# phuang1024/Starst3r

Measured on AMD Instinct MI355X. Metric: 3DGS train iters/sec @ 1M Gaussians, 8x1080p views, higher is better.
Workload: dtype f32

## Files before the change

starst3r_amd/csrc/api.hip:

```cpp
#include <stdarg.h>

#include "stages.h"

static thread_local char g_err[512] = "";

void st3r_set_error(const char* fmt, ...) {
    va_list ap;
    va_start(ap, fmt);
    vsnprintf(g_err, sizeof(g_err), fmt, ap);
    va_end(ap);
}

ST3R_EXPORT int st3r_version(void) { return ST3R_VERSION; }
ST3R_EXPORT const char* st3r_last_error(void) { return g_err; }

ST3R_EXPORT int st3r_ctx_create(int device, st3r_ctx** out) {
    ARG_CHECK(out);
    int ndev = 0;
    HIP_TRY(hipGetDeviceCount(&ndev));
    ARG_CHECK(device >= 0 && device < ndev);
    HIP_TRY(hipSetDevice(device));
    st3r_ctx* c = new (std::nothrow) st3r_ctx();
    if (!c) { st3r_set_error("out of host memory"); return ST3R_ERR_NOMEM; }
    memset(c, 0, sizeof(*c));
    c->device = device;
    hipError_t e = hipHostMalloc((void**)&c->pinned, 64 * sizeof(int64_t), hipHostMallocDefault);
    if (e != hipSuccess) { delete c; st3r_set_error("hipHostMalloc: %s", hipGetErrorString(e)); return ST3R_ERR_HIP; }
    *out = c;
    return ST3R_OK;
}

ST3R_EXPORT int st3r_ctx_destroy(st3r_ctx* ctx) {
    if (!ctx) return ST3R_OK;
    (void)hipSetDevice(ctx->device);
    (void)st3r_comm_destroy(ctx);
    for (int i = 0; i < SLOT_COUNT; ++i)
        if (ctx->slot_ptr[i]) (void)hipFree(ctx->slot_ptr[i]);
    if (ctx->pinned) (void)hipHostFree(ctx->pinned);
    if (ctx->count_event) (void)hipEventDestroy(ctx->count_event);
    if (ctx->peer_event) (void)hipEventDestroy(ctx->peer_event);
    if (ctx->comm_stream) {
        for (int j = 0; j < ST3R_MAX_RANGES; ++j) {
            (void)hipEventDestroy(ctx->ev_range_bwd[j]); (void)hipEventDestroy(ctx->ev_range_red[j]);
        }
        (void)hipStreamDestroy(ctx->comm_stream);
    }
    if (ctx->prof_ev[0][0][0])
        for (int r = 0; r < PROF_RING; ++r)
            for (int st = 0; st < STG_COUNT; ++st)
                for (int k = 0; k < 2; ++k) (void)hipEventDestroy(ctx->prof_ev[r][st][k]);
    delete ctx;
    return ST3R_OK;
}

ST3R_EXPORT int64_t st3r_ctx_arena_bytes(st3r_ctx* ctx) {
    if (!ctx) return 0;
    int64_t t = 0;
    for (int i = 0; i < SLOT_COUNT; ++i) t += (int64_t)ctx->slot_bytes[i];
    return t;
}

int st3r_arena_get(st3r_ctx* ctx, int slot, size_t bytes, void** out) {
    int grown;
    return st3r_arena_get2(ctx, slot, bytes, out, &grown);
}

int st3r_arena_get2(st3r_ctx* ctx, int slot, size_t bytes, void** out, int* grown) {
    *grown = 0;
    if (bytes == 0) bytes = 16;
    if (ctx->slot_bytes[slot] < bytes) {
        size_t want = bytes + bytes / 4;
        want = (want + 255) & ~(size_t)255;
        if (ctx->slot_ptr[slot]) {
            HIP_TRY(hipDeviceSynchronize());
            HIP_TRY(hipFree(ctx->slot_ptr[slot]));
            ctx->slot_ptr[slot] = nullptr; ctx->slot_bytes[slot] = 0;
        }
        hipError_t e = hipMalloc(&ctx->slot_ptr[slot], want);
        if (e != hipSuccess) {
            st3r_set_error("arena slot %d: hipMalloc(%zu) failed: %s", slot, want, hipGetErrorString(e));
            return ST3R_ERR_NOMEM;
        }
        ctx->slot_bytes[slot] = want;
        *grown = 1;
    }
    *out = ctx->slot_ptr[slot];
    return ST3R_OK;
}

ST3R_EXPORT int st3r_ctx_peek(st3r_ctx* ctx, void* stream, int which, void* dst, int64_t bytes) {
    ARG_CHECK(ctx && dst && bytes >= 0 && which >= 0 && which <= 13);
    static const int slots[14] = {SLOT_VALS_B, SLOT_OFFSETS, SLOT_SPLATS, SLOT_CUM,
                                  SLOT_MCMC_CUM, SLOT_MCMC_DEAD, SLOT_MCMC_SAMPLED, SLOT_MCMC_COUNT,
                                  SLOT_RGB, SLOT_ALPHA, SLOT_COUNTS, SLOT_KEYS_A, SLOT_VALS_A, SLOT_KEYS_B};
    ARG_CHECK((size_t)bytes <= ctx->slot_bytes[slots[which]]);
    HIP_TRY(hipMemcpyAsync(dst, ctx->slot_ptr[slots[which]], (size_t)bytes, hipMemcpyDeviceToDevice,
                           (hipStream_t)stream));
    return ST3R_OK;
}

static const char* k_stage_names[STG_COUNT] = {"project", "scan", "emit", "sort", "offsets", "blend_fwd", "loss",
                                               "blend_bwd", "project_bwd", "adam", "sort_depth"};

ST3R_EXPORT const char* st3r_stage_name(int stage) {
    return (stage >= 0 && stage < STG_COUNT) ? k_stage_names[stage] : "";
}

static void prof_harvest_slot(st3r_ctx* ctx, int slot) {
    for (int st = 0; st < STG_COUNT; ++st) {
        if (!ctx->prof_used[slot][st]) continue;
        float ms = 0.f;
        if (hipEventSynchronize(ctx->prof_ev[slot][st][1]) == hipSuccess &&
            hipEventElapsedTime(&ms, ctx->prof_ev[slot][st][0], ctx->prof_ev[slot][st][1]) == hipSuccess) {
            ctx->prof_ms[st] += ms; ctx->prof_n[st] += 1;
        }
        ctx->prof_used[slot][st] = 0;
    }
}

void st3r_prof_begin(st3r_ctx* ctx, hipStream_t s, int stage) {
    if (!((ctx->prof_enabled >> stage) & 1)) return;
    (void)hipEventRecord(ctx->prof_ev[ctx->prof_slot][stage][0], s);
}

void st3r_prof_end(st3r_ctx* ctx, hipStream_t s, int stage) {
    if (!((ctx->prof_enabled >> stage) & 1)) return;
    (void)hipEventRecord(ctx->prof_ev[ctx->prof_slot][stage][1], s);
    ctx->prof_used[ctx->prof_slot][stage] = 1;
}

void st3r_prof_next_step(st3r_ctx* ctx) {
    if (!ctx->prof_enabled) return;
    ctx->prof_slot = (ctx->prof_slot + 1) % PROF_RING;
    prof_harvest_slot(ctx, ctx->prof_slot);
}

ST3R_EXPORT int st3r_ctx_set_debug(st3r_ctx* ctx, int flags) {
    ARG_CHECK(ctx);
    ctx->debug_flags = flags;
    if (flags & 256) {
        ctx->scan_gen = (ctx->scan_gen & 1u) ? 0x3FFDu : 0x3FFEu;
        ctx->scan_gen_b = (ctx->scan_gen_b & 1u) ? 0x3FFDu : 0x3FFEu;
    }
    return ST3R_OK;
}

ST3R_EXPORT int st3r_ctx_set_profiling(st3r_ctx* ctx, int enable) {
    ARG_CHECK(ctx && enable >= 0 && enable < 2 + STG_COUNT);
    if (enable && !ctx->prof_ev[0][0][0]) {
        for (int r = 0; r < PROF_RING; ++r)
            for (int st = 0; st < STG_COUNT; ++st)
                for (int k = 0; k < 2; ++k) HIP_TRY(hipEventCreate(&ctx->prof_ev[r][st][k]));
    }
    ctx->prof_enabled = enable == 0 ? 0 : (enable == 1 ? (1 << STG_COUNT) - 1 : (1 << (enable - 2)));
    return ST3R_OK;
}

ST3R_EXPORT int st3r_ctx_get_stage_ms(st3r_ctx* ctx, double* ms_out, int64_t* counts_out) {
    ARG_CHECK(ctx && ms_out && counts_out);
    HIP_TRY(hipDeviceSynchronize());
    if (ctx->prof_ev[0][0][0])
        for (int r = 0; r < PROF_RING; ++r) prof_harvest_slot(ctx, r);
    for (int st = 0; st < STG_COUNT; ++st) {
        ms_out[st] = ctx->prof_ms[st]; counts_out[st] = ctx->prof_n[st];
        ctx->prof_ms[st] = 0; ctx->prof_n[st] = 0;
    }
    return ST3R_OK;
}

ST3R_EXPORT int st3r_ctx_settle(st3r_ctx* ctx) {
    ARG_CHECK(ctx);
    int rc = st3r_peer_status_settle(ctx);
    if (rc) return rc;
    return st3r_count_settle(ctx);
}

ST3R_EXPORT int st3r_ctx_release_scratch(st3r_ctx* ctx) {
    ARG_CHECK(ctx);
    HIP_TRY(hipDeviceSynchronize());
    const int rc = st3r_ctx_settle(ctx);
    for (int i = 0; i < SLOT_COUNT; ++i) {
        if (ctx->slot_ptr[i]) (void)hipFree(ctx->slot_ptr[i]);
        ctx->slot_ptr[i] = nullptr; ctx->slot_bytes[i] = 0;
    }
    return rc;
}

int st3r_counts_buffer(st3r_ctx* ctx, hipStream_t s, int32_t** out) {
    void* p; int grown = 0;
    int rc = st3r_arena_get2(ctx, SLOT_COUNTS, sizeof(int32_t) * 16, &p, &grown);
    if (rc) return rc;
    if (grown) HIP_TRY(hipMemsetAsync(p, 0, ctx->slot_bytes[SLOT_COUNTS], s));
    *out = (int32_t*)p;
    return ST3R_OK;
}
```

starst3r_amd/csrc/blend_common.h:

```cpp
#pragma once
#include "stages.h"
#include "tile_rect.h"

#define BLK 256
#define LOG2E 1.4426950408889634f

#ifndef XCD_GROUP
#define XCD_GROUP(C, n_tiles, tile_w) (tile_w)
#endif
__device__ __forceinline__ int xcd_remap(int bid, int total, int G) {
    const int n_full = (total / (8 * G)) * (8 * G);
    if (bid >= n_full) return bid;
    const int xcd = bid & 7, k = bid >> 3;
    const int round = k / G, within = k - round * G;
    return (round * 8 + xcd) * G + within;
}

struct TileGeom {
    int lb, cam, i, j, start, end, tx0, ty0;
    bool inside;
    float px, py;
};

__device__ __forceinline__ TileGeom tile_geom(int C, int W, int H, int tile_w, int tile_h,
                                              const int32_t* __restrict__ offsets, int n_isects) {
    TileGeom g;
    const int n_tiles = tile_w * tile_h, total = C * n_tiles;
    g.lb = xcd_remap(blockIdx.x, total, XCD_GROUP(C, n_tiles, tile_w));
    g.cam = g.lb / n_tiles;
    const int tile = g.lb - g.cam * n_tiles;
    const int ty = tile / tile_w, tx = tile - ty * tile_w;
    g.tx0 = tx * 16; g.ty0 = ty * 16;
    const int w = threadIdx.x >> 6, lane = threadIdx.x & 63;
    g.j = g.tx0 + ((w & 1) << 3) + (lane & 7);
    g.i = g.ty0 + ((w >> 1) << 3) + (lane >> 3);
    g.inside = (g.i < H) && (g.j < W);
    g.px = (float)g.j + 0.5f; g.py = (float)g.i + 0.5f;
    g.start = offsets[g.lb];
    g.end = (g.lb == total - 1 && n_isects >= 0) ? n_isects : offsets[g.lb + 1];
    return g;
}

__device__ __forceinline__ uint64_t uniform_u64(uint64_t v) {
    const unsigned lo = __builtin_amdgcn_readfirstlane((unsigned)v);
    const unsigned hi = __builtin_amdgcn_readfirstlane((unsigned)(v >> 32));
    return ((uint64_t)hi << 32) | lo;
}

__device__ __forceinline__ void stage_qform(const float4& a, const float4& b, const float4& c, int t, float4* sR) {
    sR[3 * t + 0] = make_float4(a.x, a.y, a.z, -0.5f * LOG2E * a.w);
    sR[3 * t + 1] = make_float4(-LOG2E * b.x, -0.5f * LOG2E * b.y, b.z, b.w);
    sR[3 * t + 2] = make_float4(c.x, 0.f, 0.f, 0.f);
}

__device__ __forceinline__ int quadrant_relevance(const float4& a, const float4& b, int tx0, int ty0) {
    EllipseTest et;
    if (!ellipse_prepare(a.z, a.w, b.x, b.y, &et)) return 0;
    const float rx = ((float)tx0 + 0.5f) - a.x, ry = ((float)ty0 + 0.5f) - a.y;
    int rel = 0;
#pragma unroll
    for (int q = 0; q < 4; ++q) {
        const float dx0 = rx + (float)((q & 1) * 8), dy0 = ry + (float)((q >> 1) * 8);
        rel |= ellipse_hits_square(et, dx0, dx0 + 7.0f, dy0, dy0 + 7.0f) ? (1 << q) : 0;
    }
    return rel;
}

__device__ __forceinline__ int64_t mask_base(int lb, int start) { return (int64_t)(start >> 6) + 4 * (int64_t)lb; }

__device__ __forceinline__ float blend_power(float dx, float dy, float qa, float qb, float qc) {
#pragma clang fp contract(off)
    const float lx = __builtin_fmaf(dx, qa, qb * dy);
    return __builtin_fmaf(dx, lx, (qc * dy) * dy);
}

__device__ __forceinline__ uint64_t mask_not_less(float a, float b) {
    uint64_t m;
    asm("v_cmp_nlt_f32_e64 %0, %1, %2" : "=s"(m) : "v"(a), "v"(b));
    return m;
}
__device__ __forceinline__ uint64_t mask_not_positive(float a) {
    uint64_t m;
    asm("v_cmp_nlt_f32_e64 %0, 0, %1" : "=s"(m) : "v"(a));
    return m;
}
__device__ __forceinline__ float zero_unless(uint64_t m, float x) {
    float r;
    asm("s_nop 1\n\tv_cndmask_b32_e64 %0, 0, %1, %2" : "=v"(r) : "v"(x), "s"(m));
    return r;
}

__device__ __forceinline__ void reduce9_rows(float g0, float g1, float g2, float g3, float g4, float g5, float g6,
                                             float g7, float g8, float& k0, float& k1, float& k2) {
    float t0, t1, t2, t3, t4;
    asm volatile(
        "s_nop 1\n\t"
        "v_add_f32_dpp %0, %5, %5 row_ror:8 row_mask:0xf bank_mask:0x3\n\t"
        "v_add_f32_dpp %1, %7, %7 row_ror:8 row_mask:0xf bank_mask:0x3\n\t"
        "v_add_f32_dpp %2, %9, %9 row_ror:8 row_mask:0xf bank_mask:0x3\n\t"
        "v_add_f32_dpp %3, %11, %11 row_ror:8 row_mask:0xf bank_mask:0x3\n\t"
        "v_add_f32_dpp %4, %13, %13 row_ror:8 row_mask:0xf bank_mask:0x3\n\t"
        "v_add_f32_dpp %0, %6, %6 row_ror:8 row_mask:0xf bank_mask:0xc\n\t"
        "v_add_f32_dpp %1, %8, %8 row_ror:8 row_mask:0xf bank_mask:0xc\n\t"
        "v_add_f32_dpp %2, %10, %10 row_ror:8 row_mask:0xf bank_mask:0xc\n\t"
        "v_add_f32_dpp %3, %12, %12 row_ror:8 row_mask:0xf bank_mask:0xc"
        : "=&v"(t0), "=&v"(t1), "=&v"(t2), "=&v"(t3), "=&v"(t4)
        : "v"(g0), "v"(g1), "v"(g2), "v"(g3), "v"(g4), "v"(g5), "v"(g6), "v"(g7), "v"(g8));
    float u0, u1, u2;
    asm volatile(
        "s_nop 1\n\t"
        "v_add_f32_dpp %0, %3, %3 row_shl:4 row_mask:0xf bank_mask:0x5\n\t"
        "v_add_f32_dpp %1, %5, %5 row_shl:4 row_mask:0xf bank_mask:0x5\n\t"
        "v_add_f32_dpp %2, %7, %7 row_shl:4 row_mask:0xf bank_mask:0x1\n\t"
        "v_add_f32_dpp %0, %4, %4 row_shr:4 row_mask:0xf bank_mask:0xa\n\t"
        "v_add_f32_dpp %1, %6, %6 row_shr:4 row_mask:0xf bank_mask:0xa"
        : "=&v"(u0), "=&v"(u1), "=&v"(u2)
        : "v"(t0), "v"(t1), "v"(t2), "v"(t3), "v"(t4));
    asm volatile(
        "s_nop 1\n\t"
        "v_add_f32_dpp %0, %0, %0 quad_perm:[1,0,3,2] row_mask:0xf bank_mask:0xf\n\t"
        "v_add_f32_dpp %1, %1, %1 quad_perm:[1,0,3,2] row_mask:0xf bank_mask:0xf\n\t"
        "v_add_f32_dpp %2, %2, %2 quad_perm:[1,0,3,2] row_mask:0xf bank_mask:0xf\n\t"
        "v_add_f32_dpp %0, %0, %0 quad_perm:[2,3,0,1] row_mask:0xf bank_mask:0xf\n\t"
        "v_add_f32_dpp %1, %1, %1 quad_perm:[2,3,0,1] row_mask:0xf bank_mask:0xf\n\t"
        "v_add_f32_dpp %2, %2, %2 quad_perm:[2,3,0,1] row_mask:0xf bank_mask:0xf"
        : "+v"(u0), "+v"(u1), "+v"(u2));
    k0 = u0; k1 = u1; k2 = u2;
}
#define ACC_VALS 9
#define VT_STRIDE (ACC_VALS + 1)
#define DACC_VALS 7
#define DVT_STRIDE (DACC_VALS + 1)
#ifndef HB
#define HB 64
#endif
#define HB_WORDS (HB / 64)
static_assert(HB == 64, "the backward walks one mask word per round");
#ifndef CHUNK
#define CHUNK 4
#endif
#define PAIR_STRIDE 66
#define PAIR_AT(pix) ((pix) + ((pix) >> 5))

__device__ __forceinline__ int slot_of_rectbase(uint64_t r, int tx0, int ty0) {
    const int x0 = (int)(r & 0x3FF), y0 = (int)((r >> 10) & 0x3FF), rw = (int)((r >> 20) & 0x3FF);
    return (int)(r >> 32) + ((ty0 >> 4) - y0) * rw + ((tx0 >> 4) - x0);
}
__device__ __forceinline__ int slot_of_rect(int cum_excl, int x0, int y0, int rw, int tx0, int ty0) {
    return cum_excl + ((ty0 >> 4) - y0) * rw + ((tx0 >> 4) - x0);
}

struct RunSums { float So, Sx, Sxx, Sy, Sxy, Syy; };
__device__ __forceinline__ RunSums run_sums(float W0, float W1, float W2, float d0, float dy) {
    const float So = W0, Sx = fmaf(d0, W0, -W1), Sxx = fmaf(d0, Sx - W1, W2);
    const float Sy = So * dy, Sxy = Sx * dy, Syy = Sy * dy;
    return RunSums{So, Sx, Sxx, Sy, Sxy, Syy};
}

__device__ __forceinline__ void wave_lds_sync() {
    __builtin_amdgcn_fence(__ATOMIC_SEQ_CST, "wavefront");
    __builtin_amdgcn_wave_barrier();
}

__device__ __forceinline__ void store_pair_sums(float4* dst, const float (&acc)[ACC_VALS]) {
    dst[0] = make_float4(acc[0], acc[1], acc[2], acc[3]);
    dst[1] = make_float4(acc[4], acc[5], acc[6], acc[7]);
    dst[2] = make_float4(acc[8], 0.f, 0.f, 0.f);
}
__device__ __forceinline__ void store_pair_sums(float4* dst, const float (&acc)[DACC_VALS]) {
    dst[0] = make_float4(acc[0], acc[1], acc[2], acc[3]);
    dst[1] = make_float4(acc[4], acc[5], 0.f, 0.f);
    dst[2] = make_float4(0.f, acc[6], 0.f, 0.f);
}

template <int NV>
__global__ __launch_bounds__(256) void k_gather_vtile(int64_t n_pairs, const int32_t* __restrict__ cum,
                                                      const float* __restrict__ vtile, int stamp, unsigned vt_cap,
                                                      float4* __restrict__ v_splats) {
    static_assert(NV & 1, "the stamp closes the slot's last 8-byte word");
    constexpr int ROW = NV;
    constexpr int NQ = (NV + 1) / 2;
    __shared__ int sCum[257];
    __shared__ float sVal[256 * ROW];
    const int tid = threadIdx.x;
    const int64_t p0 = (int64_t)blockIdx.x * 256;
    const int np = (int)min((int64_t)256, n_pairs - p0);
    if (tid == 0) sCum[0] = p0 == 0 ? 0 : cum[p0 - 1];
    sCum[tid + 1] = cum[p0 + min(tid, np - 1)];
    __syncthreads();
    const int s0 = sCum[0], s1 = sCum[np];
    const int my_start = sCum[tid], my_end = tid < np ? sCum[tid + 1] : sCum[tid];
    float acc[NV];
#pragma unroll
    for (int k = 0; k < NV; ++k) acc[k] = 0.f;
    float2 q[NQ];
    auto fetch = [&](int u) {
#pragma unroll
        for (int k = 0; k < NQ; ++k) q[k] = make_float2(0.f, 0.f);
        if (u < s1 && (unsigned)u < vt_cap) {
            const float2* src = reinterpret_cast<const float2*>(vtile + (int64_t)u * (NV + 1));
#pragma unroll
            for (int k = 0; k < NQ; ++k) q[k] = src[k];
        }
    };
    fetch(s0 + tid);
    for (int base = s0; base < s1; base += 256) {
        const bool live = __float_as_int(q[NQ - 1].y) == stamp;
        float* row = sVal + tid * ROW;
#pragma unroll
        for (int k = 0; k < NV; ++k) row[k] = live ? ((k & 1) ? q[k >> 1].y : q[k >> 1].x) : 0.f;
        __syncthreads();
        fetch(base + 256 + tid);
        const int lo = max(my_start, base) - base, hi = min(my_end, base + 256) - base;
        for (int r = lo; r < hi; ++r) {
            const float* src = sVal + r * ROW;
#pragma unroll
            for (int k = 0; k < NV; ++k) acc[k] += src[k];
        }
        __syncthreads();
    }
    if (tid < np) store_pair_sums(v_splats + (p0 + tid) * 3, acc);
}

static inline int64_t cmask_words(int64_t n_isects, int64_t total) { return (n_isects >> 6) + 4 * total + 8; }

static int hand_off_buffers(st3r_ctx* ctx, int64_t total, int64_t n_isects, bool allocate, uint64_t** cmask,
                            int64_t* words, int32_t** tile_nb) {
    *words = cmask_words(n_isects, total);
    const size_t cm_bytes = sizeof(uint64_t) * 4 * (size_t)*words, nb_bytes = sizeof(int32_t) * (size_t)total;
    if (allocate) {
        void* p; int rc;
        if ((rc = st3r_arena_get(ctx, SLOT_CMASK, cm_bytes, &p)) || (rc = st3r_arena_get(ctx, SLOT_TILE_NB, nb_bytes, &p)))
            return rc;
    } else if (!ctx->slot_ptr[SLOT_CMASK] || ctx->slot_bytes[SLOT_CMASK] < cm_bytes || !ctx->slot_ptr[SLOT_TILE_NB] ||
               ctx->slot_bytes[SLOT_TILE_NB] < nb_bytes) {
        st3r_set_error("st3r_gs_blend_depth_bwd must follow st3r_gs_blend_fwd of the same lists on the same ctx");
        return ST3R_ERR_INVALID;
    }
    *cmask = (uint64_t*)ctx->slot_ptr[SLOT_CMASK];
    *tile_nb = (int32_t*)ctx->slot_ptr[SLOT_TILE_NB];
    return ST3R_OK;
}

struct StampedSlots { float* vtile; int stamp; unsigned cap; bool restarted; };
static int stamped_slots(st3r_ctx* ctx, hipStream_t s, int slot, int stride, int64_t n_isects, int* stamp_counter,
                         StampedSlots* out) {
    void* p; int grown = 0;
    int rc = st3r_arena_get2(ctx, slot, sizeof(float) * stride * (size_t)n_isects, &p, &grown);
    if (rc) return rc;
    const bool restart = grown || *stamp_counter >= 2147483000;
    if (restart) {
        HIP_TRY(hipMemsetAsync(p, 0, ctx->slot_bytes[slot], s));
        *stamp_counter = 0;
    }
    *out = StampedSlots{(float*)p, ++*stamp_counter, (unsigned)(ctx->slot_bytes[slot] / (sizeof(float) * stride)), restart};
    return ST3R_OK;
}

static int check_blend_args(st3r_ctx* ctx, int C, int width, int height, int tile_size, int tile_w, int tile_h,
                            const float* splats, const int32_t* offsets, const int32_t* flatten_ids, int64_t n_isects) {
    ARG_CHECK(ctx && C > 0 && width > 0 && height > 0 && tile_size == 16);
    ARG_CHECK(tile_w == (width + 15) / 16 && tile_h == (height + 15) / 16);
    ARG_CHECK(splats && offsets && n_isects >= 0 && n_isects < 2147483647LL);
    ARG_CHECK(n_isects == 0 || flatten_ids);
    return ST3R_OK;
}
```

starst3r_amd/csrc/common.h:

```cpp
#pragma once
#include <hip/hip_runtime.h>
#include <stdint.h>
#include <stdio.h>
#include <string.h>

#include "../../include/st3r.h"

#define ST3R_EXPORT extern "C" __attribute__((visibility("default")))

void st3r_set_error(const char* fmt, ...);

#define HIP_TRY(expr)                                                                              \
    do {                                                                                           \
        hipError_t _e = (expr);                                                                    \
        if (_e != hipSuccess) {                                                                    \
            st3r_set_error("%s:%d: %s -> %s", __FILE__, __LINE__, #expr, hipGetErrorString(_e));   \
            return ST3R_ERR_HIP;                                                                   \
        }                                                                                          \
    } while (0)

#define ARG_CHECK(cond)                                                                    \
    do {                                                                                   \
        if (!(cond)) {                                                                     \
            st3r_set_error("%s:%d: invalid argument: %s", __FILE__, __LINE__, #cond);      \
            return ST3R_ERR_INVALID;                                                       \
        }                                                                                  \
    } while (0)

#define LAUNCH_CHECK() HIP_TRY(hipGetLastError())

enum ArenaSlot {
    SLOT_SPLATS = 0,
    SLOT_TILES,
    SLOT_CUM,
    SLOT_KEYS_A,
    SLOT_KEYS_B,
    SLOT_VALS_A,
    SLOT_VALS_B,
    SLOT_OFFSETS,
    SLOT_RGB,
    SLOT_ALPHA,
    SLOT_LAST,
    SLOT_VRENDER,
    SLOT_VSPLATS,
    SLOT_SSIM_A,
    SLOT_SORT_TMP,
    SLOT_SCAN_TMP,
    SLOT_SMALL,
    SLOT_CMASK,
    SLOT_TILE_NB,
    SLOT_VTILE,
    SLOT_DKEYS_A,
    SLOT_DKEYS_B,
    SLOT_DVALS_A,
    SLOT_DVALS_B,
    SLOT_CUM_D,
    SLOT_NN_PART,
    SLOT_MCMC_CUM,
    SLOT_MCMC_DEAD,
    SLOT_MCMC_RANK,
    SLOT_MCMC_COUNT,
    SLOT_MCMC_SAMPLED,
    SLOT_MCMC_BINOMS,
    SLOT_REG_PART,
    SLOT_RECTS,
    SLOT_RECTS_D,
    SLOT_RECTBASE,
    SLOT_COUNTS,
    SLOT_PSTAGE,
    SLOT_GSTAGE,
    SLOT_ALIGN_CTL,
    SLOT_PAIR_TOUCH,
    SLOT_KRANGE_PART,
    SLOT_SCAN_CHAIN,
    SLOT_POSE_PART,
    SLOT_VTILE_DEPTH,
    SLOT_DEPTH_PART,
    SLOT_POSE_GRAD,
    SLOT_DEPTH,
    SLOT_VDEPTH,
    SLOT_VALPHA,
    SLOT_VSPLATS_D,
    SLOT_DPRIOR_PART,
    SLOT_DPRIOR_NORM,
    SLOT_DPRIOR_SUMS,
    SLOT_EXPOSURE_PART,
    SLOT_SCAN_CHAIN_B,
    SLOT_EXPOSED,
    SLOT_KGRAD_PART,
    SLOT_LWEIGHT_PART,
    SLOT_LWEIGHT_NORM,
    SLOT_COUNT
};

enum Stage {
    STG_PROJECT = 0,
    STG_SCAN,
    STG_EMIT,
    STG_SORT,
    STG_OFFSETS,
    STG_BLEND_FWD,
    STG_LOSS,
    STG_BLEND_BWD,
    STG_PROJECT_BWD,
    STG_ADAM,
    STG_SORT_DEPTH,
    STG_COUNT
};
#define PROF_RING 64
#define ST3R_MAX_RANGES 8

#define ST3R_SPLIT_VIEWS 1000

struct st3r_vtile_ref { const int32_t* cum; const float* vtile; int stamp; unsigned vt_cap; const uint32_t* touch; };

struct ViewReg { const float* gt; int c, h, w; };

static inline int64_t view_reg_first(const ViewReg& r, const float* gt, int C, int H, int W) {
    if (!r.gt || H != r.h || W != r.w) return -1;
    const int64_t img = (int64_t)H * W * 3;
    if (gt < r.gt || (gt - r.gt) % img != 0) return -1;
    const int64_t c0 = (gt - r.gt) / img;
    return c0 + C <= r.c ? c0 : -1;
}

static inline int view_reg_set(ViewReg* r, bool on, const float* gt, int C, int height, int width) {
    if (!on) { *r = ViewReg{}; return ST3R_OK; }
    ARG_CHECK(C > 0 && height > 0 && width > 0);
    *r = ViewReg{gt, C, height, width};
    return ST3R_OK;
}

struct st3r_ctx {
    int device;
    void* slot_ptr[SLOT_COUNT];
    size_t slot_bytes[SLOT_COUNT];
    int64_t* pinned;
    int debug_flags;
    ViewReg gtm; const float* gtm_mom;
    ViewReg dp; const float* dp_depth; const float* dp_weight; float dp_fac; int dp_norm_valid;
    ViewReg ex; const float* ex_exposure; float* ex_v_exposure;
    ViewReg kg; float* kg_v_Ks;
    ViewReg lw; const float* lw_weight; int lw_norm_valid;
    int bwd_stamp;
    int depth_stamp;
    uint32_t scan_gen;
    uint32_t scan_gen_b;
    int64_t isect_hint, count_cap;
    int64_t hint_sig;
    int count_pending;
    int view_chunks;
    hipEvent_t count_event;
    void* comm;
    int comm_owned, comm_rank, comm_size;
    int exchange;
    int comm_broken;
    int peer_pending;
    hipEvent_t peer_event;
    hipStream_t comm_stream;
    hipEvent_t ev_range_bwd[ST3R_MAX_RANGES], ev_range_red[ST3R_MAX_RANGES];
    void* xwin;
    int n_ranges;
    int ranges_recorded;
    int prof_enabled;
    hipEvent_t prof_ev[PROF_RING][STG_COUNT][2];
    unsigned char prof_used[PROF_RING][STG_COUNT];
    int prof_slot;
    double prof_ms[STG_COUNT];
    int64_t prof_n[STG_COUNT];
};

void st3r_prof_begin(st3r_ctx* ctx, hipStream_t s, int stage);
void st3r_prof_end(st3r_ctx* ctx, hipStream_t s, int stage);
void st3r_prof_next_step(st3r_ctx* ctx);

int st3r_arena_get(st3r_ctx* ctx, int slot, size_t bytes, void** out);
int st3r_arena_get2(st3r_ctx* ctx, int slot, size_t bytes, void** out, int* grown);
#define ARENA_GET(slot, type, count, var)                                                    \
    type* var;                                                                               \
    {                                                                                        \
        void* _p;                                                                            \
        int _rc = st3r_arena_get(ctx, slot, sizeof(type) * (size_t)(count), &_p);            \
        if (_rc) return _rc;                                                                 \
        var = (type*)_p;                                                                     \
    }

#define ST3R_BAND_TAB 257

static inline int ceil_div(int64_t a, int64_t b) { return (int)((a + b - 1) / b); }
static inline int bit_length_u32(uint32_t v) { int n = 0; while (v) { ++n; v >>= 1; } return n; }
```

starst3r_amd/csrc/fused_step.hip:

```cpp
#include "radix_sort.h"
#include "stages.h"

int st3r_count_settle(st3r_ctx* ctx) {
    if (!ctx->count_pending) return ST3R_OK;
    HIP_TRY(hipEventSynchronize(ctx->count_event));
    ctx->count_pending = 0;
    const int64_t n = (int64_t)((int32_t*)(ctx->pinned + 8))[0];
    if (n < 0) {
        ctx->isect_hint = 0;
        ctx->view_chunks = (ctx->view_chunks > 0 ? ctx->view_chunks : 1) * 2;
        st3r_set_error("the previous step produced more than 2^31 tile intersections: its gradients were incomplete -- "
                       "repeat it (st3r_gs_train_fwd_bwd / st3r_gs_train_step now walk the views in %d chunks)",
                       ctx->view_chunks);
        return ST3R_ERR_CAPACITY;
    }
    if (n > ctx->count_cap) {
        ctx->isect_hint = 0;
        st3r_set_error("the previous step produced %lld tile intersections, more than the %lld its buffers were sized "
                       "for from the step before (+25 %%): its gradients were incomplete and st3r_adam_step / "
                       "st3r_gs_train_step did NOT apply them (the update is guarded on the device) -- repeat that step",
                       (long long)n, (long long)ctx->count_cap);
        return ST3R_ERR_CAPACITY;
    }
    ctx->isect_hint = n;
    return ST3R_OK;
}

struct FrontPlan {
    int tile_w, tile_h;
    bool key32;
    bool segments;
    int rect32;
    bool rectbase;
    uint32_t key_base;
    int l1_end_bit;
    int end_bit;
};
static const float k_near_plane = 0.01f, k_far_plane = 1e10f;
static FrontPlan front_plan(int C, int W, int H, int debug_flags, bool with_reg, bool records) {
    FrontPlan p;
    const int tile = 16;
    p.tile_w = (W + tile - 1) / tile; p.tile_h = (H + tile - 1) / tile;
    uint32_t near_bits, far_bits;
    memcpy(&near_bits, &k_near_plane, 4); memcpy(&far_bits, &k_far_plane, 4);
    p.key32 = (C <= 8) && (far_bits - near_bits < 0x1FFFFFFFu);
    p.key_base = p.key32 ? near_bits : 0u;
    p.rect32 = (p.tile_w <= 255 && p.tile_h <= 255 && !(debug_flags & 64)) ? 1 : 0;
    p.segments = p.key32 && with_reg && !records && !(debug_flags & 4);
    p.l1_end_bit = (p.key32 ? 29 : 32) + bit_length_u32((uint32_t)(C - 1));
    p.rectbase = p.tile_w <= 1023 && p.tile_h <= 1023 && !(debug_flags & 64);
    p.end_bit = bit_length_u32((uint32_t)((int64_t)C * p.tile_w * p.tile_h - 1));
    return p;
}

static int rasterize_front(st3r_ctx* ctx, hipStream_t s, const GsParams& g, const GsViews& v, double* reg_sums, int tight,
                           const float* records_in, bool allow_async, RasterOut* o, double* loss_sums = nullptr) {
    const int N = g.N, C = v.C, W = v.W, H = v.H;
    const int tile = 16;
    const FrontPlan fp = front_plan(C, W, H, ctx->debug_flags, reg_sums != nullptr, records_in != nullptr);
    const int tile_w = fp.tile_w, tile_h = fp.tile_h;
    const int64_t n_pairs = (int64_t)N * C;
    float* splats = const_cast<float*>(records_in);
    if (!records_in) {
        ARENA_GET(SLOT_SPLATS, float, n_pairs * ST3R_SPLAT_STRIDE, own);
        splats = own;
    }
    ARENA_GET(SLOT_CUM, int32_t, n_pairs, cum);
    ARENA_GET(SLOT_OFFSETS, int32_t, (int64_t)C * tile_w * tile_h + 1, offsets);
    const float near_plane = k_near_plane, far_plane = k_far_plane;
    const bool key32 = fp.key32;
    ARENA_GET(SLOT_DKEYS_A, uint64_t, n_pairs, dkeys_a);
    ARENA_GET(SLOT_DKEYS_B, uint64_t, n_pairs, dkeys_b);
    ARENA_GET(SLOT_DVALS_A, int32_t, n_pairs, dvals_a);
    ARENA_GET(SLOT_DVALS_B, int32_t, n_pairs, perm);
    const int rect32 = fp.rect32;
    ARENA_GET(SLOT_RECTS, uint64_t, rect32 ? (n_pairs + 1) / 2 : n_pairs, rects);
    int32_t* counts = nullptr;
    { int rc_ = st3r_counts_buffer(ctx, s, &counts); if (rc_) return rc_; }
    uint32_t* const krange = fp.segments ? (uint32_t*)(counts + 8) : nullptr;
    st3r_prof_begin(ctx, s, STG_PROJECT);
    const uint32_t key_base = fp.key_base;
    int rc = records_in
                 ? st3r_records_prepare_impl(s, N, C, splats, tile, tile_w, tile_h, tight, nullptr, dkeys_a, dvals_a,
                                             key_base, rects, rect32)
                 : st3r_project_impl(ctx, s, g, v, tile, 0.3f, near_plane, far_plane, 0.0f, splats, nullptr, reg_sums,
                                     dkeys_a, dvals_a, tight, key_base, rects, rect32, 1, loss_sums, 2 * C, krange);
    if (!rc && records_in && loss_sums) HIP_TRY(hipMemsetAsync(loss_sums, 0, sizeof(double) * 2 * (size_t)C, s));
    st3r_prof_end(ctx, s, STG_PROJECT);
    if (rc) return rc;
    st3r_prof_begin(ctx, s, STG_SORT_DEPTH);
    rc = krange ? st3r_radix_sort_u32_segments(ctx, s, N, C, (uint32_t*)dkeys_a, dvals_a, (uint32_t*)dkeys_b, perm, krange)
         : key32 ? st3r_radix_sort_u32(ctx, s, n_pairs, 0, fp.l1_end_bit, (uint32_t*)dkeys_a, dvals_a, (uint32_t*)dkeys_b, perm, nullptr)
                 : st3r_radix_sort_u64(ctx, s, n_pairs, 0, fp.l1_end_bit, dkeys_a, dvals_a, dkeys_b, perm);
    st3r_prof_end(ctx, s, STG_SORT_DEPTH);
    if (rc) return rc;
    int64_t n_isects = 0;
    st3r_prof_begin(ctx, s, STG_SCAN);
    uint64_t* rectbase = nullptr;
    if (fp.rectbase) {
        ARENA_GET(SLOT_RECTBASE, uint64_t, n_pairs, rb);
        rectbase = rb;
    }
    const int64_t sig = ((int64_t)N << 34) ^ ((int64_t)C << 26) ^ ((int64_t)W << 13) ^ (int64_t)H;
    const bool async = allow_async && ctx->isect_hint > 0 && ctx->hint_sig == sig;
    int32_t* total_dev = nullptr;
    rc = st3r_isect_scan_impl(ctx, s, n_pairs, nullptr, cum, nullptr, rects, rect32, rectbase, &total_dev,
                              async ? counts : nullptr, async ? (int32_t*)(ctx->pinned + 8) : nullptr);
    st3r_prof_end(ctx, s, STG_SCAN);
    if (rc) return rc;
    if (async) {
        if (!ctx->count_event) HIP_TRY(hipEventCreateWithFlags(&ctx->count_event, hipEventDisableTiming));
        HIP_TRY(hipEventRecord(ctx->count_event, s));
        n_isects = ctx->isect_hint + ctx->isect_hint / 4 + 1024;
        if (ctx->debug_flags & 8) n_isects = ctx->isect_hint / 2;
        if (n_isects > 2147483647LL) n_isects = 2147483647LL;
        ctx->count_pending = 1; ctx->count_cap = n_isects;
        o->n_visible = -1; o->n_isects_ref = -1;
    } else {
        HIP_TRY(hipMemcpyAsync(ctx->pinned, total_dev, sizeof(int32_t), hipMemcpyDeviceToHost, s));
        if (reg_sums) HIP_TRY(hipMemcpyAsync(ctx->pinned + 1, reg_sums + 2, 2 * sizeof(double), hipMemcpyDeviceToHost, s));
        HIP_TRY(hipStreamSynchronize(s));
        n_isects = (int64_t)((int32_t*)ctx->pinned)[0];
        if (n_isects < 0) {
            st3r_set_error("more than 2^31 tile intersections in one call: split the views over more calls / GPUs");
            return ST3R_SPLIT_VIEWS;
        }
        o->n_visible = reg_sums ? (int64_t)((double*)ctx->pinned)[1] : -1;
        o->n_isects_ref = reg_sums ? (int64_t)((double*)ctx->pinned)[2] : n_isects;
        if (allow_async) { ctx->isect_hint = n_isects; ctx->hint_sig = sig; }
    }
    ARENA_GET(SLOT_KEYS_A, uint32_t, n_isects, tkeys_a);
    ARENA_GET(SLOT_KEYS_B, uint32_t, n_isects, tkeys_b);
    ARENA_GET(SLOT_VALS_A, int32_t, n_isects, vals_a);
    ARENA_GET(SLOT_VALS_B, int32_t, n_isects, vals_b);
    o->n_records = async ? -1 : n_isects;
    const int64_t n_keys = (int64_t)C * tile_w * tile_h;
    const uint32_t* band_table = nullptr;
    const uint32_t* band_hist = nullptr;
    int n_bands = 0;
    if (n_isects > 0) {
        const int end_bit = fp.end_bit;
        const bool banded = st3r_sort_tile_banded(end_bit, ctx->debug_flags) != 0;
        const bool packed = banded && n_pairs <= (1 << 24) && !(ctx->debug_flags & 1024);
        n_bands = (int)((n_keys - 1) >> 8) + 1;
        st3r_prof_begin(ctx, s, STG_EMIT);
        rc = st3r_isect_emit_chain_impl(ctx, s, N, C, perm, rects, rect32, tile_w, tile_h, packed ? nullptr : tkeys_a, vals_a,
                                        n_isects, banded ? st3r_radix_sort_band_tile(n_isects) : 0, total_dev, &band_table);
        st3r_prof_end(ctx, s, STG_EMIT);
        if (rc) return rc;
        st3r_prof_begin(ctx, s, STG_SORT);
        rc = packed ? st3r_radix_sort_u32_banded_packed(ctx, s, n_isects, n_bands, band_table, (const uint32_t*)vals_a, vals_b,
                                                        &band_hist)
             : banded ? st3r_radix_sort_u32_banded(ctx, s, n_isects, n_bands, band_table, tkeys_a, vals_a, tkeys_b, vals_b)
                      : st3r_sort_tile_impl(ctx, s, n_isects, end_bit, tkeys_a, vals_a, tkeys_b, vals_b, total_dev);
        st3r_prof_end(ctx, s, STG_SORT);
        if (rc) return rc;
    }
    st3r_prof_begin(ctx, s, STG_OFFSETS);
    rc = band_hist ? st3r_radix_band_offsets(s, n_bands, band_table, band_hist, n_keys, offsets)
                   : st3r_isect_offsets32_impl(s, n_isects, tkeys_b, C, tile_w, tile_h, offsets, total_dev);
    st3r_prof_end(ctx, s, STG_OFFSETS);
    if (rc) return rc;
    o->C = C; o->W = W; o->H = H; o->tile_w = tile_w; o->tile_h = tile_h;
    o->splats = splats; o->offsets = offsets; o->flat = vals_b; o->cum = cum; o->rects = rect32 ? nullptr : rects;
    o->rectbase = rectbase;
    o->tight = tight; o->n_pairs = n_pairs;
    o->n_isects = n_isects;
    return ST3R_OK;
}

__global__ void k_finalize_loss(int C, const double* __restrict__ sums, const double* __restrict__ reg_sums,
                                double inv_px, double inv_cnt, double w_l1, double w_ssim, double reg_views,
                                double opac_k, double scale_k, float* __restrict__ loss_out,
                                const double* __restrict__ dsums, const double* __restrict__ dnorm, double depth_fac,
                                const double* __restrict__ wnorm) {
    if (threadIdx.x == 0 && blockIdx.x == 0) {
        double loss = 0;
        if (wnorm)
            for (int c = 0; c < C; ++c)
                loss += w_l1 * sums[2 * c] / (3.0 * fmax(wnorm[2 * c], 1.0)) +
                        w_ssim * (3.0 * wnorm[2 * c + 1] - sums[2 * c + 1]) / (3.0 * fmax(wnorm[2 * c + 1], 1.0));
        else
            for (int c = 0; c < C; ++c) loss += w_l1 * sums[2 * c] * inv_px + w_ssim * (1.0 - sums[2 * c + 1] * inv_cnt);
        loss += reg_views * (opac_k * reg_sums[0] + scale_k * reg_sums[1]);
        if (dsums)
            for (int c = 0; c < C; ++c) loss += depth_fac * dsums[c] / dnorm[c];
        loss_out[0] = (float)loss;
    }
}

static int finalize_loss(hipStream_t s, int C, int H, int W, const double* sums, const double* reg_sums, float ssim_fac,
                         double reg_views, double opac_k, double scale_k, float* loss_out, const double* dp_sums,
                         const DepthPrior& dp, const LossWeight& lw) {
    const int Hi = H - 10, Wi = W - 10;
    const double cnt = (Hi > 0 && Wi > 0) ? (double)Hi * Wi * 3 : 0.0;
    hipLaunchKernelGGL(k_finalize_loss, dim3(1), dim3(64), 0, s, C, sums, reg_sums, 1.0 / ((double)H * W * 3),
                       cnt > 0 ? 1.0 / cnt : 0.0, (double)(1.0f - ssim_fac), (double)ssim_fac, reg_views, opac_k, scale_k,
                       loss_out, dp_sums, dp.norm, (double)dp.fac, lw.weight ? lw.norm : nullptr);
    LAUNCH_CHECK();
    return ST3R_OK;
}

struct LossFacs { float ssim, opac, scale; };

struct ViewBatch {
    GsViews v;
    const float* gt;
    double* sums;
    double* dp_sums;
    float* v_viewmats;
    bool exposure;
    bool weighted;
    ViewBatch slice(int c0, int c1) const {
        return {v.slice(c0, c1), gt + (int64_t)c0 * v.H * v.W * 3, sums + 2 * c0, dp_sums ? dp_sums + c0 : nullptr,
                v_viewmats ? v_viewmats + 16 * c0 : nullptr, exposure, weighted};
    }
};

struct StepImages { float *rgb, *alpha; int32_t* last; float *v_rgb, *depth, *v_depth, *v_alpha, *exposed; };

static int step_images(st3r_ctx* ctx, const RasterOut& ro, bool with_depth, bool with_exposure, StepImages* im) {
    const int64_t n_px = (int64_t)ro.C * ro.H * ro.W;
    ARENA_GET(SLOT_RGB, float, n_px * 3, rgb);
    ARENA_GET(SLOT_ALPHA, float, n_px, alpha);
    ARENA_GET(SLOT_LAST, int32_t, n_px, last);
    ARENA_GET(SLOT_VRENDER, float, n_px * 3, v_rgb);
    *im = StepImages{rgb, alpha, last, v_rgb, nullptr, nullptr, nullptr, nullptr};
    if (with_exposure) {
        ARENA_GET(SLOT_EXPOSED, float, n_px * 3, exposed);
        im->exposed = exposed;
    }
    if (with_depth) {
        ARENA_GET(SLOT_DEPTH, float, n_px, depth);
        ARENA_GET(SLOT_VDEPTH, float, n_px, v_depth);
        ARENA_GET(SLOT_VALPHA, float, n_px, v_alpha);
        im->depth = depth; im->v_depth = v_depth; im->v_alpha = v_alpha;
    }
    return ST3R_OK;
}

static int forward_and_losses(st3r_ctx* ctx, hipStream_t s, const RasterOut& ro, const ViewBatch& b, float ssim_fac,
                              bool sums_cleared, const DepthPrior& dp, const ExposureReg& ex, const LossWeight& lw,
                              const StepImages& im) {
    const bool eio = true;
    st3r_prof_begin(ctx, s, STG_BLEND_FWD);
    int rc = st3r_blend_fwd_impl(ctx, s, ro, im.rgb, im.alpha, im.last, true, eio);
    if (!rc && dp.prior) rc = st3r_blend_depth_fwd_impl(ctx, s, ro, im.last, im.depth, eio);
    st3r_prof_end(ctx, s, STG_BLEND_FWD);
    if (rc) return rc;
    st3r_prof_begin(ctx, s, STG_LOSS);
    if (ex.exposure) rc = st3r_exposure_fwd_impl(s, ro.C, ro.H, ro.W, im.rgb, ex.exposure, im.exposed);
    if (!rc)
        rc = st3r_loss_impl(ctx, s, ro.C, ro.H, ro.W, ex.exposure ? im.exposed : im.rgb, b.gt, 1.0f - ssim_fac, ssim_fac,
                            b.sums, im.v_rgb, sums_cleared, lw);
    if (!rc && ex.exposure)
        rc = st3r_exposure_bwd_impl(ctx, s, ro.C, ro.H, ro.W, im.rgb, ex.exposure, im.v_rgb, im.v_rgb, ex.v_exposure);
    if (!rc && dp.prior)
        rc = st3r_depth_prior_loss_impl(ctx, s, ro.C, ro.H, ro.W, im.depth, im.alpha, dp.prior, dp.weight, dp.norm, 1, dp.fac,
                                        b.dp_sums, 1, im.v_depth, im.v_alpha);
    st3r_prof_end(ctx, s, STG_LOSS);
    return rc;
}

static int blend_backward(st3r_ctx* ctx, hipStream_t s, const RasterOut& ro, const StepImages& im, bool need_pairs,
                          st3r_vtile_ref* slots, float* v_pairs) {
    RasterOut rb = ro;
    if (ctx->debug_flags & 2) { rb.rects = nullptr; rb.rectbase = nullptr; }
    const bool eio = true;
    st3r_prof_begin(ctx, s, STG_BLEND_BWD);
    int rc = st3r_blend_bwd_impl(ctx, s, rb, im.alpha, im.last, im.v_rgb, im.v_alpha, nullptr, eio, slots);
    if (!rc && need_pairs) {
        ARENA_GET(SLOT_VSPLATS_D, float, ro.n_pairs * ST3R_SPLAT_STRIDE, v_pairs_d);
        rc = st3r_blend_depth_bwd_impl(ctx, s, rb, im.alpha, im.last, im.v_depth, v_pairs_d, eio);
        if (!rc) {
            if (slots->vtile) rc = st3r_gather_vtile_impl(s, ro.n_pairs, slots, v_pairs);
            else HIP_TRY(hipMemsetAsync(v_pairs, 0, sizeof(float) * ST3R_SPLAT_STRIDE * (size_t)ro.n_pairs, s));
        }
        if (!rc) rc = st3r_add_pairs_impl(s, ro.n_pairs, v_pairs, v_pairs_d);
    }
    st3r_prof_end(ctx, s, STG_BLEND_BWD);
    return rc;
}

static int project_backward(st3r_ctx* ctx, hipStream_t s, const GsParams& g, const GsViews& v, const RasterOut& ro,
                            const LossFacs& f, const float* v_pairs, const st3r_vtile_ref* slots, bool accumulate,
                            float* grads) {
    ctx->ranges_recorded = 0;
    if (!(ctx->n_ranges > 1 && ctx->comm_stream))
        return st3r_project_sh_bwd_impl(s, g, v, 0.3f, ro.splats, v_pairs, (float)v.C, f.opac, f.scale, grads, accumulate, 0,
                                        -1, false, slots);
    ARENA_GET(SLOT_GSTAGE, float, (int64_t)23 * g.N, gstage);
    const int K = ctx->n_ranges;
    for (int j = 0; j < K; ++j) {
        const int g0 = (int)((int64_t)g.N * j / K), g1 = (int)((int64_t)g.N * (j + 1) / K);
        int rc = st3r_project_sh_bwd_impl(s, g, v, 0.3f, ro.splats, v_pairs, (float)v.C, f.opac, f.scale, gstage, accumulate,
                                          g0, g1, true, slots);
        if (rc) return rc;
        HIP_TRY(hipEventRecord(ctx->ev_range_bwd[j], s));
    }
    ctx->ranges_recorded = K;
    return ST3R_OK;
}

static int pose_backward(st3r_ctx* ctx, hipStream_t s, const GsParams& g, const GsViews& v, const RasterOut& ro,
                         const float* v_pairs, float* v_viewmats) {
    return st3r_gs_viewmat_bwd(ctx, s, g.N, v.C, g.means, g.quats, g.scales, g.sh, g.sh_stride, v.viewmats, v.Ks, v.campos,
                               v.W, v.H, 0.3f, ro.splats, v_pairs, v_viewmats);
}

static int train_views(st3r_ctx* ctx, hipStream_t s, const GsParams& g, const ViewBatch& b, const LossFacs& f,
                       double* reg_sums, bool allow_async, bool accumulate, float* grads, RasterOut* ro_out) {
    const GsViews& v = b.v;
    DepthPrior dp{};
    int rc = b.dp_sums ? st3r_depth_prior_for(ctx, s, b.gt, v.C, v.H, v.W, &dp) : ST3R_OK;
    if (rc) return rc;
    ExposureReg ex{};
    if (b.exposure) st3r_exposure_for(ctx, b.gt, v.C, v.H, v.W, &ex);
    LossWeight lw{};
    if (b.weighted) rc = st3r_loss_weight_for(ctx, s, b.gt, v.C, v.H, v.W, &lw);
    if (rc) return rc;
    const bool need_pairs = dp.prior != nullptr;
    RasterOut& ro = *ro_out;
    rc = rasterize_front(ctx, s, g, v, reg_sums, 1, nullptr, allow_async, &ro, b.sums);
    if (rc) return rc;
    StepImages im;
    rc = step_images(ctx, ro, need_pairs, ex.exposure != nullptr, &im);
    if (rc) return rc;
    float* const v_Ks = st3r_intrinsics_grad_for(ctx, b.gt, v.C, v.H, v.W);
    float* v_pairs = nullptr;
    if (need_pairs || b.v_viewmats || v_Ks) {
        ARENA_GET(SLOT_VSPLATS, float, ro.n_pairs * ST3R_SPLAT_STRIDE, vp);
        v_pairs = vp;
    }
    rc = forward_and_losses(ctx, s, ro, b, f.ssim, true, dp, ex, lw, im);
    if (rc) return rc;
    st3r_vtile_ref slots{};
    rc = blend_backward(ctx, s, ro, im, need_pairs, &slots, v_pairs);
    if (rc) return rc;
    st3r_prof_begin(ctx, s, STG_PROJECT_BWD);
    rc = project_backward(ctx, s, g, v, ro, f, need_pairs ? v_pairs : nullptr, need_pairs ? nullptr : &slots, accumulate,
                          grads);
    if (!rc && need_pairs && b.v_viewmats) rc = pose_backward(ctx, s, g, v, ro, v_pairs, b.v_viewmats);
    if (!rc && need_pairs) rc = st3r_gs_depth_bwd(ctx, s, g.N, v.C, g.means, v.viewmats, ro.splats, v_pairs, grads, b.v_viewmats);
    st3r_prof_end(ctx, s, STG_PROJECT_BWD);
    if (!rc && !need_pairs && (b.v_viewmats || v_Ks)) {
        rc = st3r_gather_vtile_impl(s, ro.n_pairs, &slots, v_pairs);
        if (!rc && b.v_viewmats) rc = pose_backward(ctx, s, g, v, ro, v_pairs, b.v_viewmats);
    }
    if (!rc && v_Ks)
        rc = st3r_gs_intrinsics_bwd(ctx, s, g.N, v.C, g.means, g.quats, g.scales, v.viewmats, v.Ks, v.W, v.H, 0.3f,
                                    ro.splats, v_pairs, v_Ks);
    return rc;
}

static int train_chunks(st3r_ctx* ctx, hipStream_t s, const GsParams& g, const ViewBatch& all, const LossFacs& f,
                        double* reg_sums, double* reg_scratch, bool want_stats, float* grads, int* chunks, int64_t stats[3]) {
    const int C = all.v.C;
    for (;;) {
        int rc = ST3R_OK;
        stats[0] = stats[1] = stats[2] = 0;
        bool first = true;
        for (int k = 0; k < *chunks && !rc; ++k) {
            const int c0 = (int)((int64_t)k * C / *chunks), c1 = (int)((int64_t)(k + 1) * C / *chunks);
            if (c1 == c0) continue;
            RasterOut ro;
            rc = train_views(ctx, s, g, all.slice(c0, c1), f, first ? reg_sums : reg_scratch,
                             !want_stats && *chunks == 1 && !ctx->comm, !first, grads, &ro);
            if (!rc) { stats[0] += ro.n_visible; stats[1] += ro.n_records; stats[2] += ro.n_isects_ref; }
            first = false;
        }
        if (rc == ST3R_SPLIT_VIEWS && *chunks < C) {
            *chunks = *chunks * 2 < C ? *chunks * 2 : C;
            continue;
        }
        return rc == ST3R_SPLIT_VIEWS ? ST3R_ERR_INVALID : rc;
    }
}

int st3r_train_fwd_bwd_impl(st3r_ctx* ctx, hipStream_t s, const GsParams& g, const GsViews& v, const float* gt_images,
                            float ssim_fac, float opac_fac, float scale_fac, float* grads, float* loss_out,
                            int64_t* stats_host, float* v_viewmats) {
    const int N = g.N, C = v.C;
    ARG_CHECK(ctx && N > 0 && C > 0 && C <= ST3R_MAX_VIEWS && v.W > 0 && v.H > 0 && g.sh_stride >= 12);
    ARG_CHECK((int64_t)N * C < 2147483647LL);
    ARG_CHECK(g.means && g.quats && g.scales && g.opacities && g.sh && v.viewmats && v.Ks && v.campos && gt_images && grads &&
              loss_out);
    ARENA_GET(SLOT_SMALL, double, 2 * (size_t)C + 12, small);
    double* sums = small;
    double* reg_sums = small + 2 * C;
    double* dp_sums = nullptr;
    DepthPrior dp;
    int rc = st3r_depth_prior_for(ctx, s, gt_images, C, v.H, v.W, &dp);
    if (rc) return rc;
    if (dp.prior) {
        if (ctx->comm) {
            st3r_set_error("a depth prior is registered and a communicator is attached -- the depth term is not "
                           "supported in view-sharded training (clear it with st3r_ctx_set_depth_prior(ctx, NULL, ...))");
            return ST3R_ERR_INVALID;
        }
        ARENA_GET(SLOT_DPRIOR_SUMS, double, (size_t)C, ds);
        dp_sums = ds;
    }
    ExposureReg ex;
    st3r_exposure_for(ctx, gt_images, C, v.H, v.W, &ex);
    if (ex.exposure && ctx->comm) {
        st3r_set_error("exposures are registered and a communicator is attached -- per-view exposures are not supported "
                       "in view-sharded training (clear them with st3r_ctx_set_exposure(ctx, NULL, ...))");
        return ST3R_ERR_INVALID;
    }
    if (ctx->comm && st3r_intrinsics_grad_for(ctx, gt_images, C, v.H, v.W)) {
        st3r_set_error("an intrinsics gradient is registered and a communicator is attached -- intrinsics refinement is "
                       "not supported in view-sharded training (clear it with st3r_ctx_set_intrinsics_grad(ctx, NULL, ...))");
        return ST3R_ERR_INVALID;
    }
    LossWeight lw;
    rc = st3r_loss_weight_for(ctx, s, gt_images, C, v.H, v.W, &lw);
    if (rc) return rc;
    if (lw.weight && ctx->comm) {
        st3r_set_error("loss weights are registered and a communicator is attached -- per-pixel loss weights are not "
                       "supported in view-sharded training (clear them with st3r_ctx_set_loss_weight(ctx, NULL, ...))");
        return ST3R_ERR_INVALID;
    }
    st3r_prof_next_step(ctx);
    rc = st3r_count_settle(ctx);
    if (rc) return rc;
    int chunks = ctx->view_chunks > 0 ? ctx->view_chunks : 1;
    if ((ctx->debug_flags & 32) && chunks < 2) chunks = 2;
    if (chunks > C) chunks = C;
    int64_t stats[3];
    rc = train_chunks(ctx, s, g, ViewBatch{v, gt_images, sums, dp_sums, v_viewmats, ex.exposure != nullptr, lw.weight != nullptr},
                      LossFacs{ssim_fac, opac_fac, scale_fac},
                      reg_sums, reg_sums + 4, stats_host != nullptr, grads, &chunks, stats);
    if (rc) return rc;
    if (chunks > 1) ctx->view_chunks = chunks;
    rc = finalize_loss(s, C, v.H, v.W, sums, reg_sums, ssim_fac, (double)C, (double)opac_fac / N,
                       (double)scale_fac / (3.0 * N), loss_out, dp_sums, dp, lw);
    if (rc) return rc;
    if (stats_host) {
        stats_host[0] = stats[0]; stats_host[1] = stats[1]; stats_host[2] = st3r_ctx_arena_bytes(ctx);
        stats_host[3] = stats[2];
    }
    return ST3R_OK;
}

ST3R_EXPORT int st3r_gs_train_fwd_bwd(st3r_ctx* ctx, void* stream, int N, int C, const float* means,
                                      const float* quats, const float* scales, const float* opacities,
                                      const float* sh, int sh_stride, const float* viewmats, const float* Ks,
                                      const float* campos, const float* gt_images, int width, int height,
                                      float ssim_fac, float opac_fac, float scale_fac, float* grads,
                                      float* loss_out, int64_t* stats_host) {
    return st3r_train_fwd_bwd_impl(ctx, (hipStream_t)stream, GsParams{N, means, quats, scales, opacities, sh, sh_stride},
                                   GsViews{C, width, height, viewmats, Ks, campos}, gt_images, ssim_fac, opac_fac,
                                   scale_fac, grads, loss_out, stats_host, nullptr);
}

ST3R_EXPORT int st3r_gs_raster_train(st3r_ctx* ctx, void* stream, int N, int C, const float* records,
                                     const float* gt_images, int width, int height, float ssim_fac,
                                     float* v_records, float* loss_out, int64_t* stats_host) {
    ARG_CHECK(ctx && N > 0 && C > 0 && width > 0 && height > 0 && records && gt_images && v_records && loss_out);
    ARG_CHECK(C <= ST3R_MAX_VIEWS && (int64_t)N * C < 2147483647LL);
    hipStream_t s = (hipStream_t)stream;
    ARENA_GET(SLOT_SMALL, double, 2 * (size_t)C + 8, sums);
    double* reg_sums = sums + 2 * C;
    const ViewBatch b{GsViews{C, width, height}, gt_images, sums, nullptr, nullptr, false, false};
    HIP_TRY(hipMemsetAsync(reg_sums, 0, sizeof(double) * 4, s));
    st3r_prof_next_step(ctx);
    RasterOut ro;
    int rc = st3r_count_settle(ctx);
    if (rc) return rc;
    rc = rasterize_front(ctx, s, GsParams{N}, b.v, nullptr, 1, records, stats_host == nullptr, &ro);
    if (rc == ST3R_SPLIT_VIEWS) rc = ST3R_ERR_INVALID;
    if (rc) return rc;
    StepImages im;
    rc = step_images(ctx, ro, false, false, &im);
    if (rc) return rc;
    rc = forward_and_losses(ctx, s, ro, b, ssim_fac, false, DepthPrior{}, ExposureReg{}, LossWeight{}, im);
    if (rc) return rc;
    st3r_prof_begin(ctx, s, STG_BLEND_BWD);
    rc = st3r_blend_bwd_impl(ctx, s, ro, im.alpha, im.last, im.v_rgb, nullptr, v_records, true, nullptr);
    st3r_prof_end(ctx, s, STG_BLEND_BWD);
    if (rc) return rc;
    rc = finalize_loss(s, C, height, width, sums, reg_sums, ssim_fac, 0.0, 0.0, 0.0, loss_out, nullptr, DepthPrior{},
                       LossWeight{});
    if (rc) return rc;
    if (stats_host) {
        stats_host[0] = -1; stats_host[1] = ro.n_records; stats_host[2] = st3r_ctx_arena_bytes(ctx); stats_host[3] = -1;
    }
    return ST3R_OK;
}

ST3R_EXPORT int st3r_gs_render(st3r_ctx* ctx, void* stream, int N, int C, const float* means, const float* quats,
                               const float* scales, const float* opacities, const float* sh, int sh_stride,
                               const float* viewmats, const float* Ks, const float* campos, int width, int height,
                               float* rgb, float* alpha, int64_t* stats_host) {
    ARG_CHECK(ctx && N > 0 && C > 0 && width > 0 && height > 0 && sh_stride >= 12);
    ARG_CHECK(C <= ST3R_MAX_VIEWS && (int64_t)N * C < 2147483647LL);
    ARG_CHECK(means && quats && scales && opacities && sh && viewmats && Ks && campos && rgb && alpha);
    hipStream_t s = (hipStream_t)stream;
    RasterOut ro;
    int rc = st3r_count_settle(ctx);
    if (rc) return rc;
    rc = rasterize_front(ctx, s, GsParams{N, means, quats, scales, opacities, sh, sh_stride},
                         GsViews{C, width, height, viewmats, Ks, campos}, nullptr, 0, nullptr, false, &ro);
    if (rc == ST3R_SPLIT_VIEWS) rc = ST3R_ERR_INVALID;
    if (rc) return rc;
    ARENA_GET(SLOT_LAST, int32_t, (int64_t)C * height * width, last);
    rc = st3r_blend_fwd_impl(ctx, s, ro, rgb, alpha, last, false, true);
    if (rc) return rc;
    if (stats_host) {
        stats_host[0] = -1; stats_host[1] = ro.n_records; stats_host[2] = st3r_ctx_arena_bytes(ctx); stats_host[3] = 0;
    }
    return ST3R_OK;
}

ST3R_EXPORT int st3r_front_plan(int N, int C, int width, int height, int debug_flags, int training, int records,
                                int64_t n_records, int64_t* out, int n_out) {
    ARG_CHECK(N > 0 && C > 0 && C <= ST3R_MAX_VIEWS && width > 0 && height > 0 && n_records >= 0 && out &&
              n_out >= ST3R_FRONT_PLAN_WORDS && !(training && records));
    const FrontPlan fp = front_plan(C, width, height, debug_flags, training != 0, records != 0);
    const int64_t n_pairs = (int64_t)N * C;
    for (int i = 0; i < n_out; ++i) out[i] = 0;
    out[0] = fp.rect32; out[1] = fp.rectbase; out[2] = fp.key32; out[3] = fp.segments;
    out[4] = st3r_scan_tiles(n_pairs);
    int bpc, grid, self_base;
    st3r_emit_grid(N, C, &bpc, &grid, &self_base);
    out[5] = bpc; out[6] = grid; out[7] = self_base;
    int64_t sh[8];
    if (fp.segments) st3r_radix_sort_shape(4, n_pairs, N, C, 0, 0, sh);
    else st3r_radix_sort_shape(fp.key32 ? 4 : 8, n_pairs, 0, 0, 0, fp.l1_end_bit, sh);
    out[8] = sh[0]; out[9] = sh[1]; out[10] = sh[2]; out[11] = sh[3]; out[12] = sh[4];
    out[25] = sh[5];
    out[fp.key32 ? 26 : 28] = sh[6]; out[fp.key32 ? 27 : 29] = sh[7];
    st3r_radix_sort_shape(fp.key32 ? 8 : 4, 1, 0, 0, 0, 8, sh);
    out[fp.key32 ? 28 : 26] = sh[6]; out[fp.key32 ? 29 : 27] = sh[7];
    out[13] = st3r_sort_tile_end_bit(fp.end_bit);
    if (n_records > 0) {
        st3r_radix_sort_shape(4, n_records, 0, 0, 0, (int)out[13], sh);
        out[14] = sh[0]; out[15] = sh[1]; out[16] = sh[2]; out[17] = sh[4];
    }
    if (st3r_sort_tile_banded(fp.end_bit, debug_flags)) {
        out[18] = 1;
        out[19] = (((int64_t)C * fp.tile_w * fp.tile_h - 1) >> 8) + 1;
        if (n_records > 0) out[30] = n_records / st3r_radix_sort_band_tile(n_records) + out[19];
    }
    int64_t k[5];
    st3r_isect_constants(k);
    for (int i = 0; i < 5; ++i) out[20 + i] = k[i];
    return ST3R_OK;
}
```

starst3r_amd/csrc/gs_blend.hip:

```cpp
#include <type_traits>

#include "stages.h"
#include "tile_rect.h"
#include "blend_common.h"

__device__ __forceinline__ int stage_record(const float4* __restrict__ splats, int64_t id, int t, int tx0, int ty0,
                                            float4* sR) {
    const float4 a = splats[id * 3 + 0];
    const float4 b = splats[id * 3 + 1];
    const float4 c = splats[id * 3 + 2];
    stage_qform(a, b, c, t, sR);
    return quadrant_relevance(a, b, tx0, ty0);
}

template <bool TRAIN>
__global__ __launch_bounds__(BLK) void k_blend_fwd(int C, int W, int H, int tile_w, int tile_h,
                                                   const float4* __restrict__ splats,
                                                   const int32_t* __restrict__ offsets,
                                                   const int32_t* __restrict__ flat, int n_isects,
                                                   float* __restrict__ out_rgb, float* __restrict__ out_alpha,
                                                   int32_t* __restrict__ last_ids,
                                                   uint64_t* __restrict__ cmask, int64_t cmask_words,
                                                   int32_t* __restrict__ tile_nb, int no_cull) {
    __shared__ float4 sR[BLK * 3];
    __shared__ uint64_t sMask[4][4];
    const TileGeom g = tile_geom(C, W, H, tile_w, tile_h, offsets, n_isects);
    const int w = threadIdx.x >> 6, lane = threadIdx.x & 63;
    float thr = g.inside ? 1.f / 255.f : __builtin_inff();
    float T = 1.0f, r = 0.f, gg = 0.f, b = 0.f;
    int cur = TRAIN ? 0x7fffffff : 0;
    int nb = 0;
    const int64_t mbase = mask_base(g.lb, g.start);
    for (int bs = g.start; bs < g.end; bs += BLK, ++nb) {
        if (__syncthreads_and(thr > 1.0f)) break;
        const int idx = bs + threadIdx.x;
        int rel = 0;
        if (idx < g.end) {
            rel = stage_record(splats, flat[idx], threadIdx.x, g.tx0, g.ty0, sR);
            if (no_cull) rel = 0xF;
        }
        const uint64_t m0 = __ballot(rel & 1), m1 = __ballot(rel & 2), m2 = __ballot(rel & 4), m3 = __ballot(rel & 8);
        if (lane == 0) { sMask[0][w] = m0; sMask[1][w] = m1; sMask[2][w] = m2; sMask[3][w] = m3; }
        __syncthreads();
#pragma unroll 1
        for (int jj = 0; jj < 4; ++jj) {
            uint64_t m64 = uniform_u64(sMask[w][jj]);
            uint64_t contributed = 0;
            if (__builtin_amdgcn_ballot_w64(thr < 1.0f) == 0) m64 = 0;
#pragma unroll 1
            for (int hh = 0; hh < 2; ++hh) {
            uint32_t m = hh ? (uint32_t)(m64 >> 32) : (uint32_t)m64;
            uint32_t cont32 = 0;
            while (m) {
                const int bit = __builtin_ctz(m);
                m &= m - 1;
                const int t = jj * 64 + hh * 32 + bit;
                const float4 a = sR[3 * t];
                const float4 q = sR[3 * t + 1];
                const float cb = sR[3 * t + 2].x;
                const float dx = a.x - g.px, dy = a.y - g.py;
                const float P = blend_power(dx, dy, a.w, q.x, q.y);
                const float al0 = fminf(0.999f, a.z * __builtin_amdgcn_exp2f(P));
                uint64_t okm = 0;
                bool ok = false;
                float al;
                if (TRAIN) {
                    okm = mask_not_positive(P) & mask_not_less(al0, thr);
                    al = zero_unless(okm, al0);
                } else {
                    ok = !(P > 0.f) && !(al0 < thr);
                    al = ok ? al0 : 0.f;
                }
                const float nT = T * (1.0f - al);
                const bool stop = nT <= 1e-4f;
                float vis = al * T;
                uint64_t tm;
                if (TRAIN) {
                    tm = okm;
                    float Tn = nT;
                    if (__builtin_expect(__builtin_amdgcn_ballot_w64(stop) != 0, 0)) {
                        thr = stop ? __builtin_inff() : thr;
                        vis = stop ? 0.0f : vis;
                        Tn = stop ? T : nT;
                        cur = stop ? bs + t : cur;
                        tm = okm & ~__builtin_amdgcn_ballot_w64(stop);
                    }
                    T = Tn;
                } else {
                    thr = stop ? __builtin_inff() : thr;
                    al = stop ? 0.0f : al;
                    vis = al * T;
                    T = stop ? T : nT;
                    const bool took = al > 0.0f;
                    cur = took ? bs + t : cur;
                    tm = __builtin_amdgcn_ballot_w64(took);
                }
                r = __builtin_fmaf(q.z, vis, r); gg = __builtin_fmaf(q.w, vis, gg); b = __builtin_fmaf(cb, vis, b);
                cont32 |= tm ? (1u << bit) : 0u;
            }
            contributed |= (uint64_t)cont32 << (32 * hh);
            }
            if (cmask && lane == 0) cmask[(int64_t)w * cmask_words + mbase + nb * 4 + jj] = contributed;
        }
    }
    if (g.inside) {
        const int64_t p = ((int64_t)g.cam * H + g.i) * W + g.j;
        out_rgb[3 * p] = r; out_rgb[3 * p + 1] = gg; out_rgb[3 * p + 2] = b;
        out_alpha[p] = 1.0f - T;
        last_ids[p] = TRAIN ? (cur == 0x7fffffff ? cur : cur - 1) : cur;
    }
    if (tile_nb && threadIdx.x == 0) tile_nb[g.lb] = nb;
}

int st3r_blend_fwd_impl(st3r_ctx* ctx, hipStream_t s, const RasterOut& ro, float* rgb, float* alpha, int32_t* last_ids,
                        bool for_backward, bool end_in_offsets) {
    const int C = ro.C, W = ro.W, H = ro.H, tile_w = ro.tile_w, tile_h = ro.tile_h;
    const int total = C * tile_w * tile_h;
    uint64_t* cmask = nullptr; int64_t words = 0; int32_t* tile_nb = nullptr;
    if (for_backward) {
        int rc = hand_off_buffers(ctx, total, ro.n_isects, true, &cmask, &words, &tile_nb);
        if (rc) return rc;
    }
    if ((for_backward && end_in_offsets && !(ctx->debug_flags & 128)) || (end_in_offsets && (ctx->debug_flags & 512)))
        return st3r_blend_fwd_cells_impl(ctx, s, ro, rgb, alpha, last_ids, cmask, words, tile_nb);
    if (for_backward && end_in_offsets)
        hipLaunchKernelGGL(k_blend_fwd<true>, dim3(total), dim3(BLK), 0, s, C, W, H, tile_w, tile_h, (const float4*)ro.splats,
                           ro.offsets, ro.flat, -1, rgb, alpha, last_ids, cmask, words, tile_nb, ctx->debug_flags & 1);
    else
        hipLaunchKernelGGL(k_blend_fwd<false>, dim3(total), dim3(BLK), 0, s, C, W, H, tile_w, tile_h, (const float4*)ro.splats,
                           ro.offsets, ro.flat, end_in_offsets ? -1 : (int)ro.n_isects, rgb, alpha, last_ids, cmask, words, tile_nb,
                           ctx->debug_flags & 1);
    LAUNCH_CHECK();
    return ST3R_OK;
}

ST3R_EXPORT int st3r_gs_blend_fwd(st3r_ctx* ctx, void* stream, int C, int width, int height, int tile_size,
                                  int tile_w, int tile_h, const float* splats, const int32_t* offsets,
                                  const int32_t* flatten_ids, int64_t n_isects, float* rgb, float* alpha,
                                  int32_t* last_ids) {
    if (int rc = check_blend_args(ctx, C, width, height, tile_size, tile_w, tile_h, splats, offsets, flatten_ids, n_isects))
        return rc;
    ARG_CHECK(rgb && alpha && last_ids);
    return st3r_blend_fwd_impl(ctx, (hipStream_t)stream,
                               stage_lists(C, width, height, tile_w, tile_h, splats, offsets, flatten_ids, n_isects), rgb,
                               alpha, last_ids, true, false);
}

__device__ __forceinline__ void bwd_phase2(const float2* __restrict__ pr, unsigned tpack, int cnt, int lane, const float4* sA, float* accw, float qxf_lane, float qyf_lane,
                                           const float (&pvr)[CHUNK], const float (&pvg)[CHUNK],
                                           const float (&pvb)[CHUNK]) {
    static_assert(CHUNK == 4, "one DPP row per record of the chunk");
    const int r = lane >> 4, part = lane & 15;
    wave_lds_sync();
    const int t = (tpack >> (8 * r)) & 0xFF;
    const float2 mean = *reinterpret_cast<const float2*>(&sA[t]);
    const float dy = mean.y - qyf_lane;
    const float2* src = pr + r * PAIR_STRIDE + PAIR_AT(part * CHUNK);
    float W0 = 0.f, W1 = 0.f, W2 = 0.f, Sr = 0.f, Sg = 0.f, Sb = 0.f;
#pragma unroll
    for (int i = 0; i < CHUNK; ++i) {
        const float2 v = src[i];
        W0 += v.x;
        if (i == 1) { W1 = v.x; W2 = v.x; }
        if (i > 1) { W1 = fmaf((float)i, v.x, W1); W2 = fmaf((float)(i * i), v.x, W2); }
        Sr = fmaf(v.y, pvr[i], Sr); Sg = fmaf(v.y, pvg[i], Sg); Sb = fmaf(v.y, pvb[i], Sb);
    }
    const RunSums m = run_sums(W0, W1, W2, mean.x - qxf_lane, dy);
    float k0, k1, k2;
    reduce9_rows(m.Sx, m.Sy, m.So, m.Sxx, m.Sxy, m.Syy, Sr, Sg, Sb, k0, k1, k2);
    if (r < cnt && (lane & 3) == 0) {
        const int b = (lane >> 2) & 3;
        const int slot0 = ((b & 1) << 1) | (b >> 1);
        float* acc = accw + t * ACC_VALS;
        acc[slot0] = k0;
        acc[4 + slot0] = k1;
        if (b == 0) acc[8] = k2;
    }
    wave_lds_sync();
}

template <bool HAS_VA, bool TOUCH = false>
__global__ __launch_bounds__(BLK) __attribute__((amdgpu_waves_per_eu(8))) void k_blend_bwd(int C, int W, int H, int tile_w, int tile_h,
                                                   const float4* __restrict__ splats,
                                                   const int32_t* __restrict__ offsets,
                                                   const int32_t* __restrict__ flat, int n_isects,
                                                   const float* __restrict__ out_alpha,
                                                   const int32_t* __restrict__ last_ids,
                                                   const float* __restrict__ v_rgb,
                                                   const float* __restrict__ v_alpha,
                                                   const uint64_t* __restrict__ cmask, int64_t cmask_words,
                                                   const int32_t* __restrict__ tile_nb,
                                                   const int32_t* __restrict__ cum,
                                                   const uint64_t* __restrict__ rects,
                                                   const uint64_t* __restrict__ rectbase, int tight,
                                                   float* __restrict__ vtile, int stamp, unsigned vt_cap) {

    __shared__ float4 sA[HB];
    __shared__ float4 sB[HB];
    __shared__ float sC[HB];
    __shared__ float sAccW[4][HB * ACC_VALS];
    __shared__ float2 sPair[4][CHUNK * PAIR_STRIDE];
    __shared__ uint64_t sClampW;
    const TileGeom g = tile_geom(C, W, H, tile_w, tile_h, offsets, n_isects);
    const int nb = tile_nb[g.lb];
    if (nb == 0) return;
    const int w = threadIdx.x >> 6, lane = threadIdx.x & 63;
    const int64_t p = ((int64_t)g.cam * H + g.i) * W + g.j;
    float T_final = 1.0f, vr = 0.f, vg = 0.f, vb = 0.f, va = 0.f;
    int bin_final = -1;
    if (g.inside) {
        T_final = 1.0f - out_alpha[p];
        vr = v_rgb[3 * p]; vg = v_rgb[3 * p + 1]; vb = v_rgb[3 * p + 2];
        if (HAS_VA) va = v_alpha[p];
        bin_final = last_ids[p];
    }
    const bool chk_index = __builtin_amdgcn_ballot_w64(bin_final != 0x7fffffff) != 0;
    float2* pr = sPair[w];
    float* accw = sAccW[w];
    float pvr[CHUNK], pvg[CHUNK], pvb[CHUNK];
    const int pbase = (lane & 15) * CHUNK;
    {
        float* px = reinterpret_cast<float*>(pr);
        px[lane] = vr; px[64 + lane] = vg; px[128 + lane] = vb;
        wave_lds_sync();
#pragma unroll
        for (int i = 0; i < CHUNK; ++i) { pvr[i] = px[pbase + i]; pvg[i] = px[64 + pbase + i]; pvb[i] = px[128 + pbase + i]; }
        wave_lds_sync();
    }
    const float qxf = (float)(g.tx0 + ((w & 1) << 3) + (pbase & 7)) + 0.5f;
    const float qyf_part = (float)(g.ty0 + ((w >> 1) << 3) + (pbase >> 3)) + 0.5f;
    float k_big = 0x1p64f, k_neg_thr = -__int_as_float(0x3b808080) * 0x1p64f;
    asm volatile("" : "+v"(k_big), "+v"(k_neg_thr));
    float T = T_final;
    float bv = 0.f;
    const int64_t mbase = mask_base(g.lb, g.start);
    const uint64_t* wmask = cmask + (int64_t)__builtin_amdgcn_readfirstlane(w) * cmask_words + mbase;
    uint64_t m_next = wmask[(BLK / HB) * nb - 1];
    for (int hb = (BLK / HB) * nb - 1; hb >= 0; --hb) {
        const int bs = g.start + hb * HB;
        const int bsz = min(HB, g.end - bs);
        const uint64_t m_cur = m_next;
        if (hb > 0) m_next = wmask[hb - 1];
        if (bsz <= 0) continue;
        int my_u = -1, my_cb = 0;
        float my_op = 0.f, my_ca = 0.f, my_cbb = 0.f, my_cc = 0.f;
        if ((int)threadIdx.x < bsz) {
            const int t = threadIdx.x;
            const int64_t my_id = flat[bs + t];
            const int64_t word = mbase + hb;
#pragma unroll
            for (int ww = 0; ww < 4; ++ww) my_cb |= (int)((cmask[ww * cmask_words + word] >> (t & 63)) & 1ull) << ww;
            float4 a = make_float4(0.f, 0.f, 0.f, 0.f), b = a, c = a;
            if (my_cb)
            {
                a = splats[my_id * 3 + 0];
                b = splats[my_id * 3 + 1];
                c = splats[my_id * 3 + 2];
                sA[t] = make_float4(a.x, a.y, a.z, -0.5f * LOG2E * a.w);
                sB[t] = make_float4(-LOG2E * b.x, -0.5f * LOG2E * b.y, b.z, b.w);
                sC[t] = c.x;
            }
            const float det_ = a.w * b.y - b.x * b.x;
            const bool hard = my_cb && !(a.z <= 0.998f && a.w > 0.f && b.y > 0.f && det_ >= 2e-3f * (a.w * b.y));
            const uint64_t cw = __builtin_amdgcn_ballot_w64(hard);
            if (t == 0) sClampW = cw;
            if (my_cb && rectbase) {
                if (TOUCH) reinterpret_cast<uint32_t*>(const_cast<uint64_t*>(rects))[my_id] = (uint32_t)stamp;
                my_u = slot_of_rectbase(rectbase[my_id], g.tx0, g.ty0);
                my_op = a.z; my_ca = a.w; my_cbb = b.x; my_cc = b.y;
            } else if (my_cb) {
                int x0, y0, rw;
                if (rects) {
                    const uint64_t r = rects[my_id];
                    x0 = (int)(r & 0xFFFF); y0 = (int)((r >> 16) & 0xFFFF); rw = (int)((r >> 32) & 0xFFFF);
                } else {
                    TileRect tr = ref_tile_rect(a.x, a.y, (float)__float_as_int(c.z), 16, tile_w, tile_h);
                    if (tight) tr = tight_tile_rect(tr, a.x, a.y, a.z, a.w, b.x, b.y);
                    x0 = tr.x0; y0 = tr.y0; rw = tr.x1 - tr.x0;
                }
                const int cum_excl = my_id == 0 ? 0 : cum[my_id - 1];
                my_u = slot_of_rect(cum_excl, x0, y0, rw, g.tx0, g.ty0);
                my_op = a.z; my_ca = a.w; my_cbb = b.x; my_cc = b.y;
            }
        }
        __syncthreads();
        auto walk = [&](auto chk_tag, auto clamp_tag) {
            constexpr bool CHK = decltype(chk_tag)::value, CLAMP = decltype(clamp_tag)::value;
            uint64_t m = m_cur;
            while (m) {
                unsigned tpack = 0;
                int cnt = 0;
#pragma unroll
                for (int k = 0; k < CHUNK; ++k) {
                    if (m) {
                        const int t = 63 - __builtin_clzll(m);
                        m &= ~(1ull << t);
                        const float4 a = sA[t];
                        const float4 q = sB[t];
                        const float cb_ = sC[t];
                        const float dx = a.x - g.px, dy = a.y - g.py;
                        const float P = blend_power(dx, dy, a.w, q.x, q.y);
                        const float vis0 = __builtin_amdgcn_exp2f(P);
                        const float ov0 = a.z * vis0;
                        float alpha;
                        if (CLAMP) {
                            const float al0 = fminf(0.999f, ov0);
                            uint64_t okm = mask_not_positive(P) & mask_not_less(al0, 1.f / 255.f);
                            if (CHK) okm &= __builtin_amdgcn_ballot_w64(bs + t <= bin_final);
                            alpha = zero_unless(okm, al0);
                        } else {
                            float step;
                            asm("v_fma_f32 %0, %1, %2, %3 clamp" : "=v"(step) : "v"(ov0), "v"(k_big), "v"(k_neg_thr));
                            alpha = ov0 * step;
                            if (CHK) alpha = zero_unless(__builtin_amdgcn_ballot_w64(bs + t <= bin_final), alpha);
                        }
                        float alpha_u = alpha;
                        if (CLAMP) alpha_u = ov0 <= 0.999f ? alpha : 0.f;
                        const float ra = __builtin_amdgcn_rcpf(1.0f - alpha);
                        const float cv = q.z * vr + q.w * vg + cb_ * vb;
                        T *= ra;
                        const float fac = alpha * T;
                        float v_al = cv * T - bv * ra;
                        if (HAS_VA) v_al += T_final * ra * va;
                        bv += cv * fac;
                        pr[k * PAIR_STRIDE + PAIR_AT(lane)] = make_float2(alpha_u * v_al, fac);
                        tpack |= (unsigned)t << (8 * k);
                        cnt = k + 1;
                    }
                }
                bwd_phase2(pr, tpack, cnt, lane, sA, accw, qxf, qyf_part, pvr, pvg, pvb);
            }
        };
        const bool clamp_round = (uniform_u64(sClampW) & m_cur) != 0;
        if (chk_index) {
            if (clamp_round) walk(std::true_type{}, std::true_type{}); else walk(std::true_type{}, std::false_type{});
        } else {
            if (clamp_round) walk(std::false_type{}, std::true_type{}); else walk(std::false_type{}, std::false_type{});
        }
        __syncthreads();
        if (my_cb && (unsigned)my_u < vt_cap) {
            float acc[ACC_VALS];
#pragma unroll
            for (int k = 0; k < ACC_VALS; ++k) acc[k] = 0.f;
#pragma unroll
            for (int ww = 0; ww < 4; ++ww) {
                if (my_cb & (1 << ww)) {
#pragma unroll
                    for (int k = 0; k < ACC_VALS; ++k) acc[k] += sAccW[ww][threadIdx.x * ACC_VALS + k];
                }
            }
            const float sx = -acc[0], sy = -acc[1];
            float2* dst = reinterpret_cast<float2*>(vtile + (int64_t)my_u * VT_STRIDE);
            dst[0] = make_float2(my_ca * sx + my_cbb * sy, my_cbb * sx + my_cc * sy);
            dst[1] = make_float2(my_op != 0.f ? acc[2] / my_op : 0.f, -0.5f * acc[3]);
            dst[2] = make_float2(-acc[4], -0.5f * acc[5]);
            dst[3] = make_float2(acc[6], acc[7]);
            dst[4] = make_float2(acc[8], __int_as_float(stamp));
        }
    }
}

int st3r_blend_bwd_impl(st3r_ctx* ctx, hipStream_t s, const RasterOut& ro, const float* alpha, const int32_t* last_ids,
                        const float* v_rgb, const float* v_alpha, float* v_splats, bool end_in_offsets,
                        st3r_vtile_ref* defer) {
    const int C = ro.C, W = ro.W, H = ro.H, tile_w = ro.tile_w, tile_h = ro.tile_h, tight = ro.tight;
    const int32_t* cum = ro.cum; const uint64_t* rects = ro.rects; const uint64_t* rectbase = ro.rectbase;
    const int64_t n_isects = ro.n_isects, n_pairs = ro.n_pairs;
    if (defer) *defer = st3r_vtile_ref{cum, nullptr, 0, 0u, nullptr};
    if (n_isects == 0) {
        if (!defer) HIP_TRY(hipMemsetAsync(v_splats, 0, sizeof(float) * ST3R_SPLAT_STRIDE * (size_t)n_pairs, s));
        return ST3R_OK;
    }
    const int total = C * tile_w * tile_h;
    uint64_t* cmask; int64_t words; int32_t* tile_nb;
    int rc = hand_off_buffers(ctx, total, n_isects, true, &cmask, &words, &tile_nb);
    if (rc) return rc;
    StampedSlots sl;
    rc = stamped_slots(ctx, s, SLOT_VTILE, VT_STRIDE, n_isects, &ctx->bwd_stamp, &sl);
    if (rc) return rc;
    uint32_t* touch = nullptr;
    int grown_t = 0;
    if (defer && rectbase && !v_alpha && n_isects > 8 * n_pairs) {
        void* pt;
        rc = st3r_arena_get2(ctx, SLOT_PAIR_TOUCH, sizeof(uint32_t) * (size_t)n_pairs, &pt, &grown_t);
        if (rc) return rc;
        touch = (uint32_t*)pt;
    }
    if (sl.restarted) {
        if (ctx->slot_ptr[SLOT_PAIR_TOUCH])
            HIP_TRY(hipMemsetAsync(ctx->slot_ptr[SLOT_PAIR_TOUCH], 0, ctx->slot_bytes[SLOT_PAIR_TOUCH], s));
    } else if (grown_t) {
        HIP_TRY(hipMemsetAsync(touch, 0, ctx->slot_bytes[SLOT_PAIR_TOUCH], s));
    }
    const auto kernel = v_alpha ? k_blend_bwd<true> : touch ? k_blend_bwd<false, true> : k_blend_bwd<false>;
    hipLaunchKernelGGL(kernel, dim3(total), dim3(BLK), 0, s, C, W, H, tile_w, tile_h, (const float4*)ro.splats, ro.offsets,
                       ro.flat, end_in_offsets ? -1 : (int)n_isects, alpha, last_ids, v_rgb, v_alpha, cmask, words, tile_nb, cum,
                       touch ? reinterpret_cast<const uint64_t*>(touch) : rects, rectbase, tight, sl.vtile, sl.stamp, sl.cap);
    LAUNCH_CHECK();
    if (defer) { *defer = st3r_vtile_ref{cum, sl.vtile, sl.stamp, sl.cap, touch}; return ST3R_OK; }
    hipLaunchKernelGGL(k_gather_vtile<ACC_VALS>, dim3(ceil_div(n_pairs, 256)), dim3(256), 0, s, n_pairs, cum, sl.vtile,
                       sl.stamp, sl.cap, (float4*)v_splats);
    LAUNCH_CHECK();
    return ST3R_OK;
}

int st3r_gather_vtile_impl(hipStream_t s, int64_t n_pairs, const st3r_vtile_ref* slots, float* v_splats) {
    if (n_pairs <= 0) return ST3R_OK;
    hipLaunchKernelGGL(k_gather_vtile<ACC_VALS>, dim3(ceil_div(n_pairs, 256)), dim3(256), 0, s, n_pairs, slots->cum,
                       slots->vtile, slots->stamp, slots->vt_cap, (float4*)v_splats);
    LAUNCH_CHECK();
    return ST3R_OK;
}

ST3R_EXPORT int st3r_gs_blend_bwd(st3r_ctx* ctx, void* stream, int C, int width, int height, int tile_size,
                                  int tile_w, int tile_h, const float* splats, const int32_t* offsets,
                                  const int32_t* flatten_ids, int64_t n_isects, const float* alpha,
                                  const int32_t* last_ids, const float* v_rgb, const float* v_alpha,
                                  const int32_t* cum_tiles, int64_t n_pairs, float* v_splats) {
    if (int rc = check_blend_args(ctx, C, width, height, tile_size, tile_w, tile_h, splats, offsets, flatten_ids, n_isects))
        return rc;
    ARG_CHECK(alpha && last_ids && v_rgb && v_splats && cum_tiles && n_pairs >= 0);
    return st3r_blend_bwd_impl(ctx, (hipStream_t)stream,
                               stage_lists(C, width, height, tile_w, tile_h, splats, offsets, flatten_ids, n_isects, cum_tiles,
                                           n_pairs),
                               alpha, last_ids, v_rgb, v_alpha, v_splats, false, nullptr);
}
```

starst3r_amd/csrc/gs_blend_depth.hip:

```cpp
#include <type_traits>

#include "stages.h"
#include "tile_rect.h"
#include "blend_common.h"
#include "per_view.h"

__device__ __forceinline__ int stage_record_depth(const float4* __restrict__ splats, int64_t id, int t, int tx0, int ty0,
                                                  float4* sR) {
    const float4 a = splats[id * 3 + 0];
    const float4 b = splats[id * 3 + 1];
    const float z = reinterpret_cast<const float*>(splats)[id * 12 + 9];
    sR[2 * t + 0] = make_float4(a.x, a.y, a.z, -0.5f * LOG2E * a.w);
    sR[2 * t + 1] = make_float4(-LOG2E * b.x, -0.5f * LOG2E * b.y, z, 0.f);
    return quadrant_relevance(a, b, tx0, ty0);
}

__global__ __launch_bounds__(BLK) void k_blend_depth_fwd(int C, int W, int H, int tile_w, int tile_h,
                                                         const float4* __restrict__ splats,
                                                         const int32_t* __restrict__ offsets,
                                                         const int32_t* __restrict__ flat, int n_isects,
                                                         const int32_t* __restrict__ last_ids,
                                                         float* __restrict__ out_depth) {
    __shared__ float4 sR[BLK * 2];
    __shared__ uint64_t sMask[4][4];
    const TileGeom g = tile_geom(C, W, H, tile_w, tile_h, offsets, n_isects);
    const int w = threadIdx.x >> 6, lane = threadIdx.x & 63;
    const int64_t p = ((int64_t)g.cam * H + g.i) * W + g.j;
    const int last = g.inside ? last_ids[p] : -1;
    float T = 1.0f, d = 0.f;
    for (int bs = g.start; bs < g.end; bs += BLK) {
        if (__syncthreads_and(last < bs)) break;
        const int idx = bs + threadIdx.x;
        int rel = 0;
        if (idx < g.end) rel = stage_record_depth(splats, flat[idx], threadIdx.x, g.tx0, g.ty0, sR);
        const uint64_t m0 = __ballot(rel & 1), m1 = __ballot(rel & 2), m2 = __ballot(rel & 4), m3 = __ballot(rel & 8);
        if (lane == 0) { sMask[0][w] = m0; sMask[1][w] = m1; sMask[2][w] = m2; sMask[3][w] = m3; }
        __syncthreads();
#pragma unroll 1
        for (int jj = 0; jj < 4; ++jj) {
            uint64_t m64 = uniform_u64(sMask[w][jj]);
            if (__builtin_amdgcn_ballot_w64(last >= bs + jj * 64) == 0) m64 = 0;
#pragma unroll 1
            for (int hh = 0; hh < 2; ++hh) {
                uint32_t m = hh ? (uint32_t)(m64 >> 32) : (uint32_t)m64;
                while (m) {
                    const int bit = __builtin_ctz(m);
                    m &= m - 1;
                    const int t = jj * 64 + hh * 32 + bit;
                    const float4 a = sR[2 * t];
                    const float4 q = sR[2 * t + 1];
                    const float dx = a.x - g.px, dy = a.y - g.py;
                    const float P = blend_power(dx, dy, a.w, q.x, q.y);
                    const float al0 = fminf(0.999f, a.z * __builtin_amdgcn_exp2f(P));
                    const bool ok = !(P > 0.f) && !(al0 < 1.f / 255.f) && (bs + t <= last);
                    const float al = ok ? al0 : 0.f;
                    const float vis = al * T;
                    T = T * (1.0f - al);
                    d = __builtin_fmaf(q.z, vis, d);
                }
            }
        }
    }
    if (g.inside) out_depth[p] = d;
}

int st3r_blend_depth_fwd_impl(st3r_ctx* ctx, hipStream_t s, const RasterOut& ro, const int32_t* last_ids, float* depth,
                              bool end_in_offsets) {
    (void)ctx;
    hipLaunchKernelGGL(k_blend_depth_fwd, dim3(ro.C * ro.tile_w * ro.tile_h), dim3(BLK), 0, s, ro.C, ro.W, ro.H, ro.tile_w,
                       ro.tile_h, (const float4*)ro.splats, ro.offsets, ro.flat, end_in_offsets ? -1 : (int)ro.n_isects,
                       last_ids, depth);
    LAUNCH_CHECK();
    return ST3R_OK;
}

ST3R_EXPORT int st3r_gs_blend_depth_fwd(st3r_ctx* ctx, void* stream, int C, int width, int height, int tile_size,
                                        int tile_w, int tile_h, const float* splats, const int32_t* offsets,
                                        const int32_t* flatten_ids, int64_t n_isects, const float* alpha,
                                        const int32_t* last_ids, float* depth) {
    if (int rc = check_blend_args(ctx, C, width, height, tile_size, tile_w, tile_h, splats, offsets, flatten_ids, n_isects))
        return rc;
    ARG_CHECK(alpha && last_ids && depth);
    (void)alpha;
    return st3r_blend_depth_fwd_impl(ctx, (hipStream_t)stream,
                                     stage_lists(C, width, height, tile_w, tile_h, splats, offsets, flatten_ids, n_isects),
                                     last_ids, depth, false);
}

__device__ __forceinline__ void depth_bwd_phase2(const float2* __restrict__ pr, unsigned tpack, int cnt, int lane,
                                                 const float4* sA, float* accw, float qxf_lane, float qyf_lane,
                                                 const float (&pvd)[CHUNK]) {
    static_assert(CHUNK == 4, "one DPP row per record of the chunk");
    const int r = lane >> 4, part = lane & 15;
    wave_lds_sync();
    const int t = (tpack >> (8 * r)) & 0xFF;
    const float2 mean = *reinterpret_cast<const float2*>(&sA[t]);
    const float dy = mean.y - qyf_lane;
    const float2* src = pr + r * PAIR_STRIDE + PAIR_AT(part * CHUNK);
    float W0 = 0.f, W1 = 0.f, W2 = 0.f, Sz = 0.f;
#pragma unroll
    for (int i = 0; i < CHUNK; ++i) {
        const float2 v = src[i];
        W0 += v.x;
        if (i == 1) { W1 = v.x; W2 = v.x; }
        if (i > 1) { W1 = fmaf((float)i, v.x, W1); W2 = fmaf((float)(i * i), v.x, W2); }
        Sz = fmaf(v.y, pvd[i], Sz);
    }
    const RunSums m = run_sums(W0, W1, W2, mean.x - qxf_lane, dy);
    float k0, k1, k2;
    reduce9_rows(m.Sx, m.Sy, m.So, m.Sxx, m.Sxy, m.Syy, Sz, 0.f, 0.f, k0, k1, k2);
    (void)k2;
    if (r < cnt && (lane & 3) == 0) {
        const int b = (lane >> 2) & 3;
        const int slot0 = ((b & 1) << 1) | (b >> 1);
        float* acc = accw + t * DACC_VALS;
        acc[slot0] = k0;
        if (slot0 < 3) acc[4 + slot0] = k1;
    }
    wave_lds_sync();
}

__global__ __launch_bounds__(BLK) __attribute__((amdgpu_waves_per_eu(8))) void k_blend_depth_bwd(
    int C, int W, int H, int tile_w, int tile_h, const float4* __restrict__ splats, const int32_t* __restrict__ offsets,
    const int32_t* __restrict__ flat, int n_isects, const float* __restrict__ out_alpha,
    const int32_t* __restrict__ last_ids, const float* __restrict__ v_depth, const uint64_t* __restrict__ cmask,
    int64_t cmask_words, const int32_t* __restrict__ tile_nb, const int32_t* __restrict__ cum,
    const uint64_t* __restrict__ rectbase, int tight, float* __restrict__ vtile, int stamp, unsigned vt_cap) {
    __shared__ float4 sA[HB];
    __shared__ float4 sB[HB];
    __shared__ float sAccW[4][HB * DACC_VALS];
    __shared__ float2 sPair[4][CHUNK * PAIR_STRIDE];
    __shared__ uint64_t sClampW;
    const TileGeom g = tile_geom(C, W, H, tile_w, tile_h, offsets, n_isects);
    const int nb = tile_nb[g.lb];
    if (nb == 0) return;
    const int w = threadIdx.x >> 6, lane = threadIdx.x & 63;
    const int64_t p = ((int64_t)g.cam * H + g.i) * W + g.j;
    float T_final = 1.0f, vd = 0.f;
    int bin_final = -1;
    if (g.inside) {
        T_final = 1.0f - out_alpha[p];
        vd = v_depth[p];
        bin_final = last_ids[p];
    }
    float2* pr = sPair[w];
    float* accw = sAccW[w];
    float pvd[CHUNK];
    const int pbase = (lane & 15) * CHUNK;
    {
        float* px = reinterpret_cast<float*>(pr);
        px[lane] = vd;
        wave_lds_sync();
#pragma unroll
        for (int i = 0; i < CHUNK; ++i) pvd[i] = px[pbase + i];
        wave_lds_sync();
    }
    const float qxf = (float)(g.tx0 + ((w & 1) << 3) + (pbase & 7)) + 0.5f;
    const float qyf_part = (float)(g.ty0 + ((w >> 1) << 3) + (pbase >> 3)) + 0.5f;
    float k_big = 0x1p64f, k_neg_thr = -__int_as_float(0x3b808080) * 0x1p64f;
    asm volatile("" : "+v"(k_big), "+v"(k_neg_thr));
    float T = T_final;
    float bv = 0.f;
    const int64_t mbase = mask_base(g.lb, g.start);
    const uint64_t* wmask = cmask + (int64_t)__builtin_amdgcn_readfirstlane(w) * cmask_words + mbase;
    uint64_t m_next = wmask[(BLK / HB) * nb - 1];
    for (int hb = (BLK / HB) * nb - 1; hb >= 0; --hb) {
        const int bs = g.start + hb * HB;
        const int bsz = min(HB, g.end - bs);
        const uint64_t m_cur = m_next;
        if (hb > 0) m_next = wmask[hb - 1];
        if (bsz <= 0) continue;
        int my_u = -1, my_cb = 0;
        float my_op = 0.f, my_ca = 0.f, my_cbb = 0.f, my_cc = 0.f;
        if ((int)threadIdx.x < bsz) {
            const int t = threadIdx.x;
            const int64_t my_id = flat[bs + t];
            const int64_t word = mbase + hb;
#pragma unroll
            for (int ww = 0; ww < 4; ++ww) my_cb |= (int)((cmask[ww * cmask_words + word] >> (t & 63)) & 1ull) << ww;
            float4 a = make_float4(0.f, 0.f, 0.f, 0.f), b = a, c = a;
            if (my_cb) {
                a = splats[my_id * 3 + 0];
                b = splats[my_id * 3 + 1];
                c = splats[my_id * 3 + 2];
                sA[t] = make_float4(a.x, a.y, a.z, -0.5f * LOG2E * a.w);
                sB[t] = make_float4(-LOG2E * b.x, -0.5f * LOG2E * b.y, c.y, 0.f);
            }
            const float det_ = a.w * b.y - b.x * b.x;
            const bool hard = my_cb && !(a.z <= 0.998f && a.w > 0.f && b.y > 0.f && det_ >= 2e-3f * (a.w * b.y));
            const uint64_t cw = __builtin_amdgcn_ballot_w64(hard);
            if (t == 0) sClampW = cw;
            if (my_cb) {
                if (rectbase) {
                    my_u = slot_of_rectbase(rectbase[my_id], g.tx0, g.ty0);
                } else {
                    TileRect tr = ref_tile_rect(a.x, a.y, (float)__float_as_int(c.z), 16, tile_w, tile_h);
                    if (tight) tr = tight_tile_rect(tr, a.x, a.y, a.z, a.w, b.x, b.y);
                    const int cum_excl = my_id == 0 ? 0 : cum[my_id - 1];
                    my_u = slot_of_rect(cum_excl, tr.x0, tr.y0, tr.x1 - tr.x0, g.tx0, g.ty0);
                }
                my_op = a.z; my_ca = a.w; my_cbb = b.x; my_cc = b.y;
            }
        }
        __syncthreads();
        auto walk = [&](auto clamp_tag) {
            constexpr bool CLAMP = decltype(clamp_tag)::value;
            uint64_t m = m_cur;
            while (m) {
                unsigned tpack = 0;
                int cnt = 0;
#pragma unroll
                for (int k = 0; k < CHUNK; ++k) {
                    if (m) {
                        const int t = 63 - __builtin_clzll(m);
                        m &= ~(1ull << t);
                        const float4 a = sA[t];
                        const float4 q = sB[t];
                        const float dx = a.x - g.px, dy = a.y - g.py;
                        const float P = blend_power(dx, dy, a.w, q.x, q.y);
                        const float vis0 = __builtin_amdgcn_exp2f(P);
                        const float ov0 = a.z * vis0;
                        float alpha;
                        if (CLAMP) {
                            const float al0 = fminf(0.999f, ov0);
                            uint64_t okm = mask_not_positive(P) & mask_not_less(al0, 1.f / 255.f);
                            okm &= __builtin_amdgcn_ballot_w64(bs + t <= bin_final);
                            alpha = zero_unless(okm, al0);
                        } else {
                            float step;
                            asm("v_fma_f32 %0, %1, %2, %3 clamp" : "=v"(step) : "v"(ov0), "v"(k_big), "v"(k_neg_thr));
                            alpha = ov0 * step;
                            alpha = zero_unless(__builtin_amdgcn_ballot_w64(bs + t <= bin_final), alpha);
                        }
                        float alpha_u = alpha;
                        if (CLAMP) alpha_u = ov0 <= 0.999f ? alpha : 0.f;
                        const float om = 1.0f - alpha;
                        float ra = __builtin_amdgcn_rcpf(om);
                        ra = __builtin_fmaf(__builtin_fmaf(-om, ra, 1.0f), ra, ra);
                        const float cv = q.z * vd;
                        T *= ra;
                        const float fac = alpha * T;
                        const float v_al = cv * T - bv * ra;
                        bv += cv * fac;
                        pr[k * PAIR_STRIDE + PAIR_AT(lane)] = make_float2(alpha_u * v_al, fac);
                        tpack |= (unsigned)t << (8 * k);
                        cnt = k + 1;
                    }
                }
                depth_bwd_phase2(pr, tpack, cnt, lane, sA, accw, qxf, qyf_part, pvd);
            }
        };
        const bool clamp_round = (uniform_u64(sClampW) & m_cur) != 0;
        if (clamp_round) walk(std::true_type{}); else walk(std::false_type{});
        __syncthreads();
        if (my_cb && (unsigned)my_u < vt_cap) {
            float acc[DACC_VALS];
#pragma unroll
            for (int k = 0; k < DACC_VALS; ++k) acc[k] = 0.f;
#pragma unroll
            for (int ww = 0; ww < 4; ++ww) {
                if (my_cb & (1 << ww)) {
#pragma unroll
                    for (int k = 0; k < DACC_VALS; ++k) acc[k] += sAccW[ww][threadIdx.x * DACC_VALS + k];
                }
            }
            const float sx = -acc[0], sy = -acc[1];
            float2* dst = reinterpret_cast<float2*>(vtile + (int64_t)my_u * DVT_STRIDE);
            dst[0] = make_float2(my_ca * sx + my_cbb * sy, my_cbb * sx + my_cc * sy);
            dst[1] = make_float2(my_op != 0.f ? acc[2] / my_op : 0.f, -0.5f * acc[3]);
            dst[2] = make_float2(-acc[4], -0.5f * acc[5]);
            dst[3] = make_float2(acc[6], __int_as_float(stamp));
        }
    }
}

int st3r_blend_depth_bwd_impl(st3r_ctx* ctx, hipStream_t s, const RasterOut& ro, const float* alpha,
                              const int32_t* last_ids, const float* v_depth, float* v_splats, bool end_in_offsets) {
    const int C = ro.C, tile_w = ro.tile_w, tile_h = ro.tile_h;
    const int32_t* cum = ro.cum;
    const int64_t n_isects = ro.n_isects, n_pairs = ro.n_pairs;
    if (n_isects == 0) {
        HIP_TRY(hipMemsetAsync(v_splats, 0, sizeof(float) * ST3R_SPLAT_STRIDE * (size_t)n_pairs, s));
        return ST3R_OK;
    }
    uint64_t* cmask; int64_t words; int32_t* tile_nb;
    int rc = hand_off_buffers(ctx, C * tile_w * tile_h, n_isects, false, &cmask, &words, &tile_nb);
    if (rc) return rc;
    StampedSlots sl;
    rc = stamped_slots(ctx, s, SLOT_VTILE_DEPTH, DVT_STRIDE, n_isects, &ctx->depth_stamp, &sl);
    if (rc) return rc;
    hipLaunchKernelGGL(k_blend_depth_bwd, dim3(C * tile_w * tile_h), dim3(BLK), 0, s, C, ro.W, ro.H, tile_w, tile_h,
                       (const float4*)ro.splats, ro.offsets, ro.flat, end_in_offsets ? -1 : (int)n_isects, alpha, last_ids,
                       v_depth, cmask, words, tile_nb, cum, ro.rectbase, ro.tight, sl.vtile, sl.stamp, sl.cap);
    LAUNCH_CHECK();
    hipLaunchKernelGGL(k_gather_vtile<DACC_VALS>, dim3(ceil_div(n_pairs, 256)), dim3(256), 0, s, n_pairs, cum, sl.vtile,
                       sl.stamp, sl.cap, (float4*)v_splats);
    LAUNCH_CHECK();
    return ST3R_OK;
}

ST3R_EXPORT int st3r_gs_blend_depth_bwd(st3r_ctx* ctx, void* stream, int C, int width, int height, int tile_size,
                                        int tile_w, int tile_h, const float* splats, const int32_t* offsets,
                                        const int32_t* flatten_ids, int64_t n_isects, const float* alpha,
                                        const int32_t* last_ids, const float* v_depth, const int32_t* cum_tiles,
                                        int64_t n_pairs, float* v_splats) {
    if (int rc = check_blend_args(ctx, C, width, height, tile_size, tile_w, tile_h, splats, offsets, flatten_ids, n_isects))
        return rc;
    ARG_CHECK(alpha && last_ids && v_depth && v_splats && cum_tiles && n_pairs >= 0);
    return st3r_blend_depth_bwd_impl(ctx, (hipStream_t)stream,
                                     stage_lists(C, width, height, tile_w, tile_h, splats, offsets, flatten_ids, n_isects,
                                                 cum_tiles, n_pairs),
                                     alpha, last_ids, v_depth, v_splats, false);
}

__global__ __launch_bounds__(256) void k_add_pairs(int64_t n4, float4* __restrict__ a, const float4* __restrict__ b) {
    for (int64_t i = (int64_t)blockIdx.x * blockDim.x + threadIdx.x; i < n4; i += (int64_t)gridDim.x * blockDim.x) {
        float4 x = a[i];
        const float4 y = b[i];
        x.x += y.x; x.y += y.y; x.z += y.z; x.w += y.w;
        a[i] = x;
    }
}

int st3r_add_pairs_impl(hipStream_t s, int64_t n_pairs, float* a, const float* b) {
    const int64_t n4 = n_pairs * (ST3R_SPLAT_STRIDE / 4);
    if (n4 <= 0) return ST3R_OK;
    int blocks = ceil_div(n4, 256);
    if (blocks > 256 * 8) blocks = 256 * 8;
    hipLaunchKernelGGL(k_add_pairs, dim3(blocks), dim3(256), 0, s, n4, (float4*)a, (const float4*)b);
    LAUNCH_CHECK();
    return ST3R_OK;
}

#define DPOSE_VALS 4

__global__ __launch_bounds__(256) void k_depth_bwd(int N, int C, const float* __restrict__ means,
                                                   const float* __restrict__ viewmats,
                                                   const float* __restrict__ splats, const float* __restrict__ v_splats,
                                                   float* __restrict__ grads, double* __restrict__ part) {
    __shared__ double red[4 * DPOSE_VALS];
    const int g = blockIdx.x * blockDim.x + threadIdx.x;
    float mx = 0.f, my = 0.f, mz = 0.f;
    if (g < N) { mx = means[3 * g]; my = means[3 * g + 1]; mz = means[3 * g + 2]; }
    float ax = 0.f, ay = 0.f, az = 0.f;
    for (int c = 0; c < C; ++c) {
        const int64_t pid = (int64_t)c * N + g;
        float vz = 0.f;
        if (g < N && __float_as_int(splats[pid * 12 + 10]) > 0) vz = v_splats[pid * 12 + 9];
        const float* V = viewmats + 16 * c;
        ax = fmaf(V[8], vz, ax); ay = fmaf(V[9], vz, ay); az = fmaf(V[10], vz, az);
        if (part) {
            double v[DPOSE_VALS] = {(double)vz * (double)mx, (double)vz * (double)my, (double)vz * (double)mz, (double)vz};
            __syncthreads();
            const double sum = block_sum_fixed(v, red);
            if (threadIdx.x < DPOSE_VALS) part[((int64_t)c * gridDim.x + blockIdx.x) * DPOSE_VALS + threadIdx.x] = sum;
        }
    }
    if (g < N) { grads[3 * g] += ax; grads[3 * g + 1] += ay; grads[3 * g + 2] += az; }
}

__global__ __launch_bounds__(256) void k_depth_bwd_finish(int n_part, const double* __restrict__ part,
                                                          float* __restrict__ v_viewmats) {
    __shared__ double red[4 * DPOSE_VALS];
    const int c = blockIdx.x;
    double v[DPOSE_VALS] = {0.0, 0.0, 0.0, 0.0};
    const double* pc = part + (int64_t)c * n_part * DPOSE_VALS;
    for (int b = threadIdx.x; b < n_part; b += blockDim.x) {
#pragma unroll
        for (int k = 0; k < DPOSE_VALS; ++k) v[k] += pc[(int64_t)b * DPOSE_VALS + k];
    }
    const double sum = block_sum_fixed(v, red);
    if (threadIdx.x < DPOSE_VALS) {
        const int k = threadIdx.x;
        float* dst = v_viewmats + 16 * c + 8 + k;
        *dst = (float)((double)*dst + sum);
    }
}

ST3R_EXPORT int st3r_gs_depth_bwd(st3r_ctx* ctx, void* stream, int N, int C, const float* means, const float* viewmats,
                                  const float* splats, const float* v_splats, float* grads, float* v_viewmats) {
    ARG_CHECK(ctx && N >= 0 && C > 0 && C <= ST3R_MAX_VIEWS);
    ARG_CHECK(means && viewmats && splats && v_splats && grads);
    hipStream_t s = (hipStream_t)stream;
    const int nb = ceil_div(N, 256);
    if (nb == 0) return ST3R_OK;
    double* part = nullptr;
    if (v_viewmats) {
        ARENA_GET(SLOT_DEPTH_PART, double, DPOSE_VALS * (size_t)nb * C, dpart);
        part = dpart;
    }
    hipLaunchKernelGGL(k_depth_bwd, dim3(nb), dim3(256), 0, s, N, C, means, viewmats, splats, v_splats, grads, part);
    LAUNCH_CHECK();
    if (v_viewmats) {
        hipLaunchKernelGGL(k_depth_bwd_finish, dim3(C), dim3(256), 0, s, nb, (const double*)part, v_viewmats);
        LAUNCH_CHECK();
    }
    return ST3R_OK;
}
```

starst3r_amd/csrc/gs_project.hip:

```cpp
#include "stages.h"
#include "tile_rect.h"
#include "project_common.h"

__device__ __forceinline__ float dot3f(float a0, float a1, float a2, float b0, float b1, float b2) {
    return (a0 * b0 + a1 * b1) + a2 * b2;
}

__global__ __launch_bounds__(256) void k_project_sh_fwd(
    int N, int C, const float* __restrict__ means, const float* __restrict__ quats,
    const float* __restrict__ scales, const float* __restrict__ opacities, const float* __restrict__ sh,
    int sh_stride, const float* __restrict__ viewmats, const float* __restrict__ Ks,
    const float* __restrict__ campos, int W, int H, int tile_size, int tile_w, int tile_h, float eps2d,
    float near_plane, float far_plane, float radius_clip, float4* __restrict__ splats,
    int32_t* __restrict__ tiles_per_gauss, double* __restrict__ reg_part,
    uint64_t* __restrict__ depth_keys, int32_t* __restrict__ depth_vals, int tight, uint32_t key_base,
    void* __restrict__ rects, int rect32, uint32_t* __restrict__ krange_part) {
    extern __shared__ float cam[];
    __shared__ float red[8];
    for (int c = threadIdx.x; c < C; c += blockDim.x) {
        float* o = cam + c * CAM_STRIDE;
        const float* V = viewmats + 16 * c;
        for (int k = 0; k < 12; ++k) o[k] = V[k];
        const float* K = Ks + 9 * c;
        float fx = K[0], fy = K[4], cx = K[2], cy = K[5];
        o[12] = fx; o[13] = fy; o[14] = cx; o[15] = cy;
        float tan_fovx = 0.5f * (float)W / fx;
        float tan_fovy = 0.5f * (float)H / fy;
        o[16] = ((float)W - cx) / fx + 0.3f * tan_fovx;
        o[17] = cx / fx + 0.3f * tan_fovx;
        o[18] = ((float)H - cy) / fy + 0.3f * tan_fovy;
        o[19] = cy / fy + 0.3f * tan_fovy;
        o[20] = campos[3 * c]; o[21] = campos[3 * c + 1]; o[22] = campos[3 * c + 2];
    }
    __syncthreads();

    const int g = blockIdx.x * blockDim.x + threadIdx.x;
    const bool active = g < N;
    float mx = 0, my = 0, mz = 0, opac = 0;
    float cov0 = 0, cov1 = 0, cov2 = 0, cov3 = 0, cov4 = 0, cov5 = 0;
    float k[12];
    float reg_o = 0.f, reg_s = 0.f;
    if (active) {
        mx = means[3 * g]; my = means[3 * g + 1]; mz = means[3 * g + 2];
        opac = opacities[g];
        float qw = quats[4 * g], qx = quats[4 * g + 1], qy = quats[4 * g + 2], qz = quats[4 * g + 3];
        float s0 = scales[3 * g], s1 = scales[3 * g + 1], s2 = scales[3 * g + 2];
        const float* kp = sh + (int64_t)g * sh_stride;
#pragma unroll
        for (int i = 0; i < 12; ++i) k[i] = kp[i];
        float n2 = ((qw * qw + qx * qx) + qy * qy) + qz * qz;
        float inv = 1.0f / sqrtf(n2);
        qw *= inv; qx *= inv; qy *= inv; qz *= inv;
        float x2 = qx * qx, y2 = qy * qy, z2 = qz * qz;
        float xy = qx * qy, xz = qx * qz, yz = qy * qz;
        float wx = qw * qx, wy = qw * qy, wz = qw * qz;
        float m0 = (1.0f - 2.0f * (y2 + z2)) * s0, m1 = (2.0f * (xy - wz)) * s1, m2 = (2.0f * (xz + wy)) * s2;
        float m3 = (2.0f * (xy + wz)) * s0, m4 = (1.0f - 2.0f * (x2 + z2)) * s1, m5 = (2.0f * (yz - wx)) * s2;
        float m6 = (2.0f * (xz - wy)) * s0, m7 = (2.0f * (yz + wx)) * s1, m8 = (1.0f - 2.0f * (x2 + y2)) * s2;
        cov0 = dot3f(m0, m1, m2, m0, m1, m2);
        cov1 = dot3f(m0, m1, m2, m3, m4, m5);
        cov2 = dot3f(m0, m1, m2, m6, m7, m8);
        cov3 = dot3f(m3, m4, m5, m3, m4, m5);
        cov4 = dot3f(m3, m4, m5, m6, m7, m8);
        cov5 = dot3f(m6, m7, m8, m6, m7, m8);
        if (reg_part) {
            reg_o = 1.0f / (1.0f + __expf(-opac));
            reg_s = (__expf(s0) + __expf(s1)) + __expf(s2);
        }
    }
    if (reg_part) {
        for (int off = 32; off > 0; off >>= 1) {
            reg_o += __shfl_down(reg_o, off);
            reg_s += __shfl_down(reg_s, off);
        }
        int w = threadIdx.x >> 6;
        if ((threadIdx.x & 63) == 0) { red[w] = reg_o; red[4 + w] = reg_s; }
        __syncthreads();
        if (threadIdx.x == 0) {
            reg_part[4 * blockIdx.x + 0] = (double)((red[0] + red[1]) + (red[2] + red[3]));
            reg_part[4 * blockIdx.x + 1] = (double)((red[4] + red[5]) + (red[6] + red[7]));
        }
    }
    int n_vis = 0, n_ref = 0;
    uint32_t kmin = 0xFFFFFFFFu, kmax = 0u;
    for (int c = 0; active && c < C; ++c) {
        const float* o = cam + c * CAM_STRIDE;
        const float R00 = o[0], R01 = o[1], R02 = o[2], t0 = o[3];
        const float R10 = o[4], R11 = o[5], R12 = o[6], t1 = o[7];
        const float R20 = o[8], R21 = o[9], R22 = o[10], t2 = o[11];
        const int64_t pid = (int64_t)c * N + g;
        float x = dot3f(R00, R01, R02, mx, my, mz) + t0;
        float y = dot3f(R10, R11, R12, mx, my, mz) + t1;
        float z = dot3f(R20, R21, R22, mx, my, mz) + t2;
        bool valid = !(z < near_plane || z > far_plane);
        float m2x = 0, m2y = 0, ca = 0, cb = 0, cc = 0, radius = 0;
        if (valid) {
            float T0 = dot3f(R00, R01, R02, cov0, cov1, cov2), T1 = dot3f(R00, R01, R02, cov1, cov3, cov4),
                  T2 = dot3f(R00, R01, R02, cov2, cov4, cov5);
            float T3 = dot3f(R10, R11, R12, cov0, cov1, cov2), T4 = dot3f(R10, R11, R12, cov1, cov3, cov4),
                  T5 = dot3f(R10, R11, R12, cov2, cov4, cov5);
            float T6 = dot3f(R20, R21, R22, cov0, cov1, cov2), T7 = dot3f(R20, R21, R22, cov1, cov3, cov4),
                  T8 = dot3f(R20, R21, R22, cov2, cov4, cov5);
            float c0 = dot3f(T0, T1, T2, R00, R01, R02);
            float c1 = dot3f(T0, T1, T2, R10, R11, R12);
            float c2 = dot3f(T0, T1, T2, R20, R21, R22);
            float c3 = dot3f(T3, T4, T5, R10, R11, R12);
            float c4 = dot3f(T3, T4, T5, R20, R21, R22);
            float c5 = dot3f(T6, T7, T8, R20, R21, R22);
            const float fx = o[12], fy = o[13], cx = o[14], cy = o[15];
            float rz = 1.0f / z;
            float rz2 = rz * rz;
            float xr = x * rz, yr = y * rz;
            float tx = z * fminf(o[16], fmaxf(-o[17], xr));
            float ty = z * fminf(o[18], fmaxf(-o[19], yr));
            float a = fx * rz, cj = -(fx * tx) * rz2;
            float b = fy * rz, d = -(fy * ty) * rz2;
            float t0x = a * c0 + cj * c2;
            float t0y = a * c1 + cj * c4;
            float t0z = a * c2 + cj * c5;
            float t1y = b * c3 + d * c4;
            float t1z = b * c4 + d * c5;
            float c00 = t0x * a + t0z * cj;
            float c01 = t0y * b + t0z * d;
            float c11 = t1y * b + t1z * d;
            m2x = (fx * x) * rz + cx;
            m2y = (fy * y) * rz + cy;
            c00 += eps2d; c11 += eps2d;
            float det = c00 * c11 - c01 * c01;
            if (det <= 0.0f) valid = false;
            else {
                float inv_det = 1.0f / det;
                ca = c11 * inv_det; cb = -c01 * inv_det; cc = c00 * inv_det;
                float bb = 0.5f * (c00 + c11);
                float v1 = bb + sqrtf(fmaxf(0.01f, bb * bb - det));
                radius = ceilf(3.0f * sqrtf(v1));
                if (radius <= radius_clip) valid = false;
                else if (m2x + radius <= 0.0f || m2x - radius >= (float)W || m2y + radius <= 0.0f ||
                         m2y - radius >= (float)H)
                    valid = false;
            }
        }
        float4 r0 = make_float4(0, 0, 0, 0), r1 = r0, r2 = r0;
        int ntiles = 0;
        TileRect tr = {0, 0, 0, 0};
        if (valid) {
            float dx = mx - o[20], dy = my - o[21], dz = mz - o[22];
            float inorm = 1.0f / sqrtf((dx * dx + dy * dy) + dz * dz);
            dx *= inorm; dy *= inorm; dz *= inorm;
            float col[3];
#pragma unroll
            for (int ch = 0; ch < 3; ++ch) {
                float r = SH_C0 * k[ch];
                r = r + SH_C1 * ((-dy * k[3 + ch] + dz * k[6 + ch]) - dx * k[9 + ch]);
                r = r + 0.5f;
                col[ch] = r < 0.0f ? 0.0f : r;
            }
            tr = ref_tile_rect(m2x, m2y, radius, tile_size, tile_w, tile_h);
            n_ref += (tr.y1 - tr.y0) * (tr.x1 - tr.x0);
            if (tight) tr = tight_tile_rect(tr, m2x, m2y, opac, ca, cb, cc);
            ntiles = (tr.y1 - tr.y0) * (tr.x1 - tr.x0);
            r0 = make_float4(m2x, m2y, opac, ca);
            r1 = make_float4(cb, cc, col[0], col[1]);
            r2 = make_float4(col[2], z, __int_as_float((int)radius), 0.0f);
        }
        splats[pid * 3 + 0] = r0;
        splats[pid * 3 + 1] = r1;
        splats[pid * 3 + 2] = r2;
        if (tiles_per_gauss) tiles_per_gauss[pid] = ntiles;
        if (rects) rect_store(rects, rect32, pid, tr);
        if (depth_keys) {
            const uint32_t dbits = valid ? (uint32_t)__float_as_int(z) : 0xFFFFFFFFu;
            if (key_base) {
                const uint32_t kk = valid ? dbits - key_base : 0x1FFFFFFFu;
                reinterpret_cast<uint32_t*>(depth_keys)[pid] = (krange_part ? 0u : ((uint32_t)c << 29)) | kk;
                if (valid) { kmin = min(kmin, kk); kmax = max(kmax, kk); }
            } else
                depth_keys[pid] = ((uint64_t)c << 32) | dbits;
            if (!krange_part) depth_vals[pid] = (int32_t)pid;
        }
        n_vis += valid ? 1 : 0;
    }
    if (krange_part) {
        for (int off = 32; off > 0; off >>= 1) { kmin = min(kmin, (uint32_t)__shfl_down((int)kmin, off)); kmax = max(kmax, (uint32_t)__shfl_down((int)kmax, off)); }
        __shared__ uint32_t redk[8];
        const int w = threadIdx.x >> 6;
        if ((threadIdx.x & 63) == 0) { redk[w] = kmin; redk[4 + w] = kmax; }
        __syncthreads();
        if (threadIdx.x == 0) {
            krange_part[2 * blockIdx.x + 0] = min(min(redk[0], redk[1]), min(redk[2], redk[3]));
            krange_part[2 * blockIdx.x + 1] = max(max(redk[4], redk[5]), max(redk[6], redk[7]));
        }
    }
    if (reg_part) {
        for (int off = 32; off > 0; off >>= 1) { n_vis += __shfl_down(n_vis, off); n_ref += __shfl_down(n_ref, off); }
        __shared__ int redi[8];
        const int w = threadIdx.x >> 6;
        if ((threadIdx.x & 63) == 0) { redi[w] = n_vis; redi[4 + w] = n_ref; }
        __syncthreads();
        if (threadIdx.x == 0) {
            reg_part[4 * blockIdx.x + 2] = (double)((redi[0] + redi[1]) + (redi[2] + redi[3]));
            reg_part[4 * blockIdx.x + 3] = (double)((redi[4] + redi[5]) + (redi[6] + redi[7]));
        }
    }
}

__global__ __launch_bounds__(256) void k_reg_reduce(int n_blocks, const double* __restrict__ reg_part,
                                                    double* __restrict__ reg_sums, int overwrite,
                                                    double* __restrict__ zero_ptr, int zero_n,
                                                    const uint32_t* __restrict__ krange_part,
                                                    uint32_t* __restrict__ krange) {
    for (int i = threadIdx.x; i < zero_n; i += 256) zero_ptr[i] = 0.0;
    if (krange_part) {
        __shared__ uint32_t shk[2][256];
        uint32_t lo = 0xFFFFFFFFu, hi = 0u;
        for (int b = threadIdx.x; b < n_blocks; b += 256) { lo = min(lo, krange_part[2 * b]); hi = max(hi, krange_part[2 * b + 1]); }
        shk[0][threadIdx.x] = lo; shk[1][threadIdx.x] = hi;
        __syncthreads();
        for (int off = 128; off > 0; off >>= 1) {
            if (threadIdx.x < off) {
                shk[0][threadIdx.x] = min(shk[0][threadIdx.x], shk[0][threadIdx.x + off]);
                shk[1][threadIdx.x] = max(shk[1][threadIdx.x], shk[1][threadIdx.x + off]);
            }
            __syncthreads();
        }
        if (threadIdx.x == 0) {
            lo = shk[0][0]; hi = shk[1][0];
            if (hi < lo) { lo = 0u; hi = 0u; }
            const uint32_t top = hi - lo + 1u;
            krange[0] = lo; krange[1] = top;
            krange[2] = top < (1u << 8) ? 1u : top < (1u << 16) ? 2u : top < (1u << 24) ? 3u : 4u;
        }
        __syncthreads();
    }
    __shared__ double sh[4][256];
    double acc[4] = {0, 0, 0, 0};
    for (int b = threadIdx.x; b < n_blocks; b += 256)
        for (int k = 0; k < 4; ++k) acc[k] += reg_part[4 * b + k];
    for (int k = 0; k < 4; ++k) sh[k][threadIdx.x] = acc[k];
    __syncthreads();
    for (int off = 128; off > 0; off >>= 1) {
        if (threadIdx.x < off)
            for (int k = 0; k < 4; ++k) sh[k][threadIdx.x] += sh[k][threadIdx.x + off];
        __syncthreads();
    }
    if (threadIdx.x < 4) reg_sums[threadIdx.x] = (overwrite ? 0.0 : reg_sums[threadIdx.x]) + sh[threadIdx.x][0];
}

int st3r_project_impl(st3r_ctx* ctx, hipStream_t s, const GsParams& g, const GsViews& v, int tile_size, float eps2d,
                      float near_plane, float far_plane, float radius_clip, float* splats, int32_t* tiles_per_gauss,
                      double* reg_sums, uint64_t* depth_keys, int32_t* depth_vals, int tight, uint32_t key_base, void* rects,
                      int rect32, int reg_overwrite, double* zero_ptr, int zero_n, uint32_t* krange) {
    const int N = g.N, C = v.C, width = v.W, height = v.H;
    if (N == 0) {
        if (reg_sums && reg_overwrite) HIP_TRY(hipMemsetAsync(reg_sums, 0, sizeof(double) * 4, s));
        if (zero_ptr && zero_n > 0) HIP_TRY(hipMemsetAsync(zero_ptr, 0, sizeof(double) * (size_t)zero_n, s));
        return ST3R_OK;
    }
    int tile_w = (width + tile_size - 1) / tile_size, tile_h = (height + tile_size - 1) / tile_size;
    dim3 grid(ceil_div(N, 256)), block(256);
    size_t shmem = (size_t)C * CAM_STRIDE * sizeof(float);
    double* reg_part = nullptr;
    if (reg_sums) {
        ARENA_GET(SLOT_REG_PART, double, 4 * (size_t)grid.x, p);
        reg_part = p;
    }
    uint32_t* krange_part = nullptr;
    if (krange && reg_sums) {
        ARENA_GET(SLOT_KRANGE_PART, uint32_t, 2 * (size_t)grid.x, p);
        krange_part = p;
    }
    hipLaunchKernelGGL(k_project_sh_fwd, grid, block, shmem, s, N, C, g.means, g.quats, g.scales, g.opacities, g.sh,
                       g.sh_stride, v.viewmats, v.Ks, v.campos, width, height, tile_size, tile_w, tile_h, eps2d, near_plane, far_plane,
                       radius_clip, (float4*)splats, tiles_per_gauss, reg_part, depth_keys, depth_vals, tight, key_base,
                       rects, rect32, krange_part);
    if (reg_sums)
        hipLaunchKernelGGL(k_reg_reduce, dim3(1), dim3(256), 0, s, (int)grid.x, reg_part, reg_sums, reg_overwrite, zero_ptr,
                           zero_ptr ? zero_n : 0, (const uint32_t*)krange_part, krange);
    else if (zero_ptr && zero_n > 0)
        HIP_TRY(hipMemsetAsync(zero_ptr, 0, sizeof(double) * (size_t)zero_n, s));
    LAUNCH_CHECK();
    return ST3R_OK;
}

ST3R_EXPORT int st3r_gs_project_sh(st3r_ctx* ctx, void* stream, int N, int C, const float* means,
                                   const float* quats, const float* scales, const float* opacities,
                                   const float* sh, int sh_stride, const float* viewmats, const float* Ks,
                                   const float* campos, int width, int height, int tile_size, float eps2d,
                                   float near_plane, float far_plane, float radius_clip, float* splats,
                                   int32_t* tiles_per_gauss, double* reg_sums) {
    ARG_CHECK(ctx && N >= 0 && C > 0 && C <= ST3R_MAX_VIEWS && sh_stride >= 12 && width > 0 && height > 0 && tile_size > 0);
    ARG_CHECK(means && quats && scales && opacities && sh && viewmats && Ks && campos && splats && tiles_per_gauss);
    return st3r_project_impl(ctx, (hipStream_t)stream, GsParams{N, means, quats, scales, opacities, sh, sh_stride},
                             GsViews{C, width, height, viewmats, Ks, campos}, tile_size, eps2d, near_plane, far_plane, radius_clip, splats,
                             tiles_per_gauss, reg_sums, nullptr, nullptr, 0, 0u, nullptr, 0, 0, nullptr, 0, nullptr);
}
```

starst3r_amd/csrc/gs_project_bwd.hip:

```cpp
#include "stages.h"
#include "blend_common.h"
#include "project_common.h"

#ifndef GATHER_WIDE_ABOVE
#define GATHER_WIDE_ABOVE 6
#endif

template <bool GATHER>
__global__ __launch_bounds__(256) __attribute__((amdgpu_waves_per_eu(4))) void k_project_sh_bwd(
    int N, int C, const float* __restrict__ means, const float* __restrict__ quats,
    const float* __restrict__ scales, const float* __restrict__ opacities, const float* __restrict__ sh,
    int sh_stride, const float* __restrict__ viewmats, const float* __restrict__ Ks,
    const float* __restrict__ campos, int W, int H, float eps2d, const float4* __restrict__ splats,
    const float4* __restrict__ v_splats, float reg_o_k, float reg_s_k, float* __restrict__ grads, int accumulate,
    int g_begin, int g_end, int range_major, const int32_t* __restrict__ cum, const float* __restrict__ vtile, int stamp,
    unsigned vt_cap, const uint32_t* __restrict__ touch) {
    extern __shared__ float cam[];
    constexpr int ROW = ACC_VALS;
    __shared__ float sVal[GATHER ? 256 * ROW : 1];
    __shared__ float sAcc[GATHER ? 256 * ROW : 1];
    __shared__ int sStart[GATHER ? 4 * 65 : 1];
    for (int c = threadIdx.x; c < C; c += blockDim.x) {
        float* o = cam + c * CAM_STRIDE;
        const float* V = viewmats + 16 * c;
        for (int k = 0; k < 12; ++k) o[k] = V[k];
        const float* K = Ks + 9 * c;
        float fx = K[0], fy = K[4], cx = K[2], cy = K[5];
        o[12] = fx; o[13] = fy; o[14] = cx; o[15] = cy;
        float tan_fovx = 0.5f * (float)W / fx;
        float tan_fovy = 0.5f * (float)H / fy;
        o[16] = ((float)W - cx) / fx + 0.3f * tan_fovx;
        o[17] = cx / fx + 0.3f * tan_fovx;
        o[18] = ((float)H - cy) / fy + 0.3f * tan_fovy;
        o[19] = cy / fy + 0.3f * tan_fovy;
        o[20] = campos[3 * c]; o[21] = campos[3 * c + 1]; o[22] = campos[3 * c + 2];
    }
    __syncthreads();
    const int gbase = g_begin + blockIdx.x * blockDim.x;
    const bool valid = gbase + (int)threadIdx.x < g_end;
    if (!GATHER && !valid) return;
    const int g = valid ? gbase + (int)threadIdx.x : g_end - 1;

    const float mx = means[3 * g], my = means[3 * g + 1], mz = means[3 * g + 2];
    const float opac = opacities[g];
    float qw = quats[4 * g], qx = quats[4 * g + 1], qy = quats[4 * g + 2], qz = quats[4 * g + 3];
    const float s0 = scales[3 * g], s1 = scales[3 * g + 1], s2 = scales[3 * g + 2];
    float k[12];
    const float* kp = sh + (int64_t)g * sh_stride;
#pragma unroll
    for (int i = 0; i < 12; ++i) k[i] = kp[i];
    const float inv_norm = 1.0f / sqrtf(((qw * qw + qx * qx) + qy * qy) + qz * qz);
    qw *= inv_norm; qx *= inv_norm; qy *= inv_norm; qz *= inv_norm;
    const float sc[3] = {s0, s1, s2};
    auto rot_and_m = [&](float (&Rq)[9], float (&M)[9]) {
        float x2 = qx * qx, y2 = qy * qy, z2 = qz * qz, xy = qx * qy, xz = qx * qz, yz = qy * qz;
        float wx = qw * qx, wy = qw * qy, wz = qw * qz;
        Rq[0] = 1.0f - 2.0f * (y2 + z2); Rq[1] = 2.0f * (xy - wz); Rq[2] = 2.0f * (xz + wy);
        Rq[3] = 2.0f * (xy + wz); Rq[4] = 1.0f - 2.0f * (x2 + z2); Rq[5] = 2.0f * (yz - wx);
        Rq[6] = 2.0f * (xz - wy); Rq[7] = 2.0f * (yz + wx); Rq[8] = 1.0f - 2.0f * (x2 + y2);
#pragma unroll
        for (int i = 0; i < 3; ++i)
#pragma unroll
            for (int j = 0; j < 3; ++j) M[i * 3 + j] = Rq[i * 3 + j] * sc[j];
    };
    float cov[6];
    {
        float Rq[9], M[9];
        rot_and_m(Rq, M);
        cov[0] = M[0] * M[0] + M[1] * M[1] + M[2] * M[2];
        cov[1] = M[0] * M[3] + M[1] * M[4] + M[2] * M[5];
        cov[2] = M[0] * M[6] + M[1] * M[7] + M[2] * M[8];
        cov[3] = M[3] * M[3] + M[4] * M[4] + M[5] * M[5];
        cov[4] = M[3] * M[6] + M[4] * M[7] + M[5] * M[8];
        cov[5] = M[6] * M[6] + M[7] * M[7] + M[8] * M[8];
        asm volatile("" : "+v"(cov[0]), "+v"(cov[1]), "+v"(cov[2]), "+v"(cov[3]), "+v"(cov[4]), "+v"(cov[5]));
    }

    float v_mean[3] = {0, 0, 0};
    float vSw[6] = {0, 0, 0, 0, 0, 0};
    float v_k[12];
#pragma unroll
    for (int i = 0; i < 12; ++i) v_k[i] = 0.f;
    float v_opac = 0.f;

    for (int c = 0; c < C; ++c) {
        const int64_t pid = (int64_t)c * N + g;
        float4 g0, g1, g2;
        if (GATHER) {
            const int lane = threadIdx.x & 63, wv = threadIdx.x >> 6;
            float* wval = sVal + wv * (64 * ROW);
            const int my_end = cum[pid];
            const int my_start = !valid ? my_end : (pid == 0 ? 0 : cum[pid - 1]);
            const int s0 = __builtin_amdgcn_readfirstlane(my_start);
            const int s1 = __builtin_amdgcn_readlane(my_end, 63);
            float acc[ACC_VALS];
            float2 q0, q1, q2, q3, q4;
            auto fetch = [&](int u) {
                q0 = q1 = q2 = q3 = q4 = make_float2(0.f, 0.f);
                if (u < s1 && (unsigned)u < vt_cap) {
                    const float2* src = reinterpret_cast<const float2*>(vtile + (int64_t)u * VT_STRIDE);
                    q0 = src[0]; q1 = src[1]; q2 = src[2]; q3 = src[3]; q4 = src[4];
                }
            };
            auto rows_to_lds = [&]() {
                const bool live = __float_as_int(q4.y) == stamp;
                float* row = wval + lane * ROW;
                row[0] = live ? q0.x : 0.f; row[1] = live ? q0.y : 0.f; row[2] = live ? q1.x : 0.f;
                row[3] = live ? q1.y : 0.f; row[4] = live ? q2.x : 0.f; row[5] = live ? q2.y : 0.f;
                row[6] = live ? q3.x : 0.f; row[7] = live ? q3.y : 0.f; row[8] = live ? q4.x : 0.f;
            };
            if (s1 - s0 <= 64 * GATHER_WIDE_ABOVE) {
                if (s1 > s0) fetch(s0 + lane);
#pragma unroll
                for (int k2 = 0; k2 < ACC_VALS; ++k2) acc[k2] = 0.f;
                for (int base = s0; base < s1; base += 64) {
                    rows_to_lds();
                    wave_lds_sync();
                    fetch(base + 64 + lane);
                    const int lo = max(my_start, base) - base, hi = min(my_end, base + 64) - base;
                    for (int r = lo; r < hi; ++r) {
                        const float* src = wval + r * ROW;
#pragma unroll
                        for (int k2 = 0; k2 < ACC_VALS; ++k2) acc[k2] += src[k2];
                    }
                    wave_lds_sync();
                }
            } else {
                float* wacc = sAcc + wv * (64 * ROW);
                int* wst = sStart + wv * 65;
                wst[lane] = my_start;
                if (lane == 63) wst[64] = my_end;
#pragma unroll
                for (int k2 = 0; k2 < ACC_VALS; ++k2) wacc[lane * ROW + k2] = 0.f;
                const uint64_t tmask = touch ? __builtin_amdgcn_ballot_w64(valid && touch[pid] == (uint32_t)stamp) : ~0ull;
                auto meets = [&](int b) {
                    return __builtin_amdgcn_ballot_w64(my_end > my_start && my_start < b + 64 && my_end > b);
                };
                uint64_t pm_next = meets(s0);
                bool have = false;
                if (pm_next & tmask) { fetch(s0 + lane); have = true; }
                for (int base = s0; base < s1; base += 64) {
                    const uint64_t pm = pm_next & tmask;
                    const bool cur = have;
                    if (cur) { rows_to_lds(); wave_lds_sync(); }
                    pm_next = base + 64 < s1 ? meets(base + 64) : 0ull;
                    have = (pm_next & tmask) != 0;
                    if (have) fetch(base + 64 + lane);
                    if (cur) {
                        const int pa = __builtin_ctzll(pm), pb = 63 - __builtin_clzll(pm);
                        const int items = (pb - pa + 1) * ROW;
                        for (int it = lane; it < items; it += 64) {
                            const int q = (it * 7282) >> 16;
                            const int k2 = it - q * ROW, pp = pa + q;
                            const int lo = max(wst[pp], base) - base, hi = min(wst[pp + 1], base + 64) - base;
                            if (hi > lo) {
                                float sum = wacc[pp * ROW + k2];
                                const float* src = wval + k2;
                                int r = lo;
                                for (; r + 4 <= hi; r += 4) {
                                    const float a0 = src[r * ROW], a1 = src[(r + 1) * ROW], a2 = src[(r + 2) * ROW], a3 = src[(r + 3) * ROW];
                                    sum += a0; sum += a1; sum += a2; sum += a3;
                                }
                                for (; r < hi; ++r) sum += src[r * ROW];
                                wacc[pp * ROW + k2] = sum;
                            }
                        }
                        wave_lds_sync();
                    }
                }
                wave_lds_sync();
#pragma unroll
                for (int k2 = 0; k2 < ACC_VALS; ++k2) acc[k2] = wacc[lane * ROW + k2];
                wave_lds_sync();
            }
            g0 = make_float4(acc[0], acc[1], acc[2], acc[3]);
            g1 = make_float4(acc[4], acc[5], acc[6], acc[7]);
            g2 = make_float4(acc[8], 0.f, 0.f, 0.f);
            if (!valid) continue;
        }
        const float4 r2 = splats[pid * 3 + 2];
        if (__float_as_int(r2.z) <= 0) continue;
        const float4 r0 = splats[pid * 3 + 0];
        const float4 r1 = splats[pid * 3 + 1];
        if (!GATHER) {
            g0 = v_splats[pid * 3 + 0];
            g1 = v_splats[pid * 3 + 1];
            g2 = v_splats[pid * 3 + 2];
        }
        const float* o = cam + c * CAM_STRIDE;
        const float R[9] = {o[0], o[1], o[2], o[4], o[5], o[6], o[8], o[9], o[10]};
        v_opac += g0.z;
        {
            float dx = mx - o[20], dy = my - o[21], dz = mz - o[22];
            float nrm = sqrtf(dx * dx + dy * dy + dz * dz);
            float inrm = 1.0f / nrm;
            float ux = dx * inrm, uy = dy * inrm, uz = dz * inrm;
            const float vcol[3] = {g1.z, g1.w, g2.x};
            const float colf[3] = {r1.z, r1.w, r2.x};
            float vdx = 0.f, vdy = 0.f, vdz = 0.f;
#pragma unroll
            for (int ch = 0; ch < 3; ++ch) {
                float pre = SH_C0 * k[ch] + SH_C1 * ((-uy * k[3 + ch] + uz * k[6 + ch]) - ux * k[9 + ch]) + 0.5f;
                float vc = (colf[ch] > 0.0f || pre >= 0.0f) ? vcol[ch] : 0.0f;
                v_k[ch] += SH_C0 * vc;
                v_k[3 + ch] += -SH_C1 * uy * vc;
                v_k[6 + ch] += SH_C1 * uz * vc;
                v_k[9 + ch] += -SH_C1 * ux * vc;
                vdx += -SH_C1 * k[9 + ch] * vc;
                vdy += -SH_C1 * k[3 + ch] * vc;
                vdz += SH_C1 * k[6 + ch] * vc;
            }
            float dotp = vdx * ux + vdy * uy + vdz * uz;
            v_mean[0] += (vdx - dotp * ux) * inrm;
            v_mean[1] += (vdy - dotp * uy) * inrm;
            v_mean[2] += (vdz - dotp * uz) * inrm;
        }
        const float x = R[0] * mx + R[1] * my + R[2] * mz + o[3];
        const float y = R[3] * mx + R[4] * my + R[5] * mz + o[7];
        const float z = R[6] * mx + R[7] * my + R[8] * mz + o[11];
        float T[9];
#pragma unroll
        for (int i = 0; i < 3; ++i) {
            T[i * 3 + 0] = R[i * 3] * cov[0] + R[i * 3 + 1] * cov[1] + R[i * 3 + 2] * cov[2];
            T[i * 3 + 1] = R[i * 3] * cov[1] + R[i * 3 + 1] * cov[3] + R[i * 3 + 2] * cov[4];
            T[i * 3 + 2] = R[i * 3] * cov[2] + R[i * 3 + 1] * cov[4] + R[i * 3 + 2] * cov[5];
        }
        const float S00 = T[0] * R[0] + T[1] * R[1] + T[2] * R[2];
        const float S01 = T[0] * R[3] + T[1] * R[4] + T[2] * R[5];
        const float S02 = T[0] * R[6] + T[1] * R[7] + T[2] * R[8];
        const float S11 = T[3] * R[3] + T[4] * R[4] + T[5] * R[5];
        const float S12 = T[3] * R[6] + T[4] * R[7] + T[5] * R[8];
        const float S22 = T[6] * R[6] + T[7] * R[7] + T[8] * R[8];
        const float fx = o[12], fy = o[13];
        const float rz = 1.0f / z, rz2 = rz * rz, rz3 = rz2 * rz;
        const float xr = x * rz, yr = y * rz;
        const bool x_in = (xr <= o[16]) && (xr >= -o[17]);
        const bool y_in = (yr <= o[18]) && (yr >= -o[19]);
        const float tx = z * fminf(o[16], fmaxf(-o[17], xr));
        const float ty = z * fminf(o[18], fmaxf(-o[19], yr));
        const float a = fx * rz, cj = -fx * tx * rz2, b = fy * rz, d = -fy * ty * rz2;
        const Sym3 S = {S00, S01, S02, S11, S12, S22};
        Sym3 vS;
        float vJ00, vJ02, vJ11, vJ12;
        conic_chain(r0, r1, g0, g1, a, cj, b, d, S, vS, vJ00, vJ02, vJ11, vJ12);
        const float vm2x = g0.x, vm2y = g0.y;
        float vpx = fx * rz * vm2x;
        float vpy = fy * rz * vm2y;
        float vpz = -(fx * x * vm2x + fy * y * vm2y) * rz2;
        vpz += -fx * rz2 * vJ00 - fy * rz2 * vJ11;
        if (x_in) { vpx += -fx * rz2 * vJ02; vpz += 2.0f * fx * x * rz3 * vJ02; }
        else { vpz += fx * tx * rz3 * vJ02; }
        if (y_in) { vpy += -fy * rz2 * vJ12; vpz += 2.0f * fy * y * rz3 * vJ12; }
        else { vpz += fy * ty * rz3 * vJ12; }
        v_mean[0] += R[0] * vpx + R[3] * vpy + R[6] * vpz;
        v_mean[1] += R[1] * vpx + R[4] * vpy + R[7] * vpz;
        v_mean[2] += R[2] * vpx + R[5] * vpy + R[8] * vpz;
        float U[9];
        const float vSm[9] = {vS.xx, vS.xy, vS.xz, vS.xy, vS.yy, vS.yz, vS.xz, vS.yz, vS.zz};
#pragma unroll
        for (int i = 0; i < 3; ++i)
#pragma unroll
            for (int j = 0; j < 3; ++j)
                U[i * 3 + j] = vSm[i * 3] * R[j] + vSm[i * 3 + 1] * R[3 + j] + vSm[i * 3 + 2] * R[6 + j];
        vSw[0] += R[0] * U[0] + R[3] * U[3] + R[6] * U[6];
        vSw[1] += R[0] * U[1] + R[3] * U[4] + R[6] * U[7];
        vSw[2] += R[0] * U[2] + R[3] * U[5] + R[6] * U[8];
        vSw[3] += R[1] * U[1] + R[4] * U[4] + R[7] * U[7];
        vSw[4] += R[1] * U[2] + R[4] * U[5] + R[7] * U[8];
        vSw[5] += R[2] * U[2] + R[5] * U[5] + R[8] * U[8];
    }

    if (GATHER && !valid) return;
    float Rq[9], M[9];
    asm volatile("" : "+v"(qw), "+v"(qx), "+v"(qy), "+v"(qz));
    rot_and_m(Rq, M);
    const float W9[9] = {vSw[0], vSw[1], vSw[2], vSw[1], vSw[3], vSw[4], vSw[2], vSw[4], vSw[5]};
    float vM[9];
#pragma unroll
    for (int r = 0; r < 3; ++r)
#pragma unroll
        for (int s = 0; s < 3; ++s)
            vM[r * 3 + s] = 2.0f * (W9[r * 3] * M[s] + W9[r * 3 + 1] * M[3 + s] + W9[r * 3 + 2] * M[6 + s]);
    float v_scale[3], vR[9];
#pragma unroll
    for (int s = 0; s < 3; ++s) {
        v_scale[s] = Rq[s] * vM[s] + Rq[3 + s] * vM[3 + s] + Rq[6 + s] * vM[6 + s];
        vR[s] = vM[s] * sc[s]; vR[3 + s] = vM[3 + s] * sc[s]; vR[6 + s] = vM[6 + s] * sc[s];
    }
    float vq0 = 2.0f * (qx * (vR[7] - vR[5]) + qy * (vR[2] - vR[6]) + qz * (vR[3] - vR[1]));
    float vq1 = 2.0f * (-2.0f * qx * (vR[4] + vR[8]) + qy * (vR[3] + vR[1]) + qz * (vR[6] + vR[2]) + qw * (vR[7] - vR[5]));
    float vq2 = 2.0f * (qx * (vR[3] + vR[1]) - 2.0f * qy * (vR[0] + vR[8]) + qz * (vR[7] + vR[5]) + qw * (vR[2] - vR[6]));
    float vq3 = 2.0f * (qx * (vR[6] + vR[2]) + qy * (vR[7] + vR[5]) - 2.0f * qz * (vR[0] + vR[4]) + qw * (vR[3] - vR[1]));
    const float dq = vq0 * qw + vq1 * qx + vq2 * qy + vq3 * qz;
    vq0 = (vq0 - dq * qw) * inv_norm; vq1 = (vq1 - dq * qx) * inv_norm;
    vq2 = (vq2 - dq * qy) * inv_norm; vq3 = (vq3 - dq * qz) * inv_norm;

    const float sg = 1.0f / (1.0f + __expf(-opac));
    v_opac += reg_o_k * sg * (1.0f - sg);
    v_scale[0] += reg_s_k * __expf(s0);
    v_scale[1] += reg_s_k * __expf(s1);
    v_scale[2] += reg_s_k * __expf(s2);

    const int64_t Nl = range_major ? g_end - g_begin : N;
    float* gb = range_major ? grads + (int64_t)23 * g_begin : grads;
    const int gw = range_major ? g - g_begin : g;
    float* gm = gb; float* gq = gb + 3 * Nl; float* gs = gb + 7 * Nl;
    float* go = gb + 10 * Nl; float* gsh = gb + 11 * Nl;
    if (accumulate) {
        v_mean[0] += gm[3 * gw]; v_mean[1] += gm[3 * gw + 1]; v_mean[2] += gm[3 * gw + 2];
        vq0 += gq[4 * gw]; vq1 += gq[4 * gw + 1]; vq2 += gq[4 * gw + 2]; vq3 += gq[4 * gw + 3];
        v_scale[0] += gs[3 * gw]; v_scale[1] += gs[3 * gw + 1]; v_scale[2] += gs[3 * gw + 2];
        v_opac += go[gw];
#pragma unroll
        for (int i = 0; i < 12; ++i) v_k[i] += gsh[(int64_t)gw * 12 + i];
    }
    gm[3 * gw] = v_mean[0]; gm[3 * gw + 1] = v_mean[1]; gm[3 * gw + 2] = v_mean[2];
    gq[4 * gw] = vq0; gq[4 * gw + 1] = vq1; gq[4 * gw + 2] = vq2; gq[4 * gw + 3] = vq3;
    gs[3 * gw] = v_scale[0]; gs[3 * gw + 1] = v_scale[1]; gs[3 * gw + 2] = v_scale[2];
    go[gw] = v_opac;
#pragma unroll
    for (int i = 0; i < 12; ++i) gsh[(int64_t)gw * 12 + i] = v_k[i];
}

int st3r_project_sh_bwd_impl(hipStream_t s, const GsParams& g, const GsViews& v, float eps2d, const float* splats,
                             const float* v_splats, float reg_views, float opac_fac, float scale_fac, float* grads,
                             bool accumulate, int g_begin, int g_end, bool range_major, const st3r_vtile_ref* slots) {
    const int N = g.N, C = v.C;
    if (g_end < 0) g_end = N;
    if (N == 0 || g_end <= g_begin) return ST3R_OK;
    float reg_o_k = reg_views * opac_fac / (float)N;
    float reg_s_k = reg_views * scale_fac / (3.0f * (float)N);
    size_t shmem = (size_t)C * CAM_STRIDE * sizeof(float);
    if (slots)
        hipLaunchKernelGGL(k_project_sh_bwd<true>, dim3(ceil_div(g_end - g_begin, 256)), dim3(256), shmem, s, N, C, g.means,
                           g.quats, g.scales, g.opacities, g.sh, g.sh_stride, v.viewmats, v.Ks, v.campos, v.W, v.H, eps2d,
                           (const float4*)splats, (const float4*)nullptr, reg_o_k, reg_s_k, grads, accumulate ? 1 : 0, g_begin,
                           g_end, range_major ? 1 : 0, slots->cum, slots->vtile, slots->stamp, slots->vt_cap, slots->touch);
    else
        hipLaunchKernelGGL(k_project_sh_bwd<false>, dim3(ceil_div(g_end - g_begin, 256)), dim3(256), shmem, s, N, C, g.means,
                           g.quats, g.scales, g.opacities, g.sh, g.sh_stride, v.viewmats, v.Ks, v.campos, v.W, v.H, eps2d,
                           (const float4*)splats, (const float4*)v_splats, reg_o_k, reg_s_k, grads, accumulate ? 1 : 0, g_begin,
                           g_end, range_major ? 1 : 0, (const int32_t*)nullptr, (const float*)nullptr, 0, 0u, (const uint32_t*)nullptr);
    LAUNCH_CHECK();
    return ST3R_OK;
}

ST3R_EXPORT int st3r_gs_project_sh_bwd(st3r_ctx* ctx, void* stream, int N, int C, const float* means,
                                       const float* quats, const float* scales, const float* opacities,
                                       const float* sh, int sh_stride, const float* viewmats, const float* Ks,
                                       const float* campos, int width, int height, float eps2d,
                                       const float* splats, const float* v_splats, float reg_views,
                                       float opac_fac, float scale_fac, float* grads) {
    ARG_CHECK(ctx && N >= 0 && C > 0 && C <= ST3R_MAX_VIEWS && sh_stride >= 12);
    ARG_CHECK(means && quats && scales && opacities && sh && viewmats && Ks && campos && splats && v_splats && grads);
    return st3r_project_sh_bwd_impl((hipStream_t)stream, GsParams{N, means, quats, scales, opacities, sh, sh_stride},
                                    GsViews{C, width, height, viewmats, Ks, campos}, eps2d, splats, v_splats, reg_views, opac_fac, scale_fac,
                                    grads, false, 0, -1, false, nullptr);
}
```

starst3r_amd/csrc/stages.h:

```cpp
#pragma once
#include "common.h"

struct GsParams {
    int N;
    const float *means, *quats, *scales, *opacities, *sh;
    int sh_stride;
};

struct GsViews {
    int C, W, H;
    const float *viewmats, *Ks, *campos;
    GsViews slice(int c0, int c1) const { return {c1 - c0, W, H, viewmats + 16 * c0, Ks + 9 * c0, campos + 3 * c0}; }
};

struct RasterOut {
    int C, W, H, tile_w, tile_h;
    const float* splats; const int32_t *offsets, *flat, *cum; const uint64_t *rects, *rectbase;
    int tight;
    int64_t n_pairs;
    int64_t n_isects, n_records, n_isects_ref, n_visible;
};

static inline RasterOut stage_lists(int C, int W, int H, int tile_w, int tile_h, const float* splats, const int32_t* offsets,
                                    const int32_t* flat, int64_t n_isects, const int32_t* cum = nullptr,
                                    int64_t n_pairs = 0) {
    return RasterOut{C, W, H, tile_w, tile_h, splats, offsets, flat, cum, nullptr, nullptr, 0, n_pairs, n_isects, n_isects,
                     n_isects, -1};
}

struct DepthPrior { const float* prior; const float* weight; const double* norm; float fac; };

struct ExposureReg { const float* exposure; float* v_exposure; };

struct LossWeight { const float* weight = nullptr; const double* norm = nullptr; int norm_stride = 0; int sums_stride = 2; };

int st3r_counts_buffer(st3r_ctx* ctx, hipStream_t s, int32_t** out);
int st3r_count_settle(st3r_ctx* ctx);
int st3r_train_fwd_bwd_impl(st3r_ctx* ctx, hipStream_t s, const GsParams& g, const GsViews& v, const float* gt_images,
                            float ssim_fac, float opac_fac, float scale_fac, float* grads, float* loss_out,
                            int64_t* stats_host, float* v_viewmats);
int st3r_peer_status_settle(st3r_ctx* ctx);

int st3r_project_impl(st3r_ctx* ctx, hipStream_t s, const GsParams& g, const GsViews& v, int tile_size, float eps2d,
                      float near_plane, float far_plane, float radius_clip, float* splats, int32_t* tiles_per_gauss,
                      double* reg_sums, uint64_t* depth_keys, int32_t* depth_vals, int tight, uint32_t key_base, void* rects,
                      int rect32, int reg_overwrite, double* zero_ptr, int zero_n, uint32_t* krange);
int st3r_project_sh_bwd_impl(hipStream_t s, const GsParams& g, const GsViews& v, float eps2d, const float* splats,
                             const float* v_splats, float reg_views, float opac_fac, float scale_fac, float* grads,
                             bool accumulate, int g_begin, int g_end, bool range_major, const st3r_vtile_ref* slots);

int st3r_isect_scan_impl(st3r_ctx* ctx, hipStream_t s, int64_t n_pairs, const int32_t* tiles, int32_t* cum,
                         int64_t* n_isects_host, const void* pack_rects, int rect32, uint64_t* pack_out,
                         int32_t** total_dev_out, int32_t* total_copy, int32_t* total_host);
int st3r_scan_tiles(int64_t n);
void st3r_emit_grid(int N, int C, int* bpc, int* grid, int* self_base);
void st3r_isect_constants(int64_t out[5]);
int st3r_isect_emit_chain_impl(st3r_ctx* ctx, hipStream_t s, int N, int C, const int32_t* perm, const void* rects,
                               int rect32, int tile_w, int tile_h, uint32_t* tile_keys, int32_t* vals, int64_t cap,
                               int band_tile, const int32_t* n_dev, const uint32_t** band_table);
int st3r_records_prepare_impl(hipStream_t s, int N, int C, const float* splats, int tile_size, int tile_w, int tile_h,
                              int tight, int32_t* tiles, uint64_t* depth_keys, int32_t* depth_vals, uint32_t key_base,
                              void* rects, int rect32);
int st3r_isect_offsets32_impl(hipStream_t s, int64_t n_isects, const uint32_t* keys, int C, int tile_w, int tile_h,
                              int32_t* offsets, const int32_t* n_dev);
int st3r_sort_tile_end_bit(int end_bit);
int st3r_sort_tile_impl(st3r_ctx* ctx, hipStream_t s, int64_t n, int end_bit, uint32_t* keys_in, int32_t* vals_in,
                        uint32_t* keys_out, int32_t* vals_out, const int32_t* n_dev);
int st3r_sort_tile_banded(int end_bit, int debug_flags);

int st3r_blend_fwd_impl(st3r_ctx* ctx, hipStream_t s, const RasterOut& ro, float* rgb, float* alpha, int32_t* last_ids,
                        bool for_backward, bool end_in_offsets);
int st3r_blend_fwd_cells_impl(st3r_ctx* ctx, hipStream_t s, const RasterOut& ro, float* rgb, float* alpha,
                              int32_t* last_ids, uint64_t* cmask, int64_t cmask_words, int32_t* tile_nb);
int st3r_blend_bwd_impl(st3r_ctx* ctx, hipStream_t s, const RasterOut& ro, const float* alpha, const int32_t* last_ids,
                        const float* v_rgb, const float* v_alpha, float* v_splats, bool end_in_offsets,
                        st3r_vtile_ref* defer);
int st3r_gather_vtile_impl(hipStream_t s, int64_t n_pairs, const st3r_vtile_ref* slots, float* v_splats);
int st3r_blend_depth_fwd_impl(st3r_ctx* ctx, hipStream_t s, const RasterOut& ro, const int32_t* last_ids, float* depth,
                              bool end_in_offsets);
int st3r_blend_depth_bwd_impl(st3r_ctx* ctx, hipStream_t s, const RasterOut& ro, const float* alpha,
                              const int32_t* last_ids, const float* v_depth, float* v_splats, bool end_in_offsets);
int st3r_add_pairs_impl(hipStream_t s, int64_t n_pairs, float* a, const float* b);

int st3r_loss_impl(st3r_ctx* ctx, hipStream_t s, int C, int H, int W, const float* render, const float* gt,
                   float w_l1, float w_ssim, double* sums, float* v_render, bool sums_cleared, const LossWeight& lw);
int st3r_loss_weight_for(st3r_ctx* ctx, hipStream_t s, const float* gt, int C, int H, int W, LossWeight* out);
int st3r_weight_norms(st3r_ctx* ctx, hipStream_t s, int C, int H, int W, const float* weight, double* out, int stride,
                      int at_least_one, bool interior, int slot);
int st3r_registered_weight_norms(st3r_ctx* ctx, hipStream_t s, const ViewReg& reg, const float* weight, int at_least_one,
                                 bool interior, int part_slot, int norm_slot, int* valid, const double** norms);
int st3r_depth_prior_for(st3r_ctx* ctx, hipStream_t s, const float* gt, int C, int H, int W, DepthPrior* out);
int st3r_depth_prior_loss_impl(st3r_ctx* ctx, hipStream_t s, int C, int H, int W, const float* depth, const float* alpha,
                               const float* prior, const float* weight, const double* norm, int norm_stride,
                               float depth_fac, double* sums, int sums_stride, float* v_depth, float* v_alpha);

void st3r_exposure_for(st3r_ctx* ctx, const float* gt, int C, int H, int W, ExposureReg* out);
int st3r_exposure_fwd_impl(hipStream_t s, int C, int H, int W, const float* rgb, const float* exposure, float* out);
int st3r_exposure_bwd_impl(st3r_ctx* ctx, hipStream_t s, int C, int H, int W, const float* rgb, const float* exposure,
                           const float* v_out, float* v_rgb, float* v_exposure);

float* st3r_intrinsics_grad_for(st3r_ctx* ctx, const float* gt, int C, int H, int W);

int st3r_adam_impl(hipStream_t s, int N, float* means, float* quats, float* scales, float* opacities, float* sh,
                   int sh_stride, const float* grads, float* m, float* v, double lr, double b1, double b2,
                   double eps, int step, const int32_t* count_dev, uint32_t count_cap, const int32_t* status_dev, int64_t i0,
                   int64_t i1, int64_t g0, int64_t g1, float* pstage, const float* gstage, float* grads_out);
int st3r_params_from_stage_impl(hipStream_t s, int N, float* means, float* quats, float* scales, float* opacities,
                                float* sh, int sh_stride, const float* pstage, int64_t i0, int64_t i1, int64_t lim,
                                const int32_t* count_dev, uint32_t count_cap, const int32_t* status_dev);
int st3r_params_from_peers_impl(hipStream_t s, int N, float* means, float* quats, float* scales, float* opacities,
                                float* sh, int sh_stride, const float* const* tab, int r, int64_t q, int64_t lim,
                                const int32_t* status_dev);
void st3r_adam_guard(st3r_ctx* ctx, const int32_t** count_dev, uint32_t* count_cap);
```

Measured before the change: 200.6.

## Replace per-pair intersection scan with per-wave slot bases computed in projection

The projection kernel now writes per-64-Gaussian wave tile totals and per-Gaussian intra-wave offsets into the rectbase words. The scan stage then scans only C*groups wave totals instead of all C*N pairs. Blend backward, depth backward, gather and project backward rebuild each pair's slot range from the wave base plus the local offset. This shrinks the scan pass and the cum array traffic, at the cost of extra indirection in the consumers and an on-demand expansion kernel when the debug peek asks for cum.

```diff
diff --git a/starst3r_amd/csrc/api.hip b/starst3r_amd/csrc/api.hip
--- a/starst3r_amd/csrc/api.hip
+++ b/starst3r_amd/csrc/api.hip
@@ -94,6 +94,11 @@
                                   SLOT_MCMC_CUM, SLOT_MCMC_DEAD, SLOT_MCMC_SAMPLED, SLOT_MCMC_COUNT,
                                   SLOT_RGB, SLOT_ALPHA, SLOT_COUNTS, SLOT_KEYS_A, SLOT_VALS_A, SLOT_KEYS_B};
     ARG_CHECK((size_t)bytes <= ctx->slot_bytes[slots[which]]);
+    if (which == 3 && bytes > 0 && ctx->rel.tab && ctx->rel.tab == ctx->slot_ptr[SLOT_WAVE_BASE] &&
+        ctx->rel.words == ctx->slot_ptr[SLOT_RECTBASE] && ctx->slot_bytes[SLOT_CUM] >= sizeof(int32_t) * (size_t)ctx->rel_pairs) {
+        int rc = st3r_slot_scan_expand_impl((hipStream_t)stream, ctx->rel_pairs, ctx->rel, (int32_t*)ctx->slot_ptr[SLOT_CUM]);
+        if (rc) return rc;
+    }
     HIP_TRY(hipMemcpyAsync(dst, ctx->slot_ptr[slots[which]], (size_t)bytes, hipMemcpyDeviceToDevice,
                            (hipStream_t)stream));
     return ST3R_OK;
@@ -183,6 +188,7 @@
         if (ctx->slot_ptr[i]) (void)hipFree(ctx->slot_ptr[i]);
         ctx->slot_ptr[i] = nullptr; ctx->slot_bytes[i] = 0;
     }
+    ctx->rel = st3r_slot_bases{};
     return rc;
 }
 
diff --git a/starst3r_amd/csrc/blend_common.h b/starst3r_amd/csrc/blend_common.h
--- a/starst3r_amd/csrc/blend_common.h
+++ b/starst3r_amd/csrc/blend_common.h
@@ -150,6 +150,16 @@
     return cum_excl + ((ty0 >> 4) - y0) * rw + ((tx0 >> 4) - x0);
 }
 
+__device__ __forceinline__ int wave_slot_base(const int32_t* __restrict__ tab, int groups, int c, int g) {
+    return tab[c * groups + (g >> 6)];
+}
+__device__ __forceinline__ int slot_base(const st3r_slot_bases& sb, int c, int g) {
+    return wave_slot_base(sb.tab, sb.groups, c, g) + reinterpret_cast<const int32_t*>(sb.words)[2 * ((int64_t)c * sb.N + g) + 1];
+}
+__device__ __forceinline__ int slot_end(const st3r_slot_bases& sb, int c, int g) {
+    return g + 1 < sb.N ? slot_base(sb, c, g + 1) : sb.tab[(c + 1) * sb.groups];
+}
+
 struct RunSums { float So, Sx, Sxx, Sy, Sxy, Syy; };
 __device__ __forceinline__ RunSums run_sums(float W0, float W1, float W2, float d0, float dy) {
     const float So = W0, Sx = fmaf(d0, W0, -W1), Sxx = fmaf(d0, Sx - W1, W2);
@@ -176,7 +186,7 @@
 template <int NV>
 __global__ __launch_bounds__(256) void k_gather_vtile(int64_t n_pairs, const int32_t* __restrict__ cum,
                                                       const float* __restrict__ vtile, int stamp, unsigned vt_cap,
-                                                      float4* __restrict__ v_splats) {
+                                                      float4* __restrict__ v_splats, st3r_slot_bases rel) {
     static_assert(NV & 1, "the stamp closes the slot's last 8-byte word");
     constexpr int ROW = NV;
     constexpr int NQ = (NV + 1) / 2;
@@ -185,8 +195,15 @@
     const int tid = threadIdx.x;
     const int64_t p0 = (int64_t)blockIdx.x * 256;
     const int np = (int)min((int64_t)256, n_pairs - p0);
-    if (tid == 0) sCum[0] = p0 == 0 ? 0 : cum[p0 - 1];
-    sCum[tid + 1] = cum[p0 + min(tid, np - 1)];
+    if (rel.tab) {
+        const int64_t pe = p0 + min(tid, np - 1);
+        const int c = (int)(pe / rel.N);
+        sCum[tid + 1] = slot_end(rel, c, (int)(pe - (int64_t)c * rel.N));
+        if (tid == 0) sCum[0] = slot_base(rel, c, (int)(pe - (int64_t)c * rel.N));
+    } else {
+        if (tid == 0) sCum[0] = p0 == 0 ? 0 : cum[p0 - 1];
+        sCum[tid + 1] = cum[p0 + min(tid, np - 1)];
+    }
     __syncthreads();
     const int s0 = sCum[0], s1 = sCum[np];
     const int my_start = sCum[tid], my_end = tid < np ? sCum[tid + 1] : sCum[tid];
diff --git a/starst3r_amd/csrc/common.h b/starst3r_amd/csrc/common.h
--- a/starst3r_amd/csrc/common.h
+++ b/starst3r_amd/csrc/common.h
@@ -90,6 +90,8 @@
     SLOT_KGRAD_PART,
     SLOT_LWEIGHT_PART,
     SLOT_LWEIGHT_NORM,
+    SLOT_WAVE_TILES,
+    SLOT_WAVE_BASE,
     SLOT_COUNT
 };
 
@@ -112,7 +114,8 @@
 
 #define ST3R_SPLIT_VIEWS 1000
 
-struct st3r_vtile_ref { const int32_t* cum; const float* vtile; int stamp; unsigned vt_cap; const uint32_t* touch; };
+struct st3r_slot_bases { const uint64_t* words; const int32_t* tab; int N, groups; };
+struct st3r_vtile_ref { const int32_t* cum; const float* vtile; int stamp; unsigned vt_cap; const uint32_t* touch; st3r_slot_bases rel; };
 
 struct ViewReg { const float* gt; int c, h, w; };
 
@@ -146,6 +149,7 @@
     int depth_stamp;
     uint32_t scan_gen;
     uint32_t scan_gen_b;
+    st3r_slot_bases rel; int64_t rel_pairs;
     int64_t isect_hint, count_cap;
     int64_t hint_sig;
     int count_pending;
diff --git a/starst3r_amd/csrc/fused_step.hip b/starst3r_amd/csrc/fused_step.hip
--- a/starst3r_amd/csrc/fused_step.hip
+++ b/starst3r_amd/csrc/fused_step.hip
@@ -78,13 +78,32 @@
     int32_t* counts = nullptr;
     { int rc_ = st3r_counts_buffer(ctx, s, &counts); if (rc_) return rc_; }
     uint32_t* const krange = fp.segments ? (uint32_t*)(counts + 8) : nullptr;
+    uint64_t* rectbase = nullptr;
+    if (fp.rectbase) {
+        ARENA_GET(SLOT_RECTBASE, uint64_t, n_pairs, rb);
+        rectbase = rb;
+    }
+    st3r_slot_bases rel{};
+    int32_t* wave_tiles = nullptr;
+    if (!records_in && rectbase && !(ctx->debug_flags & (4096 | 2))) {
+        const int groups = (N + 63) / 64;
+        ARENA_GET(SLOT_WAVE_TILES, int32_t, (int64_t)C * groups, wt);
+        void* wb; int grown = 0;
+        int rc_ = st3r_arena_get2(ctx, SLOT_WAVE_BASE, sizeof(int32_t) * ((size_t)C * groups + 1), &wb, &grown);
+        if (rc_) return rc_;
+        if (grown) HIP_TRY(hipMemsetAsync(wb, 0, sizeof(int32_t), s));
+        wave_tiles = wt;
+        rel = st3r_slot_bases{rectbase, (const int32_t*)wb, N, groups};
+    }
+    ctx->rel = rel; ctx->rel_pairs = n_pairs;
     st3r_prof_begin(ctx, s, STG_PROJECT);
     const uint32_t key_base = fp.key_base;
     int rc = records_in
                  ? st3r_records_prepare_impl(s, N, C, splats, tile, tile_w, tile_h, tight, nullptr, dkeys_a, dvals_a,
                                              key_base, rects, rect32)
                  : st3r_project_impl(ctx, s, g, v, tile, 0.3f, near_plane, far_plane, 0.0f, splats, nullptr, reg_sums,
-                                     dkeys_a, dvals_a, tight, key_base, rects, rect32, 1, loss_sums, 2 * C, krange);
+                                     dkeys_a, dvals_a, tight, key_base, rects, rect32, 1, loss_sums, 2 * C, krange,
+                                     rel.tab ? rectbase : nullptr, wave_tiles);
     if (!rc && records_in && loss_sums) HIP_TRY(hipMemsetAsync(loss_sums, 0, sizeof(double) * 2 * (size_t)C, s));
     st3r_prof_end(ctx, s, STG_PROJECT);
     if (rc) return rc;
@@ -96,16 +115,15 @@
     if (rc) return rc;
     int64_t n_isects = 0;
     st3r_prof_begin(ctx, s, STG_SCAN);
-    uint64_t* rectbase = nullptr;
-    if (fp.rectbase) {
-        ARENA_GET(SLOT_RECTBASE, uint64_t, n_pairs, rb);
-        rectbase = rb;
-    }
     const int64_t sig = ((int64_t)N << 34) ^ ((int64_t)C << 26) ^ ((int64_t)W << 13) ^ (int64_t)H;
     const bool async = allow_async && ctx->isect_hint > 0 && ctx->hint_sig == sig;
     int32_t* total_dev = nullptr;
-    rc = st3r_isect_scan_impl(ctx, s, n_pairs, nullptr, cum, nullptr, rects, rect32, rectbase, &total_dev,
-                              async ? counts : nullptr, async ? (int32_t*)(ctx->pinned + 8) : nullptr);
+    int32_t* const total_copy = async ? counts : nullptr;
+    int32_t* const total_host = async ? (int32_t*)(ctx->pinned + 8) : nullptr;
+    rc = rel.tab ? st3r_isect_scan_impl(ctx, s, (int64_t)C * rel.groups, wave_tiles, const_cast<int32_t*>(rel.tab) + 1, nullptr,
+                                        nullptr, 0, nullptr, &total_dev, total_copy, total_host)
+                 : st3r_isect_scan_impl(ctx, s, n_pairs, nullptr, cum, nullptr, rects, rect32, rectbase, &total_dev,
+                                        total_copy, total_host);
     st3r_prof_end(ctx, s, STG_SCAN);
     if (rc) return rc;
     if (async) {
@@ -163,7 +181,7 @@
     if (rc) return rc;
     o->C = C; o->W = W; o->H = H; o->tile_w = tile_w; o->tile_h = tile_h;
     o->splats = splats; o->offsets = offsets; o->flat = vals_b; o->cum = cum; o->rects = rect32 ? nullptr : rects;
-    o->rectbase = rectbase;
+    o->rectbase = rectbase; o->rel = rel;
     o->tight = tight; o->n_pairs = n_pairs;
     o->n_isects = n_isects;
     return ST3R_OK;
diff --git a/starst3r_amd/csrc/gs_blend.hip b/starst3r_amd/csrc/gs_blend.hip
--- a/starst3r_amd/csrc/gs_blend.hip
+++ b/starst3r_amd/csrc/gs_blend.hip
@@ -179,7 +179,7 @@
     wave_lds_sync();
 }
 
-template <bool HAS_VA, bool TOUCH = false>
+template <bool HAS_VA, bool TOUCH = false, bool REL = false>
 __global__ __launch_bounds__(BLK) __attribute__((amdgpu_waves_per_eu(8))) void k_blend_bwd(int C, int W, int H, int tile_w, int tile_h,
                                                    const float4* __restrict__ splats,
                                                    const int32_t* __restrict__ offsets,
@@ -193,7 +193,8 @@
                                                    const int32_t* __restrict__ cum,
                                                    const uint64_t* __restrict__ rects,
                                                    const uint64_t* __restrict__ rectbase, int tight,
-                                                   float* __restrict__ vtile, int stamp, unsigned vt_cap) {
+                                                   float* __restrict__ vtile, int stamp, unsigned vt_cap,
+                                                   const int32_t* __restrict__ wave_base, int N, int groups) {
 
     __shared__ float4 sA[HB];
     __shared__ float4 sB[HB];
@@ -264,11 +265,12 @@
             const bool hard = my_cb && !(a.z <= 0.998f && a.w > 0.f && b.y > 0.f && det_ >= 2e-3f * (a.w * b.y));
             const uint64_t cw = __builtin_amdgcn_ballot_w64(hard);
             if (t == 0) sClampW = cw;
-            if (my_cb && rectbase) {
+            if (my_cb && (REL || rectbase)) {
                 if (TOUCH) reinterpret_cast<uint32_t*>(const_cast<uint64_t*>(rects))[my_id] = (uint32_t)stamp;
                 my_u = slot_of_rectbase(rectbase[my_id], g.tx0, g.ty0);
+                if (REL) my_u += wave_slot_base(wave_base, groups, g.cam, (int)my_id - g.cam * N);
                 my_op = a.z; my_ca = a.w; my_cbb = b.x; my_cc = b.y;
-            } else if (my_cb) {
+            } else if (my_cb && !REL) {
                 int x0, y0, rw;
                 if (rects) {
                     const uint64_t r = rects[my_id];
@@ -366,7 +368,8 @@
     const int C = ro.C, W = ro.W, H = ro.H, tile_w = ro.tile_w, tile_h = ro.tile_h, tight = ro.tight;
     const int32_t* cum = ro.cum; const uint64_t* rects = ro.rects; const uint64_t* rectbase = ro.rectbase;
     const int64_t n_isects = ro.n_isects, n_pairs = ro.n_pairs;
-    if (defer) *defer = st3r_vtile_ref{cum, nullptr, 0, 0u, nullptr};
+    const st3r_slot_bases rel = rectbase ? ro.rel : st3r_slot_bases{};
+    if (defer) *defer = st3r_vtile_ref{cum, nullptr, 0, 0u, nullptr, rel};
     if (n_isects == 0) {
         if (!defer) HIP_TRY(hipMemsetAsync(v_splats, 0, sizeof(float) * ST3R_SPLAT_STRIDE * (size_t)n_pairs, s));
         return ST3R_OK;
@@ -392,14 +395,17 @@
     } else if (grown_t) {
         HIP_TRY(hipMemsetAsync(touch, 0, ctx->slot_bytes[SLOT_PAIR_TOUCH], s));
     }
-    const auto kernel = v_alpha ? k_blend_bwd<true> : touch ? k_blend_bwd<false, true> : k_blend_bwd<false>;
+    const auto kernel = rel.tab ? (v_alpha ? k_blend_bwd<true, false, true>
+                                           : touch ? k_blend_bwd<false, true, true> : k_blend_bwd<false, false, true>)
+                                : (v_alpha ? k_blend_bwd<true> : touch ? k_blend_bwd<false, true> : k_blend_bwd<false>);
     hipLaunchKernelGGL(kernel, dim3(total), dim3(BLK), 0, s, C, W, H, tile_w, tile_h, (const float4*)ro.splats, ro.offsets,
                        ro.flat, end_in_offsets ? -1 : (int)n_isects, alpha, last_ids, v_rgb, v_alpha, cmask, words, tile_nb, cum,
-                       touch ? reinterpret_cast<const uint64_t*>(touch) : rects, rectbase, tight, sl.vtile, sl.stamp, sl.cap);
+                       touch ? reinterpret_cast<const uint64_t*>(touch) : rects, rectbase, tight, sl.vtile, sl.stamp, sl.cap,
+                       rel.tab, rel.N, rel.groups);
     LAUNCH_CHECK();
-    if (defer) { *defer = st3r_vtile_ref{cum, sl.vtile, sl.stamp, sl.cap, touch}; return ST3R_OK; }
+    if (defer) { *defer = st3r_vtile_ref{cum, sl.vtile, sl.stamp, sl.cap, touch, rel}; return ST3R_OK; }
     hipLaunchKernelGGL(k_gather_vtile<ACC_VALS>, dim3(ceil_div(n_pairs, 256)), dim3(256), 0, s, n_pairs, cum, sl.vtile,
-                       sl.stamp, sl.cap, (float4*)v_splats);
+                       sl.stamp, sl.cap, (float4*)v_splats, rel);
     LAUNCH_CHECK();
     return ST3R_OK;
 }
@@ -407,7 +413,21 @@
 int st3r_gather_vtile_impl(hipStream_t s, int64_t n_pairs, const st3r_vtile_ref* slots, float* v_splats) {
     if (n_pairs <= 0) return ST3R_OK;
     hipLaunchKernelGGL(k_gather_vtile<ACC_VALS>, dim3(ceil_div(n_pairs, 256)), dim3(256), 0, s, n_pairs, slots->cum,
-                       slots->vtile, slots->stamp, slots->vt_cap, (float4*)v_splats);
+                       slots->vtile, slots->stamp, slots->vt_cap, (float4*)v_splats, slots->rel);
+    LAUNCH_CHECK();
+    return ST3R_OK;
+}
+
+__global__ __launch_bounds__(256) void k_slot_scan_expand(int64_t n_pairs, st3r_slot_bases rel, int32_t* __restrict__ cum) {
+    const int64_t p = (int64_t)blockIdx.x * 256 + threadIdx.x;
+    if (p >= n_pairs) return;
+    const int c = (int)(p / rel.N);
+    cum[p] = slot_end(rel, c, (int)(p - (int64_t)c * rel.N));
+}
+
+int st3r_slot_scan_expand_impl(hipStream_t s, int64_t n_pairs, const st3r_slot_bases& rel, int32_t* cum) {
+    if (n_pairs <= 0) return ST3R_OK;
+    hipLaunchKernelGGL(k_slot_scan_expand, dim3(ceil_div(n_pairs, 256)), dim3(256), 0, s, n_pairs, rel, cum);
     LAUNCH_CHECK();
     return ST3R_OK;
 }
diff --git a/starst3r_amd/csrc/gs_blend_depth.hip b/starst3r_amd/csrc/gs_blend_depth.hip
--- a/starst3r_amd/csrc/gs_blend_depth.hip
+++ b/starst3r_amd/csrc/gs_blend_depth.hip
@@ -125,7 +125,8 @@
     const int32_t* __restrict__ flat, int n_isects, const float* __restrict__ out_alpha,
     const int32_t* __restrict__ last_ids, const float* __restrict__ v_depth, const uint64_t* __restrict__ cmask,
     int64_t cmask_words, const int32_t* __restrict__ tile_nb, const int32_t* __restrict__ cum,
-    const uint64_t* __restrict__ rectbase, int tight, float* __restrict__ vtile, int stamp, unsigned vt_cap) {
+    const uint64_t* __restrict__ rectbase, int tight, float* __restrict__ vtile, int stamp, unsigned vt_cap,
+    const int32_t* __restrict__ wave_base, int N, int groups) {
     __shared__ float4 sA[HB];
     __shared__ float4 sB[HB];
     __shared__ float sAccW[4][HB * DACC_VALS];
@@ -193,6 +194,7 @@
             if (my_cb) {
                 if (rectbase) {
                     my_u = slot_of_rectbase(rectbase[my_id], g.tx0, g.ty0);
+                    if (wave_base) my_u += wave_slot_base(wave_base, groups, g.cam, (int)my_id - g.cam * N);
                 } else {
                     TileRect tr = ref_tile_rect(a.x, a.y, (float)__float_as_int(c.z), 16, tile_w, tile_h);
                     if (tight) tr = tight_tile_rect(tr, a.x, a.y, a.z, a.w, b.x, b.y);
@@ -278,6 +280,7 @@
                               const int32_t* last_ids, const float* v_depth, float* v_splats, bool end_in_offsets) {
     const int C = ro.C, tile_w = ro.tile_w, tile_h = ro.tile_h;
     const int32_t* cum = ro.cum;
+    const st3r_slot_bases rel = ro.rectbase ? ro.rel : st3r_slot_bases{};
     const int64_t n_isects = ro.n_isects, n_pairs = ro.n_pairs;
     if (n_isects == 0) {
         HIP_TRY(hipMemsetAsync(v_splats, 0, sizeof(float) * ST3R_SPLAT_STRIDE * (size_t)n_pairs, s));
@@ -291,10 +294,11 @@
     if (rc) return rc;
     hipLaunchKernelGGL(k_blend_depth_bwd, dim3(C * tile_w * tile_h), dim3(BLK), 0, s, C, ro.W, ro.H, tile_w, tile_h,
                        (const float4*)ro.splats, ro.offsets, ro.flat, end_in_offsets ? -1 : (int)n_isects, alpha, last_ids,
-                       v_depth, cmask, words, tile_nb, cum, ro.rectbase, ro.tight, sl.vtile, sl.stamp, sl.cap);
+                       v_depth, cmask, words, tile_nb, cum, ro.rectbase, ro.tight, sl.vtile, sl.stamp, sl.cap, rel.tab, rel.N,
+                       rel.groups);
     LAUNCH_CHECK();
     hipLaunchKernelGGL(k_gather_vtile<DACC_VALS>, dim3(ceil_div(n_pairs, 256)), dim3(256), 0, s, n_pairs, cum, sl.vtile,
-                       sl.stamp, sl.cap, (float4*)v_splats);
+                       sl.stamp, sl.cap, (float4*)v_splats, rel);
     LAUNCH_CHECK();
     return ST3R_OK;
 }
diff --git a/starst3r_amd/csrc/gs_project.hip b/starst3r_amd/csrc/gs_project.hip
--- a/starst3r_amd/csrc/gs_project.hip
+++ b/starst3r_amd/csrc/gs_project.hip
@@ -1,6 +1,7 @@
 #include "stages.h"
 #include "tile_rect.h"
 #include "project_common.h"
+#include "wave_prims.h"
 
 __device__ __forceinline__ float dot3f(float a0, float a1, float a2, float b0, float b1, float b2) {
     return (a0 * b0 + a1 * b1) + a2 * b2;
@@ -14,7 +15,8 @@
     float near_plane, float far_plane, float radius_clip, float4* __restrict__ splats,
     int32_t* __restrict__ tiles_per_gauss, double* __restrict__ reg_part,
     uint64_t* __restrict__ depth_keys, int32_t* __restrict__ depth_vals, int tight, uint32_t key_base,
-    void* __restrict__ rects, int rect32, uint32_t* __restrict__ krange_part) {
+    void* __restrict__ rects, int rect32, uint32_t* __restrict__ krange_part, uint64_t* __restrict__ slot_words,
+    int32_t* __restrict__ wave_tiles) {
     extern __shared__ float cam[];
     __shared__ float red[8];
     for (int c = threadIdx.x; c < C; c += blockDim.x) {
@@ -83,102 +85,115 @@
     }
     int n_vis = 0, n_ref = 0;
     uint32_t kmin = 0xFFFFFFFFu, kmax = 0u;
-    for (int c = 0; active && c < C; ++c) {
-        const float* o = cam + c * CAM_STRIDE;
-        const float R00 = o[0], R01 = o[1], R02 = o[2], t0 = o[3];
-        const float R10 = o[4], R11 = o[5], R12 = o[6], t1 = o[7];
-        const float R20 = o[8], R21 = o[9], R22 = o[10], t2 = o[11];
+    const bool hand_out = slot_words != nullptr;
+    const int groups = (N + 63) >> 6;
+    for (int c = 0; (active || hand_out) && c < C; ++c) {
         const int64_t pid = (int64_t)c * N + g;
-        float x = dot3f(R00, R01, R02, mx, my, mz) + t0;
-        float y = dot3f(R10, R11, R12, mx, my, mz) + t1;
-        float z = dot3f(R20, R21, R22, mx, my, mz) + t2;
-        bool valid = !(z < near_plane || z > far_plane);
-        float m2x = 0, m2y = 0, ca = 0, cb = 0, cc = 0, radius = 0;
-        if (valid) {
-            float T0 = dot3f(R00, R01, R02, cov0, cov1, cov2), T1 = dot3f(R00, R01, R02, cov1, cov3, cov4),
-                  T2 = dot3f(R00, R01, R02, cov2, cov4, cov5);
-            float T3 = dot3f(R10, R11, R12, cov0, cov1, cov2), T4 = dot3f(R10, R11, R12, cov1, cov3, cov4),
-                  T5 = dot3f(R10, R11, R12, cov2, cov4, cov5);
-            float T6 = dot3f(R20, R21, R22, cov0, cov1, cov2), T7 = dot3f(R20, R21, R22, cov1, cov3, cov4),
-                  T8 = dot3f(R20, R21, R22, cov2, cov4, cov5);
-            float c0 = dot3f(T0, T1, T2, R00, R01, R02);
-            float c1 = dot3f(T0, T1, T2, R10, R11, R12);
-            float c2 = dot3f(T0, T1, T2, R20, R21, R22);
-            float c3 = dot3f(T3, T4, T5, R10, R11, R12);
-            float c4 = dot3f(T3, T4, T5, R20, R21, R22);
-            float c5 = dot3f(T6, T7, T8, R20, R21, R22);
-            const float fx = o[12], fy = o[13], cx = o[14], cy = o[15];
-            float rz = 1.0f / z;
-            float rz2 = rz * rz;
-            float xr = x * rz, yr = y * rz;
-            float tx = z * fminf(o[16], fmaxf(-o[17], xr));
-            float ty = z * fminf(o[18], fmaxf(-o[19], yr));
-            float a = fx * rz, cj = -(fx * tx) * rz2;
-            float b = fy * rz, d = -(fy * ty) * rz2;
-            float t0x = a * c0 + cj * c2;
-            float t0y = a * c1 + cj * c4;
-            float t0z = a * c2 + cj * c5;
-            float t1y = b * c3 + d * c4;
-            float t1z = b * c4 + d * c5;
-            float c00 = t0x * a + t0z * cj;
-            float c01 = t0y * b + t0z * d;
-            float c11 = t1y * b + t1z * d;
-            m2x = (fx * x) * rz + cx;
-            m2y = (fy * y) * rz + cy;
-            c00 += eps2d; c11 += eps2d;
-            float det = c00 * c11 - c01 * c01;
-            if (det <= 0.0f) valid = false;
-            else {
-                float inv_det = 1.0f / det;
-                ca = c11 * inv_det; cb = -c01 * inv_det; cc = c00 * inv_det;
-                float bb = 0.5f * (c00 + c11);
-                float v1 = bb + sqrtf(fmaxf(0.01f, bb * bb - det));
-                radius = ceilf(3.0f * sqrtf(v1));
-                if (radius <= radius_clip) valid = false;
-                else if (m2x + radius <= 0.0f || m2x - radius >= (float)W || m2y + radius <= 0.0f ||
-                         m2y - radius >= (float)H)
-                    valid = false;
-            }
-        }
-        float4 r0 = make_float4(0, 0, 0, 0), r1 = r0, r2 = r0;
         int ntiles = 0;
         TileRect tr = {0, 0, 0, 0};
-        if (valid) {
-            float dx = mx - o[20], dy = my - o[21], dz = mz - o[22];
-            float inorm = 1.0f / sqrtf((dx * dx + dy * dy) + dz * dz);
-            dx *= inorm; dy *= inorm; dz *= inorm;
-            float col[3];
+        if (active) {
+            const float* o = cam + c * CAM_STRIDE;
+            const float R00 = o[0], R01 = o[1], R02 = o[2], t0 = o[3];
+            const float R10 = o[4], R11 = o[5], R12 = o[6], t1 = o[7];
+            const float R20 = o[8], R21 = o[9], R22 = o[10], t2 = o[11];
+            float x = dot3f(R00, R01, R02, mx, my, mz) + t0;
+            float y = dot3f(R10, R11, R12, mx, my, mz) + t1;
+            float z = dot3f(R20, R21, R22, mx, my, mz) + t2;
+            bool valid = !(z < near_plane || z > far_plane);
+            float m2x = 0, m2y = 0, ca = 0, cb = 0, cc = 0, radius = 0;
+            if (valid) {
+                float T0 = dot3f(R00, R01, R02, cov0, cov1, cov2), T1 = dot3f(R00, R01, R02, cov1, cov3, cov4),
+                      T2 = dot3f(R00, R01, R02, cov2, cov4, cov5);
+                float T3 = dot3f(R10, R11, R12, cov0, cov1, cov2), T4 = dot3f(R10, R11, R12, cov1, cov3, cov4),
+                      T5 = dot3f(R10, R11, R12, cov2, cov4, cov5);
+                float T6 = dot3f(R20, R21, R22, cov0, cov1, cov2), T7 = dot3f(R20, R21, R22, cov1, cov3, cov4),
+                      T8 = dot3f(R20, R21, R22, cov2, cov4, cov5);
+                float c0 = dot3f(T0, T1, T2, R00, R01, R02);
+                float c1 = dot3f(T0, T1, T2, R10, R11, R12);
+                float c2 = dot3f(T0, T1, T2, R20, R21, R22);
+                float c3 = dot3f(T3, T4, T5, R10, R11, R12);
+                float c4 = dot3f(T3, T4, T5, R20, R21, R22);
+                float c5 = dot3f(T6, T7, T8, R20, R21, R22);
+                const float fx = o[12], fy = o[13], cx = o[14], cy = o[15];
+                float rz = 1.0f / z;
+                float rz2 = rz * rz;
+                float xr = x * rz, yr = y * rz;
+                float tx = z * fminf(o[16], fmaxf(-o[17], xr));
+                float ty = z * fminf(o[18], fmaxf(-o[19], yr));
+                float a = fx * rz, cj = -(fx * tx) * rz2;
+                float b = fy * rz, d = -(fy * ty) * rz2;
+                float t0x = a * c0 + cj * c2;
+                float t0y = a * c1 + cj * c4;
+                float t0z = a * c2 + cj * c5;
+                float t1y = b * c3 + d * c4;
+                float t1z = b * c4 + d * c5;
+                float c00 = t0x * a + t0z * cj;
+                float c01 = t0y * b + t0z * d;
+                float c11 = t1y * b + t1z * d;
+                m2x = (fx * x) * rz + cx;
+                m2y = (fy * y) * rz + cy;
+                c00 += eps2d; c11 += eps2d;
+                float det = c00 * c11 - c01 * c01;
+                if (det <= 0.0f) valid = false;
+                else {
+                    float inv_det = 1.0f / det;
+                    ca = c11 * inv_det; cb = -c01 * inv_det; cc = c00 * inv_det;
+                    float bb = 0.5f * (c00 + c11);
+                    float v1 = bb + sqrtf(fmaxf(0.01f, bb * bb - det));
+                    radius = ceilf(3.0f * sqrtf(v1));
+                    if (radius <= radius_clip) valid = false;
+                    else if (m2x + radius <= 0.0f || m2x - radius >= (float)W || m2y + radius <= 0.0f ||
+                             m2y - radius >= (float)H)
+                        valid = false;
+                }
+            }
+            float4 r0 = make_float4(0, 0, 0, 0), r1 = r0, r2 = r0;
+            if (valid) {
+                float dx = mx - o[20], dy = my - o[21], dz = mz - o[22];
+                float inorm = 1.0f / sqrtf((dx * dx + dy * dy) + dz * dz);
+                dx *= inorm; dy *= inorm; dz *= inorm;
+                float col[3];
 #pragma unroll
-            for (int ch = 0; ch < 3; ++ch) {
-                float r = SH_C0 * k[ch];
-                r = r + SH_C1 * ((-dy * k[3 + ch] + dz * k[6 + ch]) - dx * k[9 + ch]);
-                r = r + 0.5f;
-                col[ch] = r < 0.0f ? 0.0f : r;
-            }
-            tr = ref_tile_rect(m2x, m2y, radius, tile_size, tile_w, tile_h);
-            n_ref += (tr.y1 - tr.y0) * (tr.x1 - tr.x0);
-            if (tight) tr = tight_tile_rect(tr, m2x, m2y, opac, ca, cb, cc);
-            ntiles = (tr.y1 - tr.y0) * (tr.x1 - tr.x0);
-            r0 = make_float4(m2x, m2y, opac, ca);
-            r1 = make_float4(cb, cc, col[0], col[1]);
-            r2 = make_float4(col[2], z, __int_as_float((int)radius), 0.0f);
-        }
-        splats[pid * 3 + 0] = r0;
-        splats[pid * 3 + 1] = r1;
-        splats[pid * 3 + 2] = r2;
-        if (tiles_per_gauss) tiles_per_gauss[pid] = ntiles;
-        if (rects) rect_store(rects, rect32, pid, tr);
-        if (depth_keys) {
-            const uint32_t dbits = valid ? (uint32_t)__float_as_int(z) : 0xFFFFFFFFu;
-            if (key_base) {
-                const uint32_t kk = valid ? dbits - key_base : 0x1FFFFFFFu;
-                reinterpret_cast<uint32_t*>(depth_keys)[pid] = (krange_part ? 0u : ((uint32_t)c << 29)) | kk;
-                if (valid) { kmin = min(kmin, kk); kmax = max(kmax, kk); }
-            } else
-                depth_keys[pid] = ((uint64_t)c << 32) | dbits;
-            if (!krange_part) depth_vals[pid] = (int32_t)pid;
-        }
-        n_vis += valid ? 1 : 0;
+                for (int ch = 0; ch < 3; ++ch) {
+                    float r = SH_C0 * k[ch];
+                    r = r + SH_C1 * ((-dy * k[3 + ch] + dz * k[6 + ch]) - dx * k[9 + ch]);
+                    r = r + 0.5f;
+                    col[ch] = r < 0.0f ? 0.0f : r;
+                }
+                tr = ref_tile_rect(m2x, m2y, radius, tile_size, tile_w, tile_h);
+                n_ref += (tr.y1 - tr.y0) * (tr.x1 - tr.x0);
+                if (tight) tr = tight_tile_rect(tr, m2x, m2y, opac, ca, cb, cc);
+                ntiles = (tr.y1 - tr.y0) * (tr.x1 - tr.x0);
+                r0 = make_float4(m2x, m2y, opac, ca);
+                r1 = make_float4(cb, cc, col[0], col[1]);
+                r2 = make_float4(col[2], z, __int_as_float((int)radius), 0.0f);
+            }
+            splats[pid * 3 + 0] = r0;
+            splats[pid * 3 + 1] = r1;
+            splats[pid * 3 + 2] = r2;
+            if (tiles_per_gauss) tiles_per_gauss[pid] = ntiles;
+            if (rects) rect_store(rects, rect32, pid, tr);
+            if (depth_keys) {
+                const uint32_t dbits = valid ? (uint32_t)__float_as_int(z) : 0xFFFFFFFFu;
+                if (key_base) {
+                    const uint32_t kk = valid ? dbits - key_base : 0x1FFFFFFFu;
+                    reinterpret_cast<uint32_t*>(depth_keys)[pid] = (krange_part ? 0u : ((uint32_t)c << 29)) | kk;
+                    if (valid) { kmin = min(kmin, kk); kmax = max(kmax, kk); }
+                } else
+                    depth_keys[pid] = ((uint64_t)c << 32) | dbits;
+                if (!krange_part) depth_vals[pid] = (int32_t)pid;
+            }
+            n_vis += valid ? 1 : 0;
+        }
+        if (hand_out) {
+            const int inc = wave_incl_scan(ntiles);
+            if (active) {
+                const uint32_t w_ = (uint32_t)(tr.x1 - tr.x0);
+                const uint32_t geo = ntiles ? ((uint32_t)tr.x0 & 0x3FF) | (((uint32_t)tr.y0 & 0x3FF) << 10) | ((w_ & 0x3FF) << 20) : 0u;
+                slot_words[pid] = ((uint64_t)(uint32_t)(inc - ntiles) << 32) | geo;
+            }
+            if ((threadIdx.x & 63) == 63 && (g >> 6) < groups) wave_tiles[c * groups + (g >> 6)] = inc;
+        }
     }
     if (krange_part) {
         for (int off = 32; off > 0; off >>= 1) { kmin = min(kmin, (uint32_t)__shfl_down((int)kmin, off)); kmax = max(kmax, (uint32_t)__shfl_down((int)kmax, off)); }
@@ -249,7 +264,8 @@
 int st3r_project_impl(st3r_ctx* ctx, hipStream_t s, const GsParams& g, const GsViews& v, int tile_size, float eps2d,
                       float near_plane, float far_plane, float radius_clip, float* splats, int32_t* tiles_per_gauss,
                       double* reg_sums, uint64_t* depth_keys, int32_t* depth_vals, int tight, uint32_t key_base, void* rects,
-                      int rect32, int reg_overwrite, double* zero_ptr, int zero_n, uint32_t* krange) {
+                      int rect32, int reg_overwrite, double* zero_ptr, int zero_n, uint32_t* krange, uint64_t* slot_words,
+                      int32_t* wave_tiles) {
     const int N = g.N, C = v.C, width = v.W, height = v.H;
     if (N == 0) {
         if (reg_sums && reg_overwrite) HIP_TRY(hipMemsetAsync(reg_sums, 0, sizeof(double) * 4, s));
@@ -272,7 +288,7 @@
     hipLaunchKernelGGL(k_project_sh_fwd, grid, block, shmem, s, N, C, g.means, g.quats, g.scales, g.opacities, g.sh,
                        g.sh_stride, v.viewmats, v.Ks, v.campos, width, height, tile_size, tile_w, tile_h, eps2d, near_plane, far_plane,
                        radius_clip, (float4*)splats, tiles_per_gauss, reg_part, depth_keys, depth_vals, tight, key_base,
-                       rects, rect32, krange_part);
+                       rects, rect32, krange_part, slot_words, wave_tiles);
     if (reg_sums)
         hipLaunchKernelGGL(k_reg_reduce, dim3(1), dim3(256), 0, s, (int)grid.x, reg_part, reg_sums, reg_overwrite, zero_ptr,
                            zero_ptr ? zero_n : 0, (const uint32_t*)krange_part, krange);
@@ -292,5 +308,5 @@
     ARG_CHECK(means && quats && scales && opacities && sh && viewmats && Ks && campos && splats && tiles_per_gauss);
     return st3r_project_impl(ctx, (hipStream_t)stream, GsParams{N, means, quats, scales, opacities, sh, sh_stride},
                              GsViews{C, width, height, viewmats, Ks, campos}, tile_size, eps2d, near_plane, far_plane, radius_clip, splats,
-                             tiles_per_gauss, reg_sums, nullptr, nullptr, 0, 0u, nullptr, 0, 0, nullptr, 0, nullptr);
-}
+                             tiles_per_gauss, reg_sums, nullptr, nullptr, 0, 0u, nullptr, 0, 0, nullptr, 0, nullptr, nullptr, nullptr);
+}
diff --git a/starst3r_amd/csrc/gs_project_bwd.hip b/starst3r_amd/csrc/gs_project_bwd.hip
--- a/starst3r_amd/csrc/gs_project_bwd.hip
+++ b/starst3r_amd/csrc/gs_project_bwd.hip
@@ -6,7 +6,7 @@
 #define GATHER_WIDE_ABOVE 6
 #endif
 
-template <bool GATHER>
+template <bool GATHER, bool REL = false>
 __global__ __launch_bounds__(256) __attribute__((amdgpu_waves_per_eu(4))) void k_project_sh_bwd(
     int N, int C, const float* __restrict__ means, const float* __restrict__ quats,
     const float* __restrict__ scales, const float* __restrict__ opacities, const float* __restrict__ sh,
@@ -14,7 +14,7 @@
     const float* __restrict__ campos, int W, int H, float eps2d, const float4* __restrict__ splats,
     const float4* __restrict__ v_splats, float reg_o_k, float reg_s_k, float* __restrict__ grads, int accumulate,
     int g_begin, int g_end, int range_major, const int32_t* __restrict__ cum, const float* __restrict__ vtile, int stamp,
-    unsigned vt_cap, const uint32_t* __restrict__ touch) {
+    unsigned vt_cap, const uint32_t* __restrict__ touch, st3r_slot_bases rel) {
     extern __shared__ float cam[];
     constexpr int ROW = ACC_VALS;
     __shared__ float sVal[GATHER ? 256 * ROW : 1];
@@ -89,8 +89,14 @@
         if (GATHER) {
             const int lane = threadIdx.x & 63, wv = threadIdx.x >> 6;
             float* wval = sVal + wv * (64 * ROW);
-            const int my_end = cum[pid];
-            const int my_start = !valid ? my_end : (pid == 0 ? 0 : cum[pid - 1]);
+            int my_end, my_start;
+            if (REL) {
+                my_end = slot_end(rel, c, g);
+                my_start = valid ? slot_base(rel, c, g) : my_end;
+            } else {
+                my_end = cum[pid];
+                my_start = !valid ? my_end : (pid == 0 ? 0 : cum[pid - 1]);
+            }
             const int s0 = __builtin_amdgcn_readfirstlane(my_start);
             const int s1 = __builtin_amdgcn_readlane(my_end, 63);
             float acc[ACC_VALS];
@@ -332,15 +338,17 @@
     float reg_s_k = reg_views * scale_fac / (3.0f * (float)N);
     size_t shmem = (size_t)C * CAM_STRIDE * sizeof(float);
     if (slots)
-        hipLaunchKernelGGL(k_project_sh_bwd<true>, dim3(ceil_div(g_end - g_begin, 256)), dim3(256), shmem, s, N, C, g.means,
+        hipLaunchKernelGGL((slots->rel.tab ? k_project_sh_bwd<true, true> : k_project_sh_bwd<true, false>), dim3(ceil_div(g_end - g_begin, 256)), dim3(256), shmem, s, N, C, g.means,
                            g.quats, g.scales, g.opacities, g.sh, g.sh_stride, v.viewmats, v.Ks, v.campos, v.W, v.H, eps2d,
                            (const float4*)splats, (const float4*)nullptr, reg_o_k, reg_s_k, grads, accumulate ? 1 : 0, g_begin,
-                           g_end, range_major ? 1 : 0, slots->cum, slots->vtile, slots->stamp, slots->vt_cap, slots->touch);
+                           g_end, range_major ? 1 : 0, slots->cum, slots->vtile, slots->stamp, slots->vt_cap, slots->touch,
+                           slots->rel);
     else
-        hipLaunchKernelGGL(k_project_sh_bwd<false>, dim3(ceil_div(g_end - g_begin, 256)), dim3(256), shmem, s, N, C, g.means,
+        hipLaunchKernelGGL((k_project_sh_bwd<false, false>), dim3(ceil_div(g_end - g_begin, 256)), dim3(256), shmem, s, N, C, g.means,
                            g.quats, g.scales, g.opacities, g.sh, g.sh_stride, v.viewmats, v.Ks, v.campos, v.W, v.H, eps2d,
                            (const float4*)splats, (const float4*)v_splats, reg_o_k, reg_s_k, grads, accumulate ? 1 : 0, g_begin,
-                           g_end, range_major ? 1 : 0, (const int32_t*)nullptr, (const float*)nullptr, 0, 0u, (const uint32_t*)nullptr);
+                           g_end, range_major ? 1 : 0, (const int32_t*)nullptr, (const float*)nullptr, 0, 0u, (const uint32_t*)nullptr,
+                           st3r_slot_bases{});
     LAUNCH_CHECK();
     return ST3R_OK;
 }
diff --git a/starst3r_amd/csrc/stages.h b/starst3r_amd/csrc/stages.h
--- a/starst3r_amd/csrc/stages.h
+++ b/starst3r_amd/csrc/stages.h
@@ -17,6 +17,7 @@
     int C, W, H, tile_w, tile_h;
     const float* splats; const int32_t *offsets, *flat, *cum; const uint64_t *rects, *rectbase;
     int tight;
+    st3r_slot_bases rel;
     int64_t n_pairs;
     int64_t n_isects, n_records, n_isects_ref, n_visible;
 };
@@ -24,8 +25,8 @@
 static inline RasterOut stage_lists(int C, int W, int H, int tile_w, int tile_h, const float* splats, const int32_t* offsets,
                                     const int32_t* flat, int64_t n_isects, const int32_t* cum = nullptr,
                                     int64_t n_pairs = 0) {
-    return RasterOut{C, W, H, tile_w, tile_h, splats, offsets, flat, cum, nullptr, nullptr, 0, n_pairs, n_isects, n_isects,
-                     n_isects, -1};
+    return RasterOut{C, W, H, tile_w, tile_h, splats, offsets, flat, cum, nullptr, nullptr, 0, st3r_slot_bases{}, n_pairs,
+                     n_isects, n_isects, n_isects, -1};
 }
 
 struct DepthPrior { const float* prior; const float* weight; const double* norm; float fac; };
@@ -44,7 +45,8 @@
 int st3r_project_impl(st3r_ctx* ctx, hipStream_t s, const GsParams& g, const GsViews& v, int tile_size, float eps2d,
                       float near_plane, float far_plane, float radius_clip, float* splats, int32_t* tiles_per_gauss,
                       double* reg_sums, uint64_t* depth_keys, int32_t* depth_vals, int tight, uint32_t key_base, void* rects,
-                      int rect32, int reg_overwrite, double* zero_ptr, int zero_n, uint32_t* krange);
+                      int rect32, int reg_overwrite, double* zero_ptr, int zero_n, uint32_t* krange, uint64_t* slot_words,
+                      int32_t* wave_tiles);
 int st3r_project_sh_bwd_impl(hipStream_t s, const GsParams& g, const GsViews& v, float eps2d, const float* splats,
                              const float* v_splats, float reg_views, float opac_fac, float scale_fac, float* grads,
                              bool accumulate, int g_begin, int g_end, bool range_major, const st3r_vtile_ref* slots);
@@ -76,6 +78,7 @@
                         const float* v_rgb, const float* v_alpha, float* v_splats, bool end_in_offsets,
                         st3r_vtile_ref* defer);
 int st3r_gather_vtile_impl(hipStream_t s, int64_t n_pairs, const st3r_vtile_ref* slots, float* v_splats);
+int st3r_slot_scan_expand_impl(hipStream_t s, int64_t n_pairs, const st3r_slot_bases& rel, int32_t* cum);
 int st3r_blend_depth_fwd_impl(st3r_ctx* ctx, hipStream_t s, const RasterOut& ro, const int32_t* last_ids, float* depth,
                               bool end_in_offsets);
 int st3r_blend_depth_bwd_impl(st3r_ctx* ctx, hipStream_t s, const RasterOut& ro, const float* alpha,
```

Result: no change. 202.4 (median of 6 runs) (+0.9%).
